# ghar1821/Chronoclust

Hardware: AMD Instinct MI355X
Metric: points clustered/sec (20-dim) (higher is better)
Workload: dtype f64; 1 GPU; C2: 1 timepoint, 1000000x20 synthetic blobs (seed 42+rank), 5000 microclusters; exact sequential semantics; online + offline phases per step; one independent st; points=1000000, dim=20, microclusters=5000, clusters=5000, streams=1

## Files before the change

### chronoclust_amd/csrc/cc_api.hip

```cpp
#include <hip/hip_runtime.h>

#include <algorithm>
#include <chrono>
#include <cmath>
#include <cstdio>
#include <cstdlib>
#include <cstring>
#include <limits>
#include <optional>
#include <string>
#include <thread>
#include <type_traits>
#include <vector>

#include "../../include/chronoclust_hip.h"
#include "cc_comm.h"
#include "cc_common.h"
#include "cc_csv.h"
#include "cc_offline.h"
#include "cc_online.h"
#include "cc_policy.h"

#include "cc_handle.h"

namespace {


template <int DP, bool DIRTY>
void launch_scan_dp(cc_handle* h, hipStream_t st, int win, Rows rows, const Cand* clean, Cand* part, int S, int round,
                    int mode, int shard_rank, int shard_world, int phase);

template <int DP>
int scan_u_wgs_per_cu()
{
    constexpr int NW = ScanShape<DP, false>::NW;
    static int blocks = 0;
    static const bool ok = hipOccupancyMaxActiveBlocksPerMultiprocessor(&blocks, k_scan_u<DP, NW>, 64 * NW, 0) == hipSuccess && blocks >= 1;
    return ok ? blocks : ScanUShape<DP>::WGS;
}

template <int DP>
ScanPlan scan_plan_dp(const cc_handle* h)
{
    ScanPlan p;
    p.dp = DP;
    const bool filter = h->hc.filter != 0, pow2 = h->hc.pow2 != 0;
    p.scan_u = h->allow_scan_u && !filter && pow2 && h->d == DP;
    if (p.scan_u && DP > 8) p.chain = ScanPlan::COMMON;
    else if (h->allow_scan_p3 && h->allow_prune_general && h->d == DP && DP > 8 && DP <= 40 && (filter || !pow2))
        p.chain = ScanPlan::GENERAL;
    const bool p3 = h->allow_scan_p3 && DP <= 40;
    p.form = p3 ? ScanPlan::P3 : (h->allow_scan_p2 && DP <= 40 ? ScanPlan::P2 : ScanPlan::P1);
    if (p.chain == ScanPlan::COMMON && h->split_a_mode == 2) p.split_rows = 0;
    else if (p.chain == ScanPlan::COMMON && h->split_a_mode == 1 && !p3) p.split_rows = 10000;
    p.listed_rows = h->p3_listed_rows;
    const bool p3_sized = p3 && h->split_a_mode != 2;
    p.seed16 = h->allow_seed16 && (p.chain == ScanPlan::GENERAL || p3_sized);
    p.prune_applicable = p.chain != ScanPlan::NONE ? 1 : 0;
    p.allow_guess = (h->allow_guess && p.chain != ScanPlan::GENERAL) ? (h->allow_lean ? 1 : 2) : 0;
    p.allow_probe = (h->allow_probe && p.chain != ScanPlan::GENERAL) ? 1 : 0;
    p.force_prune_rows = (p.prune_applicable && h->allow_seed16 && p3_sized) ? h->force_prune_rows : 0;
    p.waves = ScanShape<DP, false>::NW;
    p.dirty_waves = ScanShape<DP, true>::NW;
    p.plain_wgs_per_cu = p.scan_u ? scan_u_wgs_per_cu<DP>() : ScanShape<DP, false>::WGS;
    p.prune_wgs_per_cu = h->prune_rounds4 > 0 ? h->prune_rounds4 : (DP <= 20 ? (p3_sized ? 8 : 16) : 24);
    return p;
}

ScanPlan scan_plan(const cc_handle* h)
{
    const int d = h->d;
    return d <= 4 ? scan_plan_dp<4>(h) : d <= 8 ? scan_plan_dp<8>(h) : d <= 14 ? scan_plan_dp<14>(h) : d <= 16 ? scan_plan_dp<16>(h)
         : d <= 20 ? scan_plan_dp<20>(h) : d <= 32 ? scan_plan_dp<32>(h) : d <= 40 ? scan_plan_dp<40>(h) : scan_plan_dp<64>(h);
}

template <int DP>
struct ScanCall {
    static constexpr int NW = ScanShape<DP, false>::NW;
    cc_handle* h; hipStream_t st; const Rows& rows;
    int round, mode, win, S;
    Cand* part;

    void scan_u(int n_pts, int srank, int sworld, const int* plist) const
    {
        hipLaunchKernelGGL((k_scan_u<DP, NW>), dim3((n_pts + 63) / 64, S), dim3(64 * NW), 0, st, h->ctl.p, h->Xt.p, rows.cen,
                           rows.scl, rows.kind, rows.key, part, round, mode, h->part_stride, srank, sworld, plist);
    }
    void prefix16() const
    {
        ensure_prefix16(h);
        const size_t a16_rows = h->tab.cap + 2 * CC_P16_TM;
        hipLaunchKernelGGL((k_prefix16<DP>), dim3((unsigned)((a16_rows + 255) / 256)), dim3(256), 0, st, (const Ctl*)h->ctl.p,
                           rows.cen, rows.kind, h->a16.p, h->hdr16.p, h->a16_stride, round, mode);
    }
    void seeds(int n_pts, int Sp, const int* plist, bool s16) const
    {
        const dim3 grid((n_pts + 127) / 128, Sp), block(64 * NW);
        if (s16) {
            if constexpr (DP <= 40) {
                hipLaunchKernelGGL((k_seed16<DP, NW>), grid, block, 0, st, (const Ctl*)h->ctl.p, (const double*)h->Xt.p, rows.cen, h->spart.p,
                                   round, mode, h->spart_stride, (const cc_h8*)h->a16.p, (const Prefix16Hdr*)h->hdr16.p, h->a16_stride);
                ++h->stats.seed16_launches;
            } else {
                throw HipErr{hipErrorInvalidValue, "k_seed16 is compiled up to 40 dimensions"};
            }
        } else {
            hipLaunchKernelGGL((k_seed<DP, NW>), grid, block, 0, st, h->ctl.p, h->Xt.p, rows.cen, rows.kind, h->spart.p, round, mode,
                               h->spart_stride, h->cmax.p, plist);
        }
        hipLaunchKernelGGL((k_seed_merge<DP>), dim3((2 * n_pts + 63) / 64), dim3(64), 0, st, h->ctl.p, h->X.p, rows.cen, rows.scl, h->spart.p,
                           h->spart_stride, Sp, h->thr.p, h->thr32.p, h->thr_stride, s16 ? 0.0 : h->prune_F, round, mode, h->cmax.p,
                           h->pstat_p(), plist);
    }
    template <bool LISTED, bool GENERAL>
    void scan_p3(unsigned lds, int srank, int sworld, double gF, unsigned long long* found) const
    {
        hipLaunchKernelGGL((k_scan_p3<DP, NW, LISTED, GENERAL>), dim3((win + 127) / 128, S), dim3(64 * NW), lds, st, h->ctl.p, h->Xt.p,
                           rows.cen, rows.scl, rows.kind, rows.key, h->thr.p, h->thr_stride, part, round, mode, h->part_stride, srank,
                           sworld, h->pstat_p(), gF, found, (const cc_h8*)h->a16.p, (const Prefix16Hdr*)h->hdr16.p, h->a16_stride,
                           GENERAL ? (const double*)h->X.p : nullptr, GENERAL ? rows.cf1 : nullptr, GENERAL ? rows.cf2 : nullptr,
                           GENERAL ? rows.w : nullptr);
    }
    void scan_p(int n_pts, int Sp, Cand* p, size_t p_stride, int srank, int sworld, const int* plist, double gF,
                unsigned long long* found) const
    {
        hipLaunchKernelGGL((k_scan_p<DP, NW, false>), dim3((n_pts + 63) / 64, Sp), dim3(64 * NW), 0, st, h->ctl.p, h->Xt.p, rows.cen,
                           rows.scl, rows.kind, rows.key, h->thr.p, h->thr32.p, h->thr_stride, p, round, mode, p_stride, srank, sworld,
                           h->pstat_p(), plist, gF, found, (const unsigned*)nullptr, (size_t)0, 0, 1);
    }
    void scan_split(int srank, int sworld, double gF, unsigned long long* found) const
    {
        const int nsub = S * NW;
        const int tps = cc_mask_tiles_per_sub((int)std::min<size_t>(h->tab.cap, (size_t)INT_MAX - 64), nsub);
        const size_t need = (size_t)((win + 127) / 128) * (size_t)nsub * (size_t)tps;
        if (need > h->mask_stride) { h->masks.ensure(2 * need); h->mask_stride = need; }
        hipLaunchKernelGGL((k_scan_a<DP, NW>), dim3((win + 127) / 128, S), dim3(64 * NW), 0, st, (const Ctl*)h->ctl.p,
                           (const double*)h->Xt.p, rows.cen, rows.kind, (const double*)h->thr.p, h->thr_stride, h->masks.p,
                           h->mask_stride, tps, round, mode, srank, sworld, gF);
        int q = 1;
        const int tiles = (win + 63) / 64;
        const int resident = h->n_cus * (DP <= 20 ? CC_SCANP_WGS20 : (DP <= 40 ? 3 : 2));
        for (int c = 1; c <= S; ++c)
            if (S % c == 0 && 2 * tiles * (S / c) >= 3 * resident) q = c;
        static const int q_env = []() { const char* e = getenv("CHRONOCLUST_HIP_SCANB_Q"); return e ? atoi(e) : 0; }();
        if (q_env > 0 && S % q_env == 0) q = q_env;
        hipLaunchKernelGGL((k_scan_p<DP, NW, true>), dim3(tiles, S / q), dim3(64 * NW), 0, st, h->ctl.p, h->Xt.p, rows.cen, rows.scl,
                           rows.kind, rows.key, h->thr.p, h->thr32.p, h->thr_stride, part, round, mode, h->part_stride, srank, sworld,
                           h->pstat_p(), (const int*)nullptr, gF, found, (const unsigned*)h->masks.p, h->mask_stride, tps, q);
    }
};

template <int DP, bool DIRTY>
void launch_scan_dp(cc_handle* h, hipStream_t st, int win, Rows rows, const Cand* clean, Cand* part, int S, int round,
                    int mode, int shard_rank, int shard_world, int phase)
{
    constexpr int NW = ScanShape<DP, DIRTY>::NW;
    const dim3 block(64 * NW);
    constexpr int TILE = 64 * ScanShape<DP, DIRTY>::PT;
    const dim3 grid((win + TILE - 1) / TILE, S);
    if constexpr (!DIRTY) {
        static_assert(ScanShape<DP, false>::PT == 1, "k_scan_u holds one window point per lane");
        const ScanPlan& pl = h->scan_plan;
        const ScanCall<DP> L{h, st, rows, round, mode, win, S, part};
        if (pl.scan_u) ++h->stats.scan_u_launches;
        if constexpr (DP > 8) {
            auto window_scan = [&](int srank, int sworld, double gF, unsigned long long* found, bool have_prefix16) {
                if (pl.split(h->hc.m_rows)) return L.scan_split(srank, sworld, gF, found);
                if constexpr (DP <= 40) {
                    if (pl.form == ScanPlan::P3) {
                        if (!have_prefix16) L.prefix16();
                        const bool listed = pl.listed(h->hc.m_rows);
                        if (pl.chain == ScanPlan::GENERAL) {
                            if (listed) L.template scan_p3<true, true>(0, srank, sworld, gF, found);
                            else L.template scan_p3<false, true>(0, srank, sworld, gF, found);
                        } else {
                            static const char* const lds_kb = getenv("CHRONOCLUST_HIP_SCAN_LDS_KB");
                            static const unsigned p3_lds = lds_kb ? (unsigned)atoi(lds_kb) * 1024u : 0u;
                            if (listed) L.template scan_p3<true, false>(p3_lds, srank, sworld, gF, found);
                            else L.template scan_p3<false, false>(p3_lds, srank, sworld, gF, found);
                        }
                        ++h->stats.scan_p2_launches;
                        return;
                    }
                    if (pl.form == ScanPlan::P2) {
                        hipLaunchKernelGGL((k_scan_p2<DP, NW>), dim3((win + 127) / 128, S), block, 0, st, h->ctl.p, h->Xt.p, rows.cen, rows.scl,
                                           rows.kind, rows.key, h->thr.p, h->thr_stride, part, round, mode, h->part_stride, srank, sworld,
                                           h->pstat_p(), gF, found);
                        ++h->stats.scan_p2_launches;
                        return;
                    }
                }
                L.scan_p(win, S, part, h->part_stride, srank, sworld, nullptr, gF, found);
            };
            auto seeded_chain = [&](int n_pts, const int* plist, Cand* p, size_t p_stride, int Sp, int srank, int sworld) {
                const bool whole_window = plist == nullptr && n_pts == win && p_stride == h->part_stride && Sp == S;
                const bool s16 = whole_window && pl.seed16;
                const bool have_prefix16 = whole_window && (s16 || pl.chain == ScanPlan::GENERAL);
                if constexpr (DP <= 40) if (have_prefix16) L.prefix16();
                L.seeds(n_pts, Sp, plist, s16);
                if (whole_window) window_scan(srank, sworld, 0.0, nullptr, have_prefix16);
                else L.scan_p(n_pts, Sp, p, p_stride, srank, sworld, plist, 0.0, nullptr);
            };
            auto missed_scan = [&](const int* list) {
                if (!h->allow_missed_plain) return seeded_chain(CC_MISSED_CAP, list, part, h->part_stride, S, shard_rank, shard_world);
                ++h->stats.missed_plain_launches;
                L.scan_u(CC_MISSED_CAP, shard_rank, shard_world, list);
            };
            if (pl.chain == ScanPlan::GENERAL && h->prune_now && phase == 0) {
                ++h->stats.scan_p_launches;
                return seeded_chain(win, nullptr, part, h->part_stride, S, shard_rank, shard_world);
            }
            if (pl.chain == ScanPlan::COMMON) {
                if (phase == 1) {
                    hipLaunchKernelGGL(k_missed_g, dim3(1), dim3(1024), 0, st, h->ctl.p, (const Cand*)h->gpart.p, h->gpart_stride,
                                       (size_t)win * 4 + 4, shard_world, h->missed.p, CC_MISSED_CAP, round, mode, h->found.p);
                    return missed_scan(h->missed.p);
                }
                if (!h->prune_now) {
                    L.scan_u(win, shard_rank, shard_world, nullptr);
                    if (!h->probe_now) return;
                    ++h->stats.probe_launches;
                    const int Sp = (int)std::max<size_t>(1, std::min<size_t>(128, h->spart_stride / 2 / 128));
                    h->probe_part.ensure((size_t)2 * 128 * Sp * 4);
                    return seeded_chain(std::min(win, 128), nullptr, h->probe_part.p, (size_t)128 * Sp * 4, Sp, 0, 1);
                }
                ++h->stats.scan_p_launches;
                if (!h->guess_now) return seeded_chain(win, nullptr, part, h->part_stride, S, shard_rank, shard_world);
                ++h->stats.scan_g_launches;
                unsigned long long* const found = h->lean_now ? nullptr : h->found.p;
                if (h->group_guess_now) {
                    hipLaunchKernelGGL(k_pstat_zero, dim3(1), dim3(2), 0, st, (const Ctl*)h->ctl.p, h->pstat_p(), round, mode);
                    return window_scan(shard_rank, shard_world, h->prune_F, found, false);
                }
                window_scan(0, 1, h->prune_F, found, false);
                if (h->lean_now) { ++h->stats.scan_lean_launches; return; }
                hipLaunchKernelGGL(k_missed, dim3(1), dim3(1024), 0, st, h->ctl.p, h->found.p, h->missed.p, CC_MISSED_CAP, round, mode);
                return missed_scan(h->missed.p);
            }
        }
// ... 386 lines not shown
```

### chronoclust_amd/csrc/cc_api_comm.inc

```

namespace {

void comm_all_reduce_sum(cc_handle* h, double* buf, size_t count, hipStream_t st)
{
    cc::Comm& cm = h->comm;
    if (cm.broken) throw cc::CommErr{"the group has failed earlier"};
    if (cm.rccl()) {
        cm.check(cc::RcclApi::get().AllReduce(buf, buf, count, ncclDouble, ncclSum, cm.lane(0), st), "ncclAllReduce");
        return;
    }
    if (!cm.local || cm.world == 1) return;
    h->r_gather.ensure((size_t)cm.world * count);
    cm.all_gather(buf, h->r_gather.p, count * 8, st);
    hipLaunchKernelGGL(k_sum_ranks, dim3((unsigned)((count + 255) / 256)), dim3(256), 0, st, h->r_gather.p, cm.world, count, buf);
}

int online_relaxed(cc_handle* h)
{
    const long long N = h->n_points;
    const int W = h->comm.world, rank = h->comm.rank, d = h->d;
    if (N == 0) return (int)CC_OK;
    if (d == 0) return fail(h, CC_ERR_BAD_ARG, "no points uploaded");
    const long long L = (N + W - 1) / W;
    const long long a0 = std::min(N, (long long)rank * L), e0 = std::min(N, a0 + L);
// ... 69 lines not shown
        }
        if (h->trace) {
            const auto tA3 = std::chrono::steady_clock::now();
            auto ms = [](auto x, auto y) { return std::chrono::duration<double, std::milli>(y - x).count(); };
            fprintf(stderr, "[cc] relaxed super-step %lld: %lld points | snapshot %.3f ms, sharded half %.3f ms, merge + collect %.3f ms, set aside %lld\n",
                    sidx, e - a, ms(tA0, tA1), ms(tA1, tA2), ms(tA2, tA3), total);
        }
        h->rstats.super_steps += 1;
        h->rstats.minibatch_points += e - a;
        const long long K = (long long)list.size();
        if (K > 0) {
            h->rstats.deferred_points += K;
            h->r_didx_all.ensure((size_t)std::max<long long>((long long)W * (b + 1), K));
            HIPCHK(hipMemcpyAsync(h->r_didx_all.p, list.data(), (size_t)K * 4, hipMemcpyHostToDevice, st));
            h->rg_X.ensure((size_t)K * d); h->rg_Xt.ensure((size_t)K * d); h->rg_uid.ensure((size_t)K); h->rg_path.ensure((size_t)K);
            hipLaunchKernelGGL(k_rel_gather_points, dim3((unsigned)(((size_t)K * d + 255) / 256)), dim3(256), 0, st, h->X.p,
                               h->r_didx_all.p, (int)K, d, h->rg_X.p);
            hipLaunchKernelGGL(k_transpose_points, dim3((unsigned)(((size_t)K * d + 255) / 256)), dim3(256), 0, st, h->rg_X.p,
                               h->rg_Xt.p, K, d);
            auto swap_in = [&]() {
                h->X.swap(h->rg_X);
                h->Xt.swap(h->rg_Xt);
                h->lab_uid.swap(h->rg_uid);
                h->lab_path.swap(h->rg_path);
            };
            swap_in();
            h->n_points = K;
            const int keep_win = h->adapt_win, keep_clean = h->clean_batches, keep_shrink = h->since_shrink;
            auto restore_policy = [&]() { h->adapt_win = keep_win; h->clean_batches = keep_clean; h->since_shrink = keep_shrink; };
            try {
                rc = online_range(h, 0, K, false, false);
            } catch (...) {
                swap_in();
                h->n_points = N;
                restore_policy();
                throw;
            }
            swap_in();
            h->n_points = N;
            restore_policy();
            if (rc != CC_OK) return rc;
            hipLaunchKernelGGL(k_rel_scatter_labels, dim3((unsigned)((K + 255) / 256)), dim3(256), 0, st, h->rg_uid.p,
                               h->rg_path.p, h->r_didx_all.p, (int)K, h->lab_uid.p, h->lab_path.p);
        }
    }
    h->comm.all_gather(h->lab_uid.p + (size_t)rank * L, h->lab_uid.p, (size_t)L * 8, st);
    h->comm.all_gather(h->lab_path.p + (size_t)rank * L, h->lab_path.p, (size_t)L, st);
    sync_stream(h, st);
    HIPCHK(hipGetLastError());
    h->stats.points = N;
    return (int)CC_OK;
}

}

extern "C" {


int cc_comm_unique_id(void* out_id)
{
    if (!out_id) return CC_ERR_BAD_ARG;
    cc::RcclApi& api = cc::RcclApi::get();
    if (!api.ok()) return CC_ERR_COMM;
    ncclUniqueId id;
    if (api.GetUniqueId(&id) != ncclSuccess) return CC_ERR_COMM;
    static_assert(sizeof(id) == CC_COMM_ID_BYTES, "ncclUniqueId size");
    memcpy(out_id, &id, sizeof(id));
    return CC_OK;
}

int cc_comm_init_rccl(cc_handle* h, const void* id_bytes, int rank, int world)
{
    if (!h || !id_bytes || world < 1 || rank < 0 || rank >= world) return CC_ERR_BAD_ARG;
    return guarded(h, [&]() {
        if (h->comm.active()) return fail(h, CC_ERR_BAD_ARG, "the handle already belongs to a group");
        cc::RcclApi& api = cc::RcclApi::get();
        if (!api.ok()) return fail(h, CC_ERR_COMM, std::string("librccl could not be loaded: ") + (dlerror() ? dlerror() : "missing symbol"));
        ncclUniqueId id;
        memcpy(&id, id_bytes, sizeof(id));
        ncclComm_t comm = nullptr;
        ncclResult_t r = api.CommInitRank(&comm, world, id, rank);
        if (r != ncclSuccess) return fail(h, CC_ERR_COMM, std::string("ncclCommInitRank: ") + api.GetErrorString(r));
        h->comm.nccl[0] = comm;
        h->comm.rank = rank;
        h->comm.world = world;
        h->comm.broken = false;
        const char* to = getenv("CHRONOCLUST_HIP_COMM_TIMEOUT_S");
        if (to && atof(to) > 0.0) h->comm.timeout_s = atof(to);
        const char* two = getenv("CHRONOCLUST_HIP_TWO_COMMS");
        if (two && two[0] == '1') {
            DevBuf<char> ids;
            ids.ensure((size_t)world * sizeof(ncclUniqueId) + sizeof(ncclUniqueId));
            ncclUniqueId id2;
            memset(&id2, 0, sizeof id2);
            if (rank == 0) {
                r = api.GetUniqueId(&id2);
                if (r != ncclSuccess) return fail(h, CC_ERR_COMM, std::string("ncclGetUniqueId: ") + api.GetErrorString(r));
            }
            char* send = ids.p + (size_t)world * sizeof(ncclUniqueId);
            HIPCHK(hipMemcpyAsync(send, &id2, sizeof id2, hipMemcpyHostToDevice, h->stream));
            h->comm.all_gather(send, ids.p, sizeof id2, h->stream, 0);
            HIPCHK(hipMemcpyAsync(&id2, ids.p, sizeof id2, hipMemcpyDeviceToHost, h->stream));
            sync_stream(h, h->stream);
            ncclComm_t comm2 = nullptr;
            r = api.CommInitRank(&comm2, world, id2, rank);
            if (r != ncclSuccess) return fail(h, CC_ERR_COMM, std::string("ncclCommInitRank (second communicator): ") + api.GetErrorString(r));
            h->comm.nccl[1] = comm2;
        }
        const char* cal = getenv("CHRONOCLUST_HIP_CALIBRATE");
        if (!(cal && cal[0] == '0')) {
            const int rc = cc_comm_calibrate(h);
            if (rc != CC_OK) return rc;
        }
        return (int)CC_OK;
    });
}

int cc_comm_calibrate(cc_handle* h)
{
    if (!h) return CC_ERR_BAD_ARG;
    return guarded(h, [&]() {
        if (!h->comm.active()) return fail(h, CC_ERR_BAD_ARG, "cc_comm_calibrate: the handle belongs to no group");
        const int world = h->comm.world, rank = h->comm.rank;
        hipEvent_t e0 = nullptr, e1 = nullptr;
        HIPCHK(hipEventCreate(&e0));
        HIPCHK(hipEventCreate(&e1));
        auto timed3 = [&](auto&& fn) {
            fn();
            sync_stream(h, h->stream);
            float best = 1e30f;
            for (int i = 0; i < 3; ++i) {
                HIPCHK(hipEventRecord(e0, h->stream));
                fn();
                HIPCHK(hipEventRecord(e1, h->stream));
                sync_stream(h, h->stream);
                float ms = 0.f;
                HIPCHK(hipEventElapsedTime(&ms, e0, e1));
                best = std::min(best, ms);
            }
            return (double)best * 1e3;
        };
        const int win = std::min(h->tun.window, CC_MAX_WINDOW);
        const size_t rec = ((size_t)win * 4 + 4) * sizeof(Cand);
        DevBuf<char> sbuf, rbuf;
        sbuf.ensure(rec);
        rbuf.ensure(rec * (size_t)world);
        HIPCHK(hipMemsetAsync(sbuf.p, 0, rec, h->stream));
        const double ag_us = timed3([&]() { h->comm.all_gather(sbuf.p, rbuf.p, rec, h->stream, 0); });
        constexpr int DPc = 20, Rc = 4096;
        constexpr int NWc = ScanShape<DPc, false>::NW;
        DevBuf<Ctl> cctl;
        DevBuf<double> cxt, ccen, cscl;
        DevBuf<int> ckind, ckey;
        DevBuf<Cand> cpart;
        const int tiles = (win + 63) / 64;
        const int Sc = std::max(1, std::min(16, (h->n_cus * scan_u_wgs_per_cu<DPc>()) / std::max(1, tiles)));
        cctl.ensure(1); cxt.ensure((size_t)win * DPc); ccen.ensure((size_t)Rc * DPc); cscl.ensure((size_t)Rc * DPc);
        ckind.ensure(Rc); ckey.ensure(Rc); cpart.ensure((size_t)2 * win * Sc * 4);
        {
            std::vector<double> x((size_t)win * DPc), cen((size_t)Rc * DPc), scl((size_t)Rc * DPc, 0.25);
            unsigned long long st = 0x9E3779B97F4A7C15ull;
            auto rnd = [&]() { st = st * 6364136223846793005ull + 1442695040888963407ull; return (double)(st >> 11) * 0x1p-53; };
            for (auto& v : x) v = 0.1 + 0.8 * rnd();
            for (auto& v : cen) v = 0.1 + 0.8 * rnd();
            std::vector<int> kind(Rc, CC_KIND_PCORE), key(Rc);
            for (int i = 0; i < Rc; ++i) key[i] = i;
            Ctl c;
            memset(&c, 0, sizeof c);
            c.d = DPc; c.m_rows = Rc; c.win_b = win; c.win_cfg = win; c.n_points = win; c.xt_stride = win;
            c.k = 4.0; c.inv_k = 0.25; c.pow2 = 1;
            HIPCHK(hipMemcpyAsync(cctl.p, &c, sizeof c, hipMemcpyHostToDevice, h->stream));
            HIPCHK(hipMemcpyAsync(cxt.p, x.data(), x.size() * 8, hipMemcpyHostToDevice, h->stream));
            HIPCHK(hipMemcpyAsync(ccen.p, cen.data(), cen.size() * 8, hipMemcpyHostToDevice, h->stream));
            HIPCHK(hipMemcpyAsync(cscl.p, scl.data(), scl.size() * 8, hipMemcpyHostToDevice, h->stream));
            HIPCHK(hipMemcpyAsync(ckind.p, kind.data(), (size_t)Rc * 4, hipMemcpyHostToDevice, h->stream));
            HIPCHK(hipMemcpyAsync(ckey.p, key.data(), (size_t)Rc * 4, hipMemcpyHostToDevice, h->stream));
            sync_stream(h, h->stream);
        }
        const double scan_us = timed3([&]() {
            hipLaunchKernelGGL((k_scan_u<DPc, NWc>), dim3(tiles, Sc), dim3(64 * NWc), 0, h->stream, (const Ctl*)cctl.p, (const double*)cxt.p,
                               (const double*)ccen.p, (const double*)cscl.p, (const int*)ckind.p, (const int*)ckey.p, cpart.p, 0, 0,
                               (size_t)win * Sc * 4, 0, 1);
        });
        HIPCHK(hipGetLastError());
        (void)hipEventDestroy(e0);
        (void)hipEventDestroy(e1);
        double mine[2] = {ag_us, scan_us * 1e3 / ((double)Rc * DPc)};
        DevBuf<double> dsend, drecv;
        dsend.ensure(2);
        drecv.ensure((size_t)2 * world);
        HIPCHK(hipMemcpyAsync(dsend.p, mine, sizeof mine, hipMemcpyHostToDevice, h->stream));
        h->comm.all_gather(dsend.p, drecv.p, sizeof mine, h->stream, 0);
        std::vector<double> all((size_t)2 * world);
        HIPCHK(hipMemcpyAsync(all.data(), drecv.p, all.size() * 8, hipMemcpyDeviceToHost, h->stream));
        sync_stream(h, h->stream);
        double ag = 0.0, sc = 0.0;
        for (int r = 0; r < world; ++r) { ag = std::max(ag, all[(size_t)2 * r]); sc = std::max(sc, all[(size_t)2 * r + 1]); }
        h->calib_ag_us = ag;
        h->calib_scan_ns = sc;
        if (world > 1 && sc > 0.0) {
            const double row_dims = ag * 1e3 * (double)world / (double)(world - 1) / sc;
            h->shard_min_row_dims = (long long)std::min(row_dims, 1e15);
            h->shard_min_row_dims_pruned = (long long)std::min(row_dims * 3.3, 1e15);
        }
        if (h->trace)
            fprintf(stderr, "[cc] rank %d of %d: all-gather of a %d-point window's records %.1f us, plain scan %.3f ns per (row, dim) "
                    "(group maxima) -> scans split from %lld (plain) / %lld (pruned) row-dims on\n", rank, world, win, ag, sc,
                    (long long)h->shard_min_row_dims, (long long)(h->shard_min_row_dims_pruned > 0 ? h->shard_min_row_dims_pruned : h->shard_min_row_dims));
        return (int)CC_OK;
    });
}

int cc_comm_init_local(cc_handle** handles, int world)
{
    if (!handles || world < 1) return CC_ERR_BAD_ARG;
    for (int r = 0; r < world; ++r)
        if (!handles[r] || handles[r]->comm.active()) return CC_ERR_BAD_ARG;
    auto grp = std::make_shared<cc::LocalGroup>(world);
    for (int r = 0; r < world; ++r) {
        cc_handle* h = handles[r];
        int rc = guarded(h, [&]() {
            HIPCHK(hipEventCreateWithFlags(&h->comm.ev_ready, hipEventDisableTiming));
            HIPCHK(hipEventCreateWithFlags(&h->comm.ev_done, hipEventDisableTiming));
            return (int)CC_OK;
        });
        if (rc != CC_OK) {
            for (int q = 0; q <= r; ++q) handles[q]->comm.destroy();
            return rc;
        }
    }
    for (int r = 0; r < world; ++r) {
        handles[r]->comm.local = grp;
        handles[r]->comm.rank = r;
        handles[r]->comm.world = world;
    }
    return CC_OK;
}

int cc_comm_destroy(cc_handle* h)
{
    if (!h) return CC_ERR_BAD_ARG;
    return guarded(h, [&]() {
        try {
            sync_stream(h, h->stream);
            sync_stream(h, h->stream2);
        } catch (const cc::CommErr&) {
        }
        h->comm.destroy();
        return (int)CC_OK;
    });
}

int cc_comm_info(cc_handle* h, int32_t* rank, int32_t* world, int32_t* transport)
{
    if (!h) return CC_ERR_BAD_ARG;
    if (rank) *rank = h->comm.rank;
    if (world) *world = h->comm.world;
    if (transport) *transport = h->comm.rccl() ? 1 : (h->comm.local ? 2 : 0);
    return CC_OK;
}

int cc_comm_set_relaxed(cc_handle* h, int32_t minibatch_points)
{
    if (!h || minibatch_points < 0) return CC_ERR_BAD_ARG;
    if (minibatch_points > 0 && !h->comm.active()) return fail(h, CC_ERR_BAD_ARG, "the relaxed mode needs a group (cc_comm_init_*)");
    h->relaxed_minibatch = minibatch_points;
    return CC_OK;
}

int cc_get_relaxed_stats(cc_handle* h, cc_relaxed_stats* out)
{
    if (!h || !out) return CC_ERR_BAD_ARG;
    *out = h->rstats;
    return CC_OK;
}

int cc_set_shard_thresholds(cc_handle* h, int64_t min_row_dims, int32_t offline_min_rows)
{
    if (!h) return CC_ERR_BAD_ARG;
    if (min_row_dims >= 0) { h->shard_min_row_dims = min_row_dims; h->shard_min_row_dims_pruned = 0; }
    if (offline_min_rows >= 0) h->offline_shard_min_rows = offline_min_rows;
    return CC_OK;
}

}
```

### chronoclust_amd/csrc/cc_common.h

```cpp
#pragma once
#include <hip/hip_runtime.h>
#include <stdint.h>

#include "cc_host.h"

#define CC_KIND_PCORE 0
#define CC_KIND_OUTLIER 1
#define CC_KIND_DEAD 2

#define CC_MAX_ROUNDS 8
#define CC_T_UNKNOWN (-2)
#define CC_T_NONE (-3)
#define CC_IDX_INF 0x7fffffff

#define CC_SLOT_BOUND (-2)
struct __attribute__((aligned(16))) Cand {
    double dist;
    int key;
    int slot;
};

struct Table {
    double* cf1;
    double* cf2;
    double* cen;
    double* pref;
    double* scl;
    double* w;
    int* kind;
    int* key;
    long long* id;
    long long* uid;
    unsigned long long* touch;
    unsigned long long* last;
    unsigned long long* carry_of;
    unsigned long long* cnt;
    int* memb;
    int* clen;
    int* heavy;
    size_t cap;
};
#define CC_HEAVY_CAP 64
#define CC_HEAVY_NEW 32

#define CC_CAR_BASE (1 << 24)
#define CC_MAX_WINDOW 49152
#define CC_CHAIN_MEMB 32
#define CC_LONG_CAP 512
#define CC_LONG_LISTED (1ull << 23)
#ifndef CC_CHAIN_AHEAD
#define CC_CHAIN_AHEAD 4
#endif

struct Carry {
    double* cf1;
    double* cf2;
    double* cen;
    double* pref;
    double* scl;
    double* w;
    int* kind;
    int* key;
    int* slot;
    double* c0;
    double* w0;
    int* kind0;
    double* dsq;
    unsigned long long* tile_dsq;
};

struct Versions {
    double* cf1;
    double* cf2;
    double* cen;
    double* pref;
    double* scl;
    double* w;
    int* kind;
    int* key;
    int* next;
    int* upg;
    int* acc;
    int* tgt;
    double* dsq;
    unsigned long long* tile_dsq;
    double* tau;
    int* skip;
    int* skip_car;
    int* unsafe;
};

struct Rows {
    const double* cen;
    const double* scl;
    const double* pref;
    const double* cf1;
    const double* cf2;
    const double* w;
    const int* kind;
    const int* key;
    const int* next;
    const unsigned long long* tile_dsq;
    const double* dsq;
    const double* tau;
    const int* skip;
    const int* plist;
    const int* slot;
    const unsigned long long* touch;
    size_t cap;
};

struct Ctl {
    long long cursor;
    long long n_points;
    long long xt_stride;
    int no_create;
    int pad1;
    int d;
    int m_rows;
    int n_pkeys, n_okeys;
    long long pcore_last_id, outlier_last_id;
    unsigned long long window_seq;
    int win_cfg;
    int win_b;
    int max_rounds;
    int last_round;
    int fc[CC_MAX_ROUNDS + 2];
    int any_new[CC_MAX_ROUNDS + 2], any_up[CC_MAX_ROUNDS + 2];
    int n_long[CC_MAX_ROUNDS + 2];
    long long stat_long;
    double eps_sq, delta_sq, k, inv_k, beta_mu, mu, omicron;
    int pi;
    int filter;
    int pow2;
    int pad0;
    int mode;
    int car_n;
    int la_on;
    int stall_b;
    long long la_cursor[2];
    int la_b[2];
    int la_rows[2];
    long long stat_windows, stat_rounds, stat_truncated;
    long long stat_table_rows;
    double stat_pair_rows;
    long long round_hist[CC_MAX_ROUNDS + 2];
    long long stat_lookahead;
    long long stat_trunc_unknown;
    long long stat_unprovable, stat_unsafe;
    long long stat_tiles, stat_dirty_tiles;
    long long stat_seq_points;
    long long stat_seq_clk, stat_seq_wall;
    unsigned long long stat_prune_rows, stat_prune_full;
    int n_sparse;
    int pad2;
    double tg[2][2];
    int tg_ok[2][2];
    int n_missed[2];
    unsigned long long cen_absmax;
    double x_absmax;
    long long stat_missed;
    unsigned long long pstat[2][2];
    int n_missed_all[2];
    int seq_rest;
    int pad3;
    long long stat_seq_r_points;
    long long seed_at;
    int rdiff[CC_MAX_ROUNDS + 2];
    int n_heavy, n_heavy_new;
    int heavy_list[CC_HEAVY_CAP];
    int heavy_new[CC_HEAVY_NEW];
#ifdef CC_LONG_TIMERS
    unsigned long long dbg_long[8];
#endif
#ifdef CC_ROUND_DEBUG
    unsigned long long dbg_round[CC_MAX_ROUNDS + 2][6];
#endif
};

#define CC_MISSED_CAP 2048
#define CC_DSQ_STRIDE 4
#define CC_TAU_STRIDE 4
#define CC_FLAG_U0 1
#define CC_FLAG_U1 2
#define CC_FLAG_C0 4
#define CC_FLAG_C1 8
#define CC_FLAG_N1SKIP 32
#define CC_FLAG_SPARSE 64

__host__ __device__ inline bool cand_less(double ad, int ak, double bd, int bk)
{
    return ad < bd || (ad == bd && ak < bk);
}
```

### chronoclust_amd/csrc/cc_handle.h

```cpp
#pragma once
#include "cc_knobs.h"

namespace {

struct HipErr {
    hipError_t e;
    const char* what;
};

#define HIPCHK(call)                                  \
    do {                                              \
        hipError_t _e = (call);                       \
        if (_e != hipSuccess) throw HipErr{_e, #call}; \
    } while (0)

template <typename T>
struct DevBuf {
    T* p = nullptr;
    size_t n = 0;
    void ensure(size_t count)
    {
        if (count <= n && p) return;
        release();
        size_t want = std::max<size_t>(count, 1);
        if (hipMalloc((void**)&p, want * sizeof(T)) != hipSuccess) {
            p = nullptr;
            throw HipErr{hipErrorOutOfMemory, "hipMalloc"};
        }
        n = want;
    }
    void release()
    {
        if (p) (void)hipFree(p);
        p = nullptr;
        n = 0;
    }
    ~DevBuf() { release(); }
    DevBuf() = default;
    DevBuf(const DevBuf&) = delete;
    DevBuf& operator=(const DevBuf&) = delete;
    DevBuf(DevBuf&& o) noexcept { swap(o); }
    DevBuf& operator=(DevBuf&& o) noexcept
    {
        if (this != &o) { release(); swap(o); }
        return *this;
    }
    void swap(DevBuf& o) noexcept
    {
        std::swap(p, o.p);
        std::swap(n, o.n);
    }
};

struct TableStore {
    DevBuf<double> cf1, cf2, cen, pref, scl, w;
    DevBuf<int> kind, key;
    DevBuf<long long> id, uid;
    DevBuf<unsigned long long> touch, last, carry_of, cnt;
    DevBuf<int> memb, clen, heavy;
    size_t cap = 0;
    int d = 0;
    enum Grow { KEPT, CLEARED, CLEARED_KEPT, SCRATCH };
    template <typename F>
    static void for_each_column(int dims, F&& f)
    {
        const size_t dim = (size_t)dims;
        f(&TableStore::cf1, dim, KEPT); f(&TableStore::cf2, dim, KEPT); f(&TableStore::cen, dim, KEPT);
        f(&TableStore::pref, dim, KEPT); f(&TableStore::scl, dim, KEPT);
        f(&TableStore::w, (size_t)1, KEPT); f(&TableStore::kind, (size_t)1, KEPT); f(&TableStore::key, (size_t)1, KEPT);
        f(&TableStore::id, (size_t)1, KEPT); f(&TableStore::uid, (size_t)1, KEPT);
        f(&TableStore::touch, (size_t)2, CLEARED); f(&TableStore::last, (size_t)2, CLEARED);
        f(&TableStore::carry_of, (size_t)1, CLEARED_KEPT);
        f(&TableStore::cnt, (size_t)1, CLEARED); f(&TableStore::memb, (size_t)CC_CHAIN_MEMB, SCRATCH);
        f(&TableStore::clen, (size_t)1, CLEARED);
        f(&TableStore::heavy, (size_t)1, CLEARED_KEPT);
    }
    void alloc(size_t rows, int dim)
    {
        for_each_column(dim, [&](auto col, size_t per_row, Grow) { (this->*col).ensure(rows * per_row); });
        cap = rows;
        d = dim;
    }
    Table view() const { return Table{cf1.p, cf2.p, cen.p, pref.p, scl.p, w.p, kind.p, key.p, id.p, uid.p, touch.p, last.p, carry_of.p, cnt.p, memb.p, clen.p, heavy.p, cap}; }
};

struct HostClusters {
    std::vector<int> mem, off{0};
    size_t size() const { return off.size() - 1; }
    void clear() { mem.clear(); off.assign(1, 0); }
};

}

struct PinArena {
    char* p = nullptr;
    size_t cap = 0, used = 0;
    void reset() { used = 0; }
    void reserve(size_t bytes)
    {
        if (bytes <= cap) return;
        if (p) (void)hipHostFree(p);
        p = nullptr;
        cap = 0;
        const size_t want = std::max<size_t>(bytes, (size_t)1 << 20);
        if (hipHostMalloc((void**)&p, want, hipHostMallocDefault) != hipSuccess) {
            p = nullptr;
            throw HipErr{hipErrorOutOfMemory, "hipHostMalloc"};
        }
        cap = want;
    }
    template <typename T>
    T* take(size_t n)
    {
        used = (used + 63) & ~(size_t)63;
        T* r = reinterpret_cast<T*>(p + used);
        used += std::max<size_t>(n, 1) * sizeof(T);
        if (used > cap) throw HipErr{hipErrorOutOfMemory, "page-locked scratch exhausted"};
        return r;
    }
    ~PinArena() { if (p) (void)hipHostFree(p); }
    PinArena() = default;
    PinArena(const PinArena&) = delete;
    PinArena& operator=(const PinArena&) = delete;
};

struct ScanPlan {
    int dp = 0;
    bool scan_u = false;
    enum Chain { NONE, COMMON, GENERAL } chain = NONE;
    enum Form { P3, P2, P1 } form = P1;
    long long split_rows = std::numeric_limits<long long>::max(), listed_rows = 0;
    bool seed16 = false;
    int prune_applicable = 0, allow_guess = 0, allow_probe = 0, force_prune_rows = 0;
    int waves = 4, dirty_waves = 4;
    int plain_wgs_per_cu = 1, prune_wgs_per_cu = 1;
    bool split(long long m_rows) const { return m_rows >= split_rows; }
    bool listed(long long m_rows) const { return m_rows >= listed_rows; }
};


struct BatchScanState {
    bool prune_now = false;
    bool group_guess_now = false;
    bool lean_now = false;
    bool guess_now = false;
    bool probe_now = false;
    ScanPlan scan_plan;
    void set_prune(int prune)
    {
        prune_now = prune != 0;
        guess_now = prune >= 2;
        lean_now = prune == 3;
    }
};

struct PrunedScanBuffers {
    DevBuf<Cand> probe_part;
    DevBuf<unsigned long long> found;
    DevBuf<int> missed;
    DevBuf<SeedCand> spart;
    DevBuf<double> thr;
    DevBuf<float> thr32;
    DevBuf<unsigned long long> cmax;
    DevBuf<cc_h8> a16;
    DevBuf<Prefix16Hdr> hdr16;
    size_t a16_stride = 0;
    DevBuf<unsigned> masks;
    size_t mask_stride = 0;
    size_t spart_stride = 0, thr_stride = 0;
};

struct WindowBuffers {
    int win_alloc = 0, seg_alloc = 0, d_alloc = 0;
    DevBuf<double> v_cf1, v_cf2, v_cen, v_pref, v_scl, v_w, v_dsq, v_tau;
    DevBuf<unsigned long long> v_tile_dsq;
    DevBuf<int> v_kind, v_key, v_next, v_upg, v_acc, v_tgt, v_skip, v_skip_car, v_unsafe;
    DevBuf<Cand> part, clean, dpart, dpart2, dseed;
    size_t part_stride = 0;
    DevBuf<double> c_cf1v, c_cf2v, c_cenv, c_prefv, c_sclv, c_wv, c_c0, c_w0, c_dsq;
    DevBuf<int> c_kind, c_key, c_slot, c_kind0;
    DevBuf<unsigned long long> c_tile_dsq;
    DevBuf<int> T0, T1, rk;
    DevBuf<int> link_near;
    DevBuf<int> sp_list;
    DevBuf<int> long_list;
    DevBuf<unsigned long long> lstat, lprev;
    bool prep_launched = false;
    DevBuf<CommitRec> rec;
    DevBuf<double> sh_cen[2], sh_scl[2], sh_cf1[2], sh_cf2[2], sh_w[2];
    DevBuf<int> sh_kind[2], sh_key[2];
    DevBuf<int8_t> dpath;
};

struct OfflineResults {
    DevBuf<double> pv_cf1, pv_cf2, pv_cen, pv_pref, pv_w, wvec;
    DevBuf<long long> pv_id;
    DevBuf<int> prow, nn, pdim, mem_dev, off_dev, nw_cnt, nw_nbr;
    DevBuf<long long> nw_off;
    DevBuf<int8_t> core;
    DevBuf<unsigned long long> adj, adjw;
    DevBuf<double> c_cf1, c_cf2, c_cen, c_pref, c_w;
    HostClusters clusters;
    PinArena pin;
    std::vector<long long> pcore_ids_host, pcore_uid_host;
    DevBuf<int32_t> pc_map, pc_out;
    int n_core = 0;
};

struct AssocScratch {
    DevBuf<double> a_cur_cen, a_cur_pref, a_prev_cen, a_dist, a_pdist;
    DevBuf<int> a_idx, a_pidx;
    DevBuf<int> flags;
};

struct RelaxedState {
    int relaxed_minibatch = 0;
    bool shard_suspended = false;
    DevBuf<double> rs_cf1, rs_cf2, rs_w, r_delta, r_gather;
    DevBuf<int> rs_kind, rs_key, r_didx, r_didx_all, r_cnt_all;
    DevBuf<long long> rs_id;
    DevBuf<double> rg_X, rg_Xt;
    DevBuf<long long> rg_uid;
    DevBuf<int8_t> rg_path;
    cc_relaxed_stats rstats{};
};

struct cc_handle : Knobs, BatchScanState, PrunedScanBuffers, WindowBuffers, OfflineResults, AssocScratch, RelaxedState {
    int device = 0;
    hipStream_t stream = nullptr;
    hipStream_t stream2 = nullptr;
    std::string err;
    cc_params par{};
    bool have_par = false;
    cc_tuning tun{};
    cc_stats stats{};

    int d = 0;
    TableStore tab, tab2;
    Ctl hc{};
    Ctl* hc_pin = nullptr;
    DevBuf<Ctl> ctl;
    unsigned long long* pstat_p() const { return (unsigned long long*)((char*)ctl.p + offsetof(Ctl, pstat)); }
    bool tainted = false;
    int adapt_win = 0;
    int clean_batches = 0;
    int since_shrink = 1000;
    DevBuf<int> seq_lists;
    DevBuf<double> seq_img;
    bool seq_sticky = false;
    int n_cus = 256;

    DevBuf<double> X, Xt;
    long long n_points = 0;
    double x_absmax = 0.0;
    DevBuf<long long> lab_uid;
    DevBuf<int8_t> lab_path;
    DevBuf<int> badflag;
    DevBuf<double> scr, scr2;

    struct Prefetch {
        std::thread worker;
        bool active = false;
        const double* x = nullptr;
        long long n = 0;
        int d = 0;
        bool scaled = false;
        std::vector<double> scale, mn;
        DevBuf<double> X, Xt, sm;
        DevBuf<int> bad;
        hipStream_t stream = nullptr;
        void* pin[2] = {nullptr, nullptr};
        size_t pin_bytes = 0;
        int bad_host[4] = {0, 0, 0, 0};
        int rc = 0;
        const char* what = "";
    } pf;

    std::vector<hipEvent_t> ev_pool, sync_pool;

    cc::Comm comm;
    long long shard_min_row_dims = 400000;
    long long shard_min_row_dims_pruned = 0;
    double calib_ag_us = 0.0, calib_scan_ns = 0.0;
    int offline_shard_min_rows = 8192;
    DevBuf<Cand> gsend, gpart;
    DevBuf<Cand> gsend2, gpart2;
    size_t gsend_stride = 0, gpart_stride = 0;
    DevBuf<int> g_i32;
};

namespace {

template <typename F>
void with_bools(F&& f)
{
    f();
}
template <typename F, typename... Rest>
void with_bools(F&& f, bool b, Rest... rest)
{
    if (b) with_bools([&](auto... c) { f(std::true_type{}, c...); }, rest...);
    else with_bools([&](auto... c) { f(std::false_type{}, c...); }, rest...);
}

struct CapacityErr {
    std::string what;
};

int fail(cc_handle* h, int code, const std::string& msg)
{
    if (h) h->err = msg;
    return code;
}

void group_lost(cc_handle* h)
{
    if (h && h->comm.active()) h->comm.fail_group();
}

template <typename F>
int guarded(cc_handle* h, F&& f)
{
    try {
        if (h) HIPCHK(hipSetDevice(h->device));
        const int rc = f();
        if (rc < 0) group_lost(h);
        return rc;
    } catch (const HipErr& e) {
        char buf[512];
        snprintf(buf, sizeof buf, "HIP error %d (%s) in %s", (int)e.e, hipGetErrorString(e.e), e.what);
        group_lost(h);
        return fail(h, e.e == hipErrorOutOfMemory ? CC_ERR_OOM : CC_ERR_NO_DEVICE, buf);
    } catch (const cc::CommErr& e) {
        group_lost(h);
        return fail(h, CC_ERR_COMM, "exchange between ranks failed: " + e.what);
    } catch (const std::bad_alloc&) {
        group_lost(h);
        return fail(h, CC_ERR_OOM, "host allocation failed");
    } catch (const CapacityErr& e) {
        group_lost(h);
        return fail(h, CC_ERR_OOM, e.what);
    }
}

void sync_stream(cc_handle* h, hipStream_t st)
{
    if (h->comm.rccl() || h->comm.broken) h->comm.wait_stream(st);
    else HIPCHK(hipStreamSynchronize(st));
}

bool is_pow2(double k)
{
    if (!(k > 0.0) || !std::isfinite(k)) return false;
    int e;
    double m = std::frexp(k, &e);
    return m == 0.5 && e > -1000 && e < 1000;
}

void refresh_ctl_params(cc_handle* h)
{
    Ctl& c = h->hc;
    const cc_params& p = h->par;
    c.eps_sq = p.eps_sq;
    c.delta_sq = p.delta_sq;
    c.k = p.k;
    c.pow2 = (is_pow2(p.k) && !h->tainted) ? 1 : 0;
    c.inv_k = c.pow2 ? 1.0 / p.k : 0.0;
    c.beta_mu = p.beta * p.mu;
    c.mu = p.mu;
    c.omicron = p.omicron;
    c.pi = p.pi;
    c.filter = (h->d > 0 && p.pi < h->d) ? 1 : 0;
    c.d = h->d;
}

void push_ctl(cc_handle* h)
{
    memset(h->hc.pstat, 0, sizeof(h->hc.pstat));
    h->hc.n_missed_all[0] = h->hc.n_missed_all[1] = 0;
    HIPCHK(hipMemcpyAsync(h->ctl.p, &h->hc, sizeof(Ctl), hipMemcpyHostToDevice, h->stream));
}
void pull_ctl(cc_handle* h)
{
    HIPCHK(hipMemcpyAsync(&h->hc, h->ctl.p, sizeof(Ctl), hipMemcpyDeviceToHost, h->stream));
    sync_stream(h, h->stream);
}
void pull_ctl_pinned(cc_handle* h)
{
    if (!h->hc_pin) { pull_ctl(h); return; }
    HIPCHK(hipMemcpyAsync(h->hc_pin, h->ctl.p, sizeof(Ctl), hipMemcpyDeviceToHost, h->stream));
    sync_stream(h, h->stream);
    memcpy(&h->hc, h->hc_pin, sizeof(Ctl));
}
void push_ctl_pinned(cc_handle* h)
{
    if (!h->hc_pin) { push_ctl(h); return; }
    memset(h->hc.pstat, 0, sizeof(h->hc.pstat));
    h->hc.n_missed_all[0] = h->hc.n_missed_all[1] = 0;
    memcpy(h->hc_pin + 1, &h->hc, sizeof(Ctl));
    HIPCHK(hipMemcpyAsync(h->ctl.p, h->hc_pin + 1, sizeof(Ctl), hipMemcpyHostToDevice, h->stream));
}

#define CC_MAX_TABLE_ELEMS ((size_t)INT_MAX - 1023)

void ensure_table(cc_handle* h, size_t rows)
{
    if (h->tab.cap >= rows && h->tab.d == h->d) return;
    const size_t max_rows = CC_MAX_TABLE_ELEMS / (size_t)std::max(h->d, 1);
    if (rows > max_rows)
        throw CapacityErr{"a table of " + std::to_string(rows) + " rows of " + std::to_string(h->d) + " dimensions: more than " +
                          std::to_string(max_rows) + " rows (" + std::to_string(CC_MAX_TABLE_ELEMS) + " elements) at this width"};
    size_t want = std::min(max_rows, std::max<size_t>(rows, std::max<size_t>(1024, h->tab.cap * 2)));
    TableStore nt;
    nt.alloc(want, h->d);
    const size_t m = (size_t)h->hc.m_rows;
    TableStore& old = h->tab;
    TableStore::for_each_column(h->d, [&](auto col, size_t per_row, TableStore::Grow grow) {
        auto& to = nt.*col;
        const size_t elem = sizeof(*to.p);
        if (grow == TableStore::CLEARED || grow == TableStore::CLEARED_KEPT)
            HIPCHK(hipMemsetAsync(to.p, 0, want * per_row * elem, h->stream));
        if ((grow == TableStore::KEPT || grow == TableStore::CLEARED_KEPT) && m > 0)
            HIPCHK(hipMemcpyAsync(to.p, (old.*col).p, m * per_row * elem, hipMemcpyDeviceToDevice, h->stream));
    });
    sync_stream(h, h->stream);
    std::swap(h->tab, nt);
}

int set_dim(cc_handle* h, int d)
{
    if (d <= 0 || d > CC_MAX_DIM) return fail(h, CC_ERR_BAD_ARG, "d must be in 1.." + std::to_string(CC_MAX_DIM));
    if (h->d == 0) h->d = d;
    if (h->d != d) {
        if (h->hc.m_rows == 0) h->d = d;
        else return fail(h, CC_ERR_BAD_ARG, "dimensionality differs from the microclusters already held");
    }
    return CC_OK;
}

void ensure_window_buffers(cc_handle* h, int win, int seg)
{
    if (win <= h->win_alloc && seg <= h->seg_alloc && h->d <= h->d_alloc) return;
    win = std::max(win, h->win_alloc);
    seg = std::max(seg, h->seg_alloc);
    const size_t w = (size_t)win, d = (size_t)std::max(h->d, h->d_alloc);
    h->v_cf1.ensure(w * d); h->v_cf2.ensure(w * d); h->v_cen.ensure(w * d); h->v_pref.ensure(w * d); h->v_scl.ensure(w * d); h->v_w.ensure(w);
    h->v_kind.ensure(w); h->v_key.ensure(w); h->v_next.ensure(w); h->v_upg.ensure(w); h->v_acc.ensure(w);
    h->v_dsq.ensure(w); h->v_tau.ensure(CC_TAU_STRIDE * w); h->v_tile_dsq.ensure(CC_DSQ_STRIDE * (w / 16 + 2));
    h->v_tgt.ensure(w);
    h->v_skip.ensure(w / 64 + 2); h->v_skip_car.ensure(w / 64 + 2); h->v_unsafe.ensure(w);
    h->part_stride = w * seg * 4;
    h->spart_stride = w * seg * 2;
    h->thr_stride = w * 2;
    h->spart.ensure(2 * h->spart_stride);
    h->thr.ensure(2 * h->thr_stride);
    h->thr32.ensure(2 * h->thr_stride);
    h->cmax.ensure(2);
    h->found.ensure(2 * (CC_MAX_WINDOW / 64));
    h->missed.ensure(2 * CC_MISSED_CAP);
    h->part.ensure(2 * h->part_stride); h->dpart.ensure(w * seg * 2); h->dpart2.ensure(w * seg * 2);
    h->clean.ensure(w * 4); h->dseed.ensure(w * 4);
    h->c_cf1v.ensure(w * d); h->c_cf2v.ensure(w * d); h->c_cenv.ensure(w * d); h->c_prefv.ensure(w * d);
    h->c_sclv.ensure(w * d); h->c_wv.ensure(w); h->c_c0.ensure(w * d); h->c_w0.ensure(w * d);
    h->c_kind.ensure(w); h->c_key.ensure(w); h->c_slot.ensure(w); h->c_kind0.ensure(w); h->c_dsq.ensure(w); h->c_tile_dsq.ensure(CC_DSQ_STRIDE * (w / 16 + 2));
    h->T0.ensure(w + 128); h->T1.ensure(w + 128);
    h->long_list.ensure(2 * CC_LONG_CAP);
    h->lstat.ensure(2 * CC_LSTAT_ROWS + 2);
    h->lprev.ensure(CC_MAX_WINDOW);
    h->dpath.ensure(w); h->rk.ensure(w); h->rec.ensure(1); h->sp_list.ensure(w); h->link_near.ensure(w);
    h->win_alloc = win; h->seg_alloc = seg; h->d_alloc = (int)d;
}

Carry carry_view(cc_handle* h)
{
    return Carry{h->c_cf1v.p, h->c_cf2v.p, h->c_cenv.p, h->c_prefv.p, h->c_sclv.p, h->c_wv.p, h->c_kind.p, h->c_key.p,
                 h->c_slot.p, h->c_c0.p, h->c_w0.p, h->c_kind0.p, h->c_dsq.p, h->c_tile_dsq.p};
}

void scan_copy_sync(cc_handle* h, ScanCopy (&out)[2])
{
    const size_t cap = h->tab.cap, d = (size_t)h->d, m = (size_t)h->hc.m_rows;
    const bool filter = h->hc.filter != 0;
    const TableStore& t = h->tab;
    for (int q = 0; q < 2; ++q) {
        h->sh_cen[q].ensure(cap * d); h->sh_scl[q].ensure(cap * d); h->sh_kind[q].ensure(cap); h->sh_key[q].ensure(cap);
        if (filter) { h->sh_cf1[q].ensure(cap * d); h->sh_cf2[q].ensure(cap * d); h->sh_w[q].ensure(cap); }
        if (m > 0) {
            HIPCHK(hipMemcpyAsync(h->sh_cen[q].p, t.cen.p, m * d * 8, hipMemcpyDeviceToDevice, h->stream));
            HIPCHK(hipMemcpyAsync(h->sh_scl[q].p, t.scl.p, m * d * 8, hipMemcpyDeviceToDevice, h->stream));
            HIPCHK(hipMemcpyAsync(h->sh_kind[q].p, t.kind.p, m * 4, hipMemcpyDeviceToDevice, h->stream));
            HIPCHK(hipMemcpyAsync(h->sh_key[q].p, t.key.p, m * 4, hipMemcpyDeviceToDevice, h->stream));
            if (filter) {
                HIPCHK(hipMemcpyAsync(h->sh_cf1[q].p, t.cf1.p, m * d * 8, hipMemcpyDeviceToDevice, h->stream));
                HIPCHK(hipMemcpyAsync(h->sh_cf2[q].p, t.cf2.p, m * d * 8, hipMemcpyDeviceToDevice, h->stream));
                HIPCHK(hipMemcpyAsync(h->sh_w[q].p, t.w.p, m * 8, hipMemcpyDeviceToDevice, h->stream));
            }
        }
        out[q] = ScanCopy{h->sh_cen[q].p, h->sh_scl[q].p, h->sh_cf1[q].p, h->sh_cf2[q].p, h->sh_w[q].p, h->sh_kind[q].p,
                          h->sh_key[q].p};
    }
}

Versions versions_view(cc_handle* h)
{
    return Versions{h->v_cf1.p, h->v_cf2.p, h->v_cen.p, h->v_pref.p, h->v_scl.p, h->v_w.p, h->v_kind.p,
                    h->v_key.p, h->v_next.p, h->v_upg.p, h->v_acc.p, h->v_tgt.p, h->v_dsq.p, h->v_tile_dsq.p,
                    h->v_tau.p, h->v_skip.p, h->v_skip_car.p, h->v_unsafe.p};
}

void ensure_prefix16(cc_handle* h)
{
    const size_t a16_rows = h->tab.cap + 2 * CC_P16_TM;
    if (h->a16_stride >= a16_rows * 4) return;
    sync_stream(h, h->stream);
    sync_stream(h, h->stream2);
    h->a16.ensure(2 * a16_rows * 4);
    h->a16_stride = a16_rows * 4;
    h->hdr16.ensure(2);
}

hipEvent_t get_event(cc_handle* h, size_t i)
{
    while (h->ev_pool.size() <= i) {
        hipEvent_t e;
        HIPCHK(hipEventCreateWithFlags(&e, h->light_sync_events ? hipEventReleaseToDevice : hipEventDefault));
        h->ev_pool.push_back(e);
    }
    return h->ev_pool[i];
}

hipEvent_t get_sync_event(cc_handle* h, size_t i)
{
    if (!h->light_sync_events) return get_event(h, i);
    while (h->sync_pool.size() <= i) {
        hipEvent_t e;
        HIPCHK(hipEventCreateWithFlags(&e, hipEventDisableTiming | hipEventReleaseToDevice));
        h->sync_pool.push_back(e);
    }
    return h->sync_pool[i];
}


}
```

### chronoclust_amd/csrc/cc_knobs.h

```cpp
#pragma once
#include <algorithm>
#include <climits>
#include <cstdlib>

struct Knobs {
    bool trace = false;
    bool light_sync_events = true;
    int chain_threads = 64, decide_threads = 256, commit_threads = 256;
    bool allow_scan_u = true;
    int prune_mode = 1;
    double prune_F = 16.0;
    int prune_rounds4 = 0;
    bool group_guess_always = false;
    bool allow_guess = true;
    bool allow_lean = true;
    int force_prune_rows = 0;
    bool allow_seed16 = false;
    bool allow_prune_general = true;
    bool la_pruned = false;
    bool allow_probe = true;
    int split_a_mode = 1;
    bool allow_nodirty = true;
    bool allow_claims = true;
    bool allow_long = true;
    bool allow_prep = true;
    bool allow_quiet = true;
    bool allow_missed_plain = true;
    int p3_listed_rows = 10000;
    bool allow_scan_p3 = true;
    bool allow_scan_p2 = true;
    bool allow_link = true;
    bool allow_heavy = true;
    bool allow_seq_r = true;
    bool allow_seq_g = true;
    int allow_sparse = 128;
};

namespace {

void knob_off_when_starts_with_0(bool& v, const char* name) { const char* e = getenv(name); v = !(e && e[0] == '0'); }
void knob_on_when_starts_with_1(bool& v, const char* name) { const char* e = getenv(name); v = e && e[0] == '1'; }
void knob_atoi_nonzero_when_set(bool& v, const char* name) { if (const char* e = getenv(name)) v = atoi(e) != 0; }
void knob_int_in(int& v, const char* name, int lo, int hi) { const char* e = getenv(name); if (e && atoi(e) >= lo && atoi(e) <= hi) v = atoi(e); }
void knob_threads(int& v, const char* name) { int t = 0; knob_int_in(t, name, 64, 256); if (t == 64 || t == 128 || t == 256) v = t; }

void read_knobs(Knobs& k)
{
    knob_on_when_starts_with_1(k.trace, "CHRONOCLUST_HIP_TRACE");
    knob_on_when_starts_with_1(k.group_guess_always, "CHRONOCLUST_HIP_GROUP_GUESS");
    knob_off_when_starts_with_0(k.allow_nodirty, "CHRONOCLUST_HIP_NODIRTY");
    knob_off_when_starts_with_0(k.allow_claims, "CHRONOCLUST_HIP_CLAIMS");
    knob_off_when_starts_with_0(k.allow_long, "CHRONOCLUST_HIP_LONGCHAINS");
    knob_off_when_starts_with_0(k.allow_prep, "CHRONOCLUST_HIP_LONGPREP");
    knob_off_when_starts_with_0(k.allow_quiet, "CHRONOCLUST_HIP_QUIET");
    knob_off_when_starts_with_0(k.allow_heavy, "CHRONOCLUST_HIP_HEAVY");
    knob_off_when_starts_with_0(k.allow_seq_r, "CHRONOCLUST_HIP_SEQR");
    knob_off_when_starts_with_0(k.allow_seq_g, "CHRONOCLUST_HIP_SEQG");
    knob_off_when_starts_with_0(k.allow_probe, "CHRONOCLUST_HIP_PROBE");
    knob_off_when_starts_with_0(k.allow_guess, "CHRONOCLUST_HIP_GUESS");
    knob_off_when_starts_with_0(k.allow_lean, "CHRONOCLUST_HIP_LEAN");
    knob_off_when_starts_with_0(k.allow_scan_p2, "CHRONOCLUST_HIP_SCANP2");
    knob_off_when_starts_with_0(k.allow_link, "CHRONOCLUST_HIP_LINK");
    knob_atoi_nonzero_when_set(k.light_sync_events, "CHRONOCLUST_HIP_LIGHT_EVENTS");
    knob_atoi_nonzero_when_set(k.allow_scan_u, "CHRONOCLUST_HIP_SCANU");
    knob_atoi_nonzero_when_set(k.allow_seed16, "CHRONOCLUST_HIP_SEED16");
    knob_atoi_nonzero_when_set(k.allow_missed_plain, "CHRONOCLUST_HIP_MISSED_PLAIN");
    knob_atoi_nonzero_when_set(k.allow_prune_general, "CHRONOCLUST_HIP_PRUNE_GENERAL");
    knob_atoi_nonzero_when_set(k.allow_scan_p3, "CHRONOCLUST_HIP_SCANP3");
    knob_atoi_nonzero_when_set(k.la_pruned, "CHRONOCLUST_HIP_LA_PRUNED");
    knob_threads(k.chain_threads, "CHRONOCLUST_HIP_CHAIN_THREADS");
    knob_threads(k.decide_threads, "CHRONOCLUST_HIP_DECIDE_THREADS");
    knob_threads(k.commit_threads, "CHRONOCLUST_HIP_COMMIT_THREADS");
    knob_int_in(k.prune_mode, "CHRONOCLUST_HIP_PRUNE", 0, 2);
    knob_int_in(k.prune_rounds4, "CHRONOCLUST_HIP_PRUNE_WGS", 1, 64);
    knob_int_in(k.allow_sparse, "CHRONOCLUST_HIP_SPARSE", 0, INT_MAX);
    knob_int_in(k.force_prune_rows, "CHRONOCLUST_HIP_FORCE_PRUNE_ROWS", INT_MIN, INT_MAX);
    knob_int_in(k.p3_listed_rows, "CHRONOCLUST_HIP_P3_LISTED", INT_MIN, INT_MAX);
    if (const char* e = getenv("CHRONOCLUST_HIP_SCANA")) k.split_a_mode = std::max(0, std::min(2, atoi(e)));
    if (const char* e = getenv("CHRONOCLUST_HIP_PRUNE_F")) if (atof(e) >= 1.0) k.prune_F = atof(e);
}

}
```

### chronoclust_amd/csrc/cc_online.h

```cpp
#pragma once
#include <type_traits>

#include "cc_common.h"

#define CC_INF (__builtin_huge_val())
#define CC_GROUP_THREADS 256

#define CC_LATENCY_KERNEL() __builtin_amdgcn_s_setprio(3)

#define CC_WAVE_SYNC()                                          \
    do {                                                        \
        __builtin_amdgcn_fence(__ATOMIC_RELEASE, "wavefront"); \
        __builtin_amdgcn_wave_barrier();                        \
        __builtin_amdgcn_fence(__ATOMIC_ACQUIRE, "wavefront"); \
    } while (0)


__device__ __forceinline__ double cc_sqvar(double cf1, double cf2, double w)
{
    double a = cf2 / w;
    double b = cf1 / w;
    b = b * b;
    return a - b;
}

struct Par {
    double delta_sq, k, inv_k, eps_sq, beta_mu;
    int pow2, pi, filter, d;
};

__device__ __forceinline__ Par cc_load_par(const Ctl* ctl)
{
    Par p;
    p.delta_sq = ctl->delta_sq; p.k = ctl->k; p.inv_k = ctl->inv_k; p.eps_sq = ctl->eps_sq; p.beta_mu = ctl->beta_mu;
    p.pow2 = ctl->pow2; p.pi = ctl->pi; p.filter = ctl->filter; p.d = ctl->d;
    return p;
}

__device__ __forceinline__ double cc_div_pref(double x, double pref, const Par& c)
{
    if (pref == 1.0) return x;
    return (c.pow2 && pref == c.k) ? x * c.inv_k : x / pref;
}

__device__ inline double cc_tentative_radius(const double* bcf1, const double* bcf2, double bw, const double* p,
                                             int d, const Par& c, int* cnt_gt1, int* cnt_ne1)
{
    const double w1 = bw + 1.0;
    double r2 = 0.0;
    int g = 0, n = 0;
    for (int i = 0; i < d; ++i) {
        double x = p[i];
        double c1 = (bcf1 ? bcf1[i] : 0.0) + x;
        double c2 = (bcf2 ? bcf2[i] : 0.0) + x * x;
        double var = cc_sqvar(c1, c2, w1);
        double pr = (var <= c.delta_sq) ? c.k : 1.0;
        g += (pr > 1.0);
        n += (pr != 1.0);
        r2 = r2 + cc_div_pref(var, pr, c);
    }
    if (cnt_gt1) *cnt_gt1 = g;
    if (cnt_ne1) *cnt_ne1 = n;
    return r2;
}

__device__ __forceinline__ void cc_top2_push(Cand& a, Cand& b, const Cand& x)
{
    const bool ok = x.slot != -1;
    const bool beats_a = ok && (a.slot == -1 || cand_less(x.dist, x.key, a.dist, a.key));
    const bool beats_b = ok && !beats_a && (b.slot == -1 || cand_less(x.dist, x.key, b.dist, b.key));
    b.dist = beats_a ? a.dist : (beats_b ? x.dist : b.dist);
    b.key = beats_a ? a.key : (beats_b ? x.key : b.key);
    b.slot = beats_a ? a.slot : (beats_b ? x.slot : b.slot);
    a.dist = beats_a ? x.dist : a.dist;
    a.key = beats_a ? x.key : a.key;
    a.slot = beats_a ? x.slot : a.slot;
}

__device__ __forceinline__ double cc_vmin(double a, double b)
{
    double r;
    asm("v_min_f64 %0, %1, %2" : "=v"(r) : "v"(a), "v"(b));
    return r;
}
__device__ __forceinline__ double cc_vmax(double a, double b)
{
    double r;
    asm("v_max_f64 %0, %1, %2" : "=v"(r) : "v"(a), "v"(b));
    return r;
}

template <int N, int I = 0, typename F>
__device__ __forceinline__ void cc_static_for(F&& f)
{
    if constexpr (I < N) {
        f(std::integral_constant<int, I>{});
        cc_static_for<N, I + 1>(f);
    }
}

#define CC_TINY 0x1p-400
__device__ __forceinline__ bool cc_is_tiny(double v) { return v != 0.0 && __builtin_fabs(v) < CC_TINY; }

__device__ __forceinline__ unsigned long long cc_dsq_code(double dq) { return (unsigned long long)__double_as_longlong(dq) + 1ull; }
__device__ __forceinline__ bool cc_dsq_below(unsigned long long code, double tau)
{
    if (code == 0ull) return true;
    const double dq = __longlong_as_double((long long)(code - 1ull));
    return dq < CC_INF && sqrt(dq) * (1.0 + 1e-9) < tau;
}

__device__ __forceinline__ int cc_dsq_class(int kind, double dsq_stored)
{
    return (kind == CC_KIND_PCORE) ? (__builtin_signbit(dsq_stored) ? 2 : 0) : 1;
}
__device__ __forceinline__ double cc_dsq_store(double dq, int kind, int kind0, int* cls)
{
    const bool promoted = kind == CC_KIND_PCORE && kind0 == CC_KIND_OUTLIER && dq < CC_INF;
    *cls = (kind == CC_KIND_PCORE) ? (promoted ? 2 : 0) : 1;
    return promoted ? -dq : dq;
}
template <int BIT>
__device__ __forceinline__ double cc_sel_scale(unsigned mask, double scaled, double one)
{
    double r;
    asm("s_bitcmp1_b32 %1, %2\n\ts_cselect_b64 %0, %3, %4" : "=s"(r) : "s"(mask), "n"(BIT), "s"(scaled), "s"(one) : "scc");
    return r;
}

#include "cc_scan.h"
#include "cc_scan16.h"
#include "cc_validate.h"
#include "cc_link.h"
#include "cc_seq.h"
#include "cc_seq_r.h"
#include "cc_seq_g.h"
#include "cc_relaxed.h"
#include "cc_points.h"
```

### chronoclust_amd/csrc/cc_online_run.h

```cpp
#pragma once

namespace {

struct PolicyTrace {
    FILE* f = nullptr;
    static void obs_json(FILE* f, const cc_policy_obs& o)
    {
        fprintf(f, "{\"cursor\": %lld, \"m_rows\": %d, \"stall_b\": %d, \"stat_windows\": %lld, \"stat_truncated\": %lld, "
                   "\"stat_trunc_unknown\": %lld, \"stat_tiles\": %lld, \"stat_dirty_tiles\": %lld, \"stat_unsafe\": %lld, \"stat_missed\": %lld, \"tg_ok\": %d, \"round_hist\": [",
                (long long)o.cursor, o.m_rows, o.stall_b, (long long)o.stat_windows, (long long)o.stat_truncated,
                (long long)o.stat_trunc_unknown, (long long)o.stat_tiles, (long long)o.stat_dirty_tiles, (long long)o.stat_unsafe,
                (long long)o.stat_missed, o.tg_ok);
        for (int r = 0; r < CC_POLICY_MAX_ROUNDS + 2; ++r) fprintf(f, "%s%lld", r ? ", " : "", (long long)o.round_hist[r]);
        fprintf(f, "], \"prune_rows\": %llu, \"prune_full\": %llu, \"after_sequential\": %d}", (unsigned long long)o.prune_rows,
                (unsigned long long)o.prune_full, o.after_sequential);
    }
    static void dec_json(FILE* f, const cc_policy_decision& d)
    {
        fprintf(f, "{\"win_cfg\": %d, \"want\": %d, \"rounds\": %d, \"batch_windows\": %d, \"lookahead\": %d, \"nodirty\": %d, "
                   "\"prune\": %d, \"shard\": %d, \"restart\": %d, \"bad\": %d, \"stalled\": %d, \"sparse\": %d, \"probe\": %d}",
                d.win_cfg, d.want, d.rounds, d.batch_windows, d.lookahead, d.nodirty, d.prune, d.shard, d.restart, d.bad, d.stalled, d.sparse, d.probe);
    }
    PolicyTrace(const cc_policy_config& c, const cc_policy_carry& k, long long cursor, int rows, const cc_policy_decision& d0,
                int rank)
    {
        const char* path = getenv("CHRONOCLUST_HIP_POLICY_TRACE");
        if (!path || !path[0]) return;
        const std::string name = rank >= 0 ? std::string(path) + ".rank" + std::to_string(rank) : std::string(path);
        f = fopen(name.c_str(), "a");
        if (!f) return;
        fprintf(f, "{\"call\": {\"config\": {\"window\": %d, \"rounds_max\": %d, \"windows_per_sync\": %d, \"early_window\": %d, "
                   "\"lookahead\": %d, \"allow_nodirty\": %d, \"prune_mode\": %d, \"prune_applicable\": %d, \"can_shard\": %d, \"d\": %d, "
                   "\"resume\": %d, \"allow_sparse\": %d, \"allow_guess\": %d, \"allow_probe\": %d, \"shard_min_row_dims\": %lld, \"n_end\": %lld, \"shard_min_row_dims_pruned\": %lld, \"lookahead_pruned\": %d, \"force_prune_rows\": %d}, \"carry\": [%d, %d, %d], \"start\": [%lld, %d], \"dec\": ",
                c.window, c.rounds_max, c.windows_per_sync, c.early_window, c.lookahead, c.allow_nodirty, c.prune_mode,
                c.prune_applicable, c.can_shard, c.d, c.resume, c.allow_sparse, c.allow_guess, c.allow_probe, (long long)c.shard_min_row_dims, (long long)c.n_end, (long long)c.shard_min_row_dims_pruned, c.lookahead_pruned, c.force_prune_rows,
                k.adapt_win, k.clean_batches, k.since_shrink, cursor, rows);
        dec_json(f, d0);
        fprintf(f, "}}\n");
    }
    void batch(const cc_policy_obs& o, const cc_policy_decision& d)
    {
        if (!f) return;
        fprintf(f, "{\"obs\": ");
        obs_json(f, o);
        fprintf(f, ", \"dec\": ");
        dec_json(f, d);
        fprintf(f, "}\n");
    }
    void sequential(long long cursor, int rows, const cc_policy_decision& d)
    {
        cc_policy_obs o{};
        o.cursor = cursor;
        o.m_rows = rows;
        o.after_sequential = 1;
        batch(o, d);
    }
    ~PolicyTrace()
    {
        if (f) fclose(f);
    }
    PolicyTrace(const PolicyTrace&) = delete;
    PolicyTrace& operator=(const PolicyTrace&) = delete;
};

void launch_link_scan(cc_handle* h, hipStream_t st, int win)
{
    const dim3 grid((win + 63) / 64, (win + 4 * CC_LINK_SUB - 1) / (4 * CC_LINK_SUB)), block(256);
    const int d = h->d;
#define CC_LINK_DP(DP) hipLaunchKernelGGL((k_link_scan<DP>), grid, block, 0, st, (const Ctl*)h->ctl.p, (const double*)h->X.p, \
                                          (const double*)h->Xt.p, (const int*)h->T0.p, h->link_near.p)
    if (d <= 4) CC_LINK_DP(4);
    else if (d <= 8) CC_LINK_DP(8);
    else if (d <= 14) CC_LINK_DP(14);
    else if (d <= 16) CC_LINK_DP(16);
    else if (d <= 20) CC_LINK_DP(20);
    else if (d <= 32) CC_LINK_DP(32);
    else if (d <= 40) CC_LINK_DP(40);
    else CC_LINK_DP(64);
#undef CC_LINK_DP
}

struct OnlineRun {
    cc_handle* const h;
    const long long range_a, N;
    const bool no_create, resume;
    Ctl& c;

    int win = 0, R = 0;
    int S_cfg = 1, Sd_full = 1, Sd = 1;
    int world = 1, myrank = 0;
    bool grouped = false;
    size_t batch_max = 2;
    bool timing = false;
    int seq_mode = 0, seq_cap = 0;
    Versions ver{};
    Carry car{};
    hipStream_t sA = nullptr, sB = nullptr;
    static constexpr size_t ev_base = 4;

    cc_policy_config pcfg{};
    std::optional<cc::WindowPolicy> policy;
    std::optional<PolicyTrace> ptrace;
    cc_policy_decision dec{};
    bool nodirty = false;
    bool sparse_now = false;
    bool la_on = false;
    bool shard_on = false;
    bool link_now = false;
    int Rcur = 1;
    int batch_windows = 2;

    long long done = 0;
    int m_known = 0;
    unsigned long long seq_host = 0;
    long long cursor_prev = 0;
    double batch_t0 = 0.0;

    hipEvent_t ev0 = nullptr, ev1 = nullptr, evCommit = nullptr, evScan = nullptr;
    size_t ev_used = 2, ev_sync = ev_base;
    std::vector<std::pair<size_t, double>> timed;
    std::vector<size_t> timed_comm;
    double pair_rows_eff = 0.0, pair_rows_prev = 0.0;
    double pair_rows_pruned = 0.0;
    long long sharded_windows = 0;

    bool seq_on = false;
    int bad_batches = 0;
    long long seq_stint_len = 32768, seq_stint_left = 32768;
    bool seq_probe = false;
    double win_rate = 0.0, seq_rate_last = 0.0;

    long long long_prev = 0;
    bool long_seen = false;
    bool long_few = true;
    long long rounds_prev = 0, long_avg = 1;
    long long long_launches = 0;

    OnlineRun(cc_handle* handle, long long a, long long e, bool no_create_, bool resume_)
        : h(handle), range_a(a), N(e), no_create(no_create_), resume(resume_), c(handle->hc) {}

    static double now_ms()
    {
        return std::chrono::duration<double, std::milli>(std::chrono::steady_clock::now().time_since_epoch()).count();
    }
    bool seq_r_applies() const { return h->allow_seq_r && h->d >= 2 && h->d <= 4; }
    bool wide() const { return h->d > CC_WINDOW_MAX_DIM; }
    size_t window_rows() const { return wide() ? 0 : (size_t)win * batch_max; }
    bool seq_g_applies() const { return h->allow_seq_g && h->hc.m_rows >= seq_cap; }
    double seq_rate_guess() const { return cc::seq_rate_guess(h->d, h->hc.m_rows, seq_cap, h->allow_seq_r, h->allow_seq_g); }
    bool seq_possible() const { return seq_mode != 1 && !h->comm.active() && !no_create && (h->hc.m_rows < seq_cap || h->allow_seq_g); }

    void set_lookahead(bool on)
    {
        la_on = on;
        c.la_on = on ? 1 : 0;
        c.stall_b = 0;
        c.mode = 0;
        c.car_n = 0;
        const int q = (int)((c.window_seq + 1ull) & 1ull);
        const long long c1 = c.cursor + c.win_b;
        const long long left1 = c.n_points - c1;
        c.la_cursor[q] = c1;
        c.la_b[q] = (on && left1 > 0) ? (int)std::min<long long>(left1, c.win_cfg) : 0;
        c.la_rows[q] = c.m_rows;
        c.la_cursor[q ^ 1] = 0;
        c.la_b[q ^ 1] = 0;
        c.la_rows[q ^ 1] = 0;
    }

    void prepare()
    {
        refresh_ctl_params(h);
        h->scan_plan = scan_plan(h);
        const ScanPlan& plan = h->scan_plan;
        win = h->tun.window; R = h->tun.rounds;
        S_cfg = std::max(1, h->tun.segments / plan.waves);
        Sd_full = std::max(1, (h->tun.dirty_segments > 0 ? h->tun.dirty_segments : h->tun.segments) / plan.dirty_waves);
        Sd = Sd_full;
        nodirty = false;
        ensure_window_buffers(h, wide() ? 64 : win, std::max(S_cfg, Sd_full));
        world = h->comm.world; myrank = h->comm.rank;
        grouped = h->comm.active();
        if (grouped) {
            const size_t gmax = (size_t)std::max(64, h->win_alloc);
            h->gsend_stride = gmax * 4 + 4;
            h->gpart_stride = (size_t)world * (gmax * 4 + 4);
            h->gsend.ensure(2 * h->gsend_stride);
            h->gpart.ensure(2 * h->gpart_stride);
            h->gsend2.ensure((size_t)2 * CC_MISSED_CAP * 4);
            h->gpart2.ensure((size_t)2 * world * CC_MISSED_CAP * 4);
        }
        batch_max = (size_t)std::max(2, h->tun.windows_per_sync);
        ensure_table(h, (size_t)h->hc.m_rows + window_rows() + 1);

        c.cursor = range_a;
        c.n_points = N;
        c.xt_stride = h->n_points;
        c.no_create = no_create ? 1 : 0;
        pcfg.window = win;
        pcfg.rounds_max = R;
        pcfg.windows_per_sync = h->tun.windows_per_sync;
        pcfg.early_window = h->tun.early_window;
        pcfg.lookahead = h->tun.lookahead;
        pcfg.allow_nodirty = h->allow_nodirty ? 1 : 0;
        pcfg.prune_mode = h->prune_mode;
        pcfg.prune_applicable = plan.prune_applicable;
        pcfg.can_shard = (grouped && !h->shard_suspended) ? 1 : 0;
        pcfg.d = h->d;
        pcfg.resume = resume ? 1 : 0;
        pcfg.allow_sparse = h->allow_sparse;
        pcfg.allow_guess = plan.allow_guess;
        pcfg.allow_probe = plan.allow_probe;
        pcfg.lookahead_pruned = h->la_pruned ? 1 : 0;
        pcfg.force_prune_rows = plan.force_prune_rows;
        pcfg.shard_min_row_dims = h->shard_min_row_dims;
        pcfg.shard_min_row_dims_pruned = h->shard_min_row_dims_pruned;
        pcfg.n_end = N;
        const cc_policy_carry pcarry{h->adapt_win, h->clean_batches, h->since_shrink, 0};
        policy.emplace(pcfg, pcarry);
        dec = policy->start(range_a, c.m_rows);
        ptrace.emplace(pcfg, pcarry, range_a, c.m_rows, dec, grouped ? myrank : -1);
        c.win_cfg = dec.win_cfg;
        c.win_b = (int)std::min<long long>(c.win_cfg, N - range_a);
        c.max_rounds = R;
        c.last_round = 0;
        c.fc[0] = 0;
        for (int i = 1; i < CC_MAX_ROUNDS + 2; ++i) c.fc[i] = CC_IDX_INF;
        c.stat_windows = c.stat_rounds = c.stat_truncated = 0;
        c.stat_lookahead = 0;
        c.stat_tiles = c.stat_dirty_tiles = 0;
        c.stat_unprovable = c.stat_unsafe = 0;
        c.stat_long = 0;
        for (int i = 0; i < CC_MAX_ROUNDS + 2; ++i) c.n_long[i] = 0;
        c.stat_trunc_unknown = 0;
        c.stat_table_rows = 0;
        c.stat_seq_points = 0;
        c.stat_seq_r_points = 0;
#ifdef CC_LONG_TIMERS
        for (int i = 0; i < 8; ++i) c.dbg_long[i] = 0;
#endif
#ifdef CC_ROUND_DEBUG
        for (int i = 0; i < CC_MAX_ROUNDS + 2; ++i)
            for (int q = 0; q < 6; ++q) c.dbg_round[i][q] = 0;
#endif
        c.n_heavy = c.n_heavy_new = 0;
        HIPCHK(hipMemsetAsync(h->tab.heavy.p, 0, h->tab.cap * sizeof(int), h->stream));
        c.stat_seq_clk = c.stat_seq_wall = 0;
        c.stat_prune_rows = c.stat_prune_full = 0;
        c.stat_missed = 0;
        c.seed_at = -1;
        for (int q = 0; q < 2; ++q) {
            c.n_missed[q] = 0;
            for (int K = 0; K < 2; ++K) { c.tg[q][K] = 0.0; c.tg_ok[q][K] = 0; }
        }
        c.cen_absmax = 0ull;
        c.x_absmax = h->x_absmax;
        set_lookahead(dec.lookahead != 0);
        c.stat_pair_rows = 0.0;
        for (int i = 0; i < CC_MAX_ROUNDS + 2; ++i) c.round_hist[i] = 0;
        push_ctl(h);

        HIPCHK(hipMemsetAsync(h->rec.p, 0, sizeof(CommitRec), h->stream));
        HIPCHK(hipMemsetAsync(h->cmax.p, 0, 2 * sizeof(unsigned long long), h->stream));
        HIPCHK(hipMemsetAsync(h->found.p, 0, h->found.n * sizeof(unsigned long long), h->stream));
        HIPCHK(hipMemsetAsync(h->lstat.p, 0, h->lstat.n * sizeof(unsigned long long), h->stream));
        HIPCHK(hipMemsetAsync(h->lprev.p, 0, h->lprev.n * sizeof(unsigned long long), h->stream));
        if (c.m_rows > 0)
            hipLaunchKernelGGL(k_rebuild_scl, dim3((c.m_rows * h->d + 255) / 256), dim3(256), 0, h->stream, h->ctl.p, h->tab.view(),
                               c.m_rows, h->d, c.pow2, c.inv_k);
        ev0 = get_event(h, 0); ev1 = get_event(h, 1);
        HIPCHK(hipEventRecord(ev0, h->stream));
        ev_used = 2;
        timing = h->tun.time_kernels != 0;
        shard_on = dec.shard != 0;

        ver = versions_view(h);
        car = carry_view(h);
        sA = h->stream; sB = h->stream2;
        evCommit = get_event(h, 2); evScan = nullptr;
        ev_sync = ev_base;
        ev_used = ev_base + 3 * (batch_max + 2);

        done = range_a;
        m_known = c.m_rows;
        seq_mode = wide() ? 2 : h->tun.sequential;
        seq_cap = wide() ? 0 : cc_seq_cap_rows(h->d);
        seq_on = seq_possible() && (seq_mode == 2 || h->seq_sticky);
        Rcur = dec.rounds;
        batch_windows = dec.batch_windows;
        h->set_prune(dec.prune);
        nodirty = dec.nodirty != 0;
        sparse_now = dec.sparse != 0;
        cursor_prev = range_a;
        seq_host = c.window_seq;
        link_now = h->allow_link && !no_create && !wide();
    }

    void sequential_stint(const Table& tab)
    {
        const int chunk = 8192;
        const double t0 = now_ms();
        const bool use_g = seq_g_applies();
        const bool f = h->hc.filter != 0, p2 = h->hc.pow2 != 0;
        if (use_g) {
            const int list_cap = (int)std::min<size_t>(h->tab.cap, (size_t)INT_MAX / 2);
            h->seq_lists.ensure(2 * (size_t)list_cap);
            h->seq_img.ensure(4 * (size_t)list_cap * (size_t)h->d);
            with_bools([&](auto F, auto P, auto W) {
                hipLaunchKernelGGL((k_seq_g<decltype(F)::value, decltype(P)::value, decltype(W)::value>), dim3(1), dim3(CC_SEQG_THREADS), 0, sA, h->ctl.p, h->X.p, tab,
                                   h->lab_uid.p, h->lab_path.p, chunk, h->seq_lists.p, list_cap, h->seq_img.p);
            }, f, p2, h->d > CC_SEQG_NARROW_DIM);
        } else {
            int follow = 0;
            auto seq_r = [&](auto D) {
                with_bools([&](auto P) {
                    hipLaunchKernelGGL((k_seq_r<decltype(D)::value, decltype(P)::value>), dim3(1), dim3(64), 0, sA, h->ctl.p, h->X.p, tab, h->lab_uid.p,
                                       h->lab_path.p, chunk);
                }, p2);
                follow = 1;
            };
            if (h->allow_seq_r) {
                if (h->d == 2) seq_r(std::integral_constant<int, 2>{});
                else if (h->d == 3) seq_r(std::integral_constant<int, 3>{});
                else if (h->d == 4) seq_r(std::integral_constant<int, 4>{});
            }
            with_bools([&](auto F, auto P) {
                hipLaunchKernelGGL((k_seq<decltype(F)::value, decltype(P)::value>), dim3(1), dim3(64), 0, sA, h->ctl.p, h->X.p, tab, h->lab_uid.p,
                                   h->lab_path.p, chunk, follow);
            }, f, p2);
        }
        HIPCHK(hipGetLastError());
        pull_ctl(h);
        const double dt = now_ms() - t0;
        const long long got = h->hc.cursor - done;
        done = h->hc.cursor;
        m_known = h->hc.m_rows;
        seq_host = h->hc.window_seq;
        cursor_prev = h->hc.cursor;
        const double seq_rate = got > 0 ? (double)got / std::max(dt, 1e-3) : 0.0;
        if (h->trace)
            fprintf(stderr, "[cc] done %lld rows %d | sequential kernel: %lld points in %.3f ms (so far %lld shader cycles, %.3f ms of kernel time)\n",
                    done, h->hc.m_rows, got, dt, (long long)h->hc.stat_seq_clk, (double)h->hc.stat_seq_wall / 1e5);
        if (got >= 1024) seq_rate_last = seq_rate;
        seq_stint_left -= got;
        if (use_g) h->stats.seq_g_points += got;
        const bool full = !seq_possible() || (got < chunk && done < N && (use_g || !h->allow_seq_g));
        const bool stint_over = seq_mode != 2 && seq_stint_left <= 0;
        if ((full || stint_over) && done < N && !wide()) {
            seq_on = false;
            seq_probe = stint_over && !full;
            bad_batches = 0;
            HIPCHK(hipMemsetAsync(h->rec.p, 0, sizeof(CommitRec), h->stream));
            h->hc.win_b = (int)std::min<long long>(h->hc.win_cfg, N - done);
            dec = policy->after_sequential(h->hc.cursor, h->hc.m_rows);
            ptrace->sequential(h->hc.cursor, h->hc.m_rows, dec);
            nodirty = dec.nodirty != 0;
            sparse_now = dec.sparse != 0;
            set_lookahead(dec.lookahead != 0);
            push_ctl(h);
        }
    }

    void enqueue_batch(const Table& tab)
    {
        batch_t0 = now_ms();
        const Rows trows{tab.cen, tab.scl, tab.pref, tab.cf1, tab.cf2, tab.w, tab.kind, tab.key, nullptr, nullptr, nullptr,
                         nullptr, nullptr, nullptr, nullptr, nullptr, 0};
        const Rows vrows{ver.cen, ver.scl, ver.pref, ver.cf1, ver.cf2, ver.w, ver.kind, ver.key, ver.next,
                         ver.tile_dsq, ver.dsq, ver.tau, ver.skip, nullptr, nullptr, nullptr, 0};
        const Rows crows{car.cen, car.scl, car.pref, car.cf1, car.cf2, car.w, car.kind, car.key, nullptr,
                         car.tile_dsq, car.dsq, ver.tau, ver.skip_car, nullptr, car.slot, tab.touch, tab.cap};
        Rows vrows_sp = vrows, crows_sp = crows;
        vrows_sp.skip = nullptr; vrows_sp.plist = h->sp_list.p;
        crows_sp.skip = nullptr; crows_sp.plist = h->sp_list.p;
        ev_sync = ev_base;
        const int gw = std::max(64, std::min(win, h->hc.win_cfg));
        const int scan_cus = h->n_cus;
        const ScanPlan& plan = h->scan_plan;
        const int S = h->prune_now ? std::max(1, std::min(S_cfg, (scan_cus * plan.prune_wgs_per_cu) / std::max(1, (gw + 63) / 64)))
                                   : scan_partials_for((gw + 63) / 64, S_cfg, scan_cus * plan.plain_wgs_per_cu);
        const int sparse_cap = std::min(CC_MAX_WINDOW / 16, std::max(64, ((gw / 16 + 63) / 64) * 64));
        const int decide_threads = h->decide_threads;
        const int dblocks = (gw + decide_threads / 32 - 1) / (decide_threads / 32);
        const int chain_threads = h->chain_threads;
        const int cblocks = (gw + chain_threads / 32 - 1) / (chain_threads / 32);
        const int commit_threads = h->commit_threads;
        const int rblocks = std::min((gw + commit_threads / 32 - 1) / (commit_threads / 32), 1024 * (256 / commit_threads));
        const int scan_rows = (h->allow_claims && h->hc.m_rows > 0 && h->hc.m_rows <= 1024) ? h->hc.m_rows : 0;
        const int long_rows = h->allow_long ? scan_rows : 0;
        const bool long_listed = h->allow_long && scan_rows == 0 && long_seen;
        const bool heavy_on = h->allow_heavy && scan_rows == 0 && h->hc.n_heavy > 0;
        int* const long_list = long_listed ? h->long_list.p : nullptr;
        const int long_cap = long_few ? (int)std::min<long long>(CC_LONG_CAP, 2 * long_avg + 8) : CC_LONG_CAP;
        ScanCopy scopy[2] = {ScanCopy{}, ScanCopy{}};
        if (la_on) scan_copy_sync(h, scopy);
        Rows srows[2];
        for (int q = 0; q < 2; ++q)
            srows[q] = Rows{scopy[q].cen, scopy[q].scl, nullptr, scopy[q].cf1, scopy[q].cf2, scopy[q].w, scopy[q].kind,
                            scopy[q].key, nullptr, nullptr, nullptr, nullptr, nullptr, nullptr, nullptr, nullptr, 0};
        evScan = nullptr;
        if (la_on) HIPCHK(hipEventRecord(evCommit, sA));
        int probe_left = (dec.probe != 0) ? 1 : 0;
        const int windows_now = (int)std::max<long long>(1, std::min<long long>(batch_windows,
                                    (N - done + (long long)std::max(1, h->hc.win_cfg) - 1) / (long long)std::max(1, h->hc.win_cfg)));
        for (int wv = 0; wv < windows_now; ++wv, ++seq_host) {
            hipEvent_t scan_end = nullptr;
            auto timed_scan = [&](hipStream_t st, int mode, int round) {
                const Rows& rws = (mode == 1) ? srows[round & 1] : trows;
                h->probe_now = probe_left > 0 && !h->prune_now;
                if (h->probe_now) --probe_left;
                const int srank = shard_on ? myrank : 0, sworld = shard_on ? world : 1;
                h->group_guess_now = shard_on && (sworld > 1 || h->group_guess_always);
                scan_end = nullptr;
                if (timing) {
                    hipEvent_t a = get_event(h, ev_used), b = get_event(h, ev_used + 1);
                    HIPCHK(hipEventRecord(a, st));
                    launch_scan<false>(h, st, gw, rws, nullptr, h->part.p, S, round, mode, srank, sworld);
                    HIPCHK(hipEventRecord(b, st));
                    timed.push_back({ev_used, h->prune_now ? 1.0 : 0.0});
                    ev_used += 2;
                    if (!shard_on) scan_end = b;
                } else {
                    launch_scan<false>(h, st, gw, rws, nullptr, h->part.p, S, round, mode, srank, sworld);
                }
                if (shard_on) {
                    const int q = (mode == 1) ? (round & 1) : (int)(seq_host & 1ull);
                    if (timing) HIPCHK(hipEventRecord(get_event(h, ev_used), st));
                    hipLaunchKernelGGL(k_merge_partials, dim3((gw + 255) / 256), dim3(256), 0, st, h->ctl.p, h->part.p,
                                       h->part_stride, S, h->gsend.p, h->gsend_stride, round, mode,
                                       (const unsigned long long*)h->pstat_p(), gw * 4,
                                       (const int*)nullptr);
                    h->comm.all_gather(h->gsend.p + (size_t)q * h->gsend_stride, h->gpart.p + (size_t)q * h->gpart_stride,
                                       ((size_t)gw * 4 + 4) * sizeof(Cand), st, st == h->stream2 ? 1 : 0);
                    if (h->prune_now && h->guess_now && h->group_guess_now && h->lean_now) ++h->stats.scan_lean_launches;
                    if (h->prune_now && h->guess_now && h->group_guess_now && !h->lean_now) {
                        launch_scan<false>(h, st, gw, rws, nullptr, h->part.p, S, round, mode, srank, sworld, 1);
                        Cand* const send2 = h->gsend2.p + (size_t)q * CC_MISSED_CAP * 4;
                        Cand* const recv2 = h->gpart2.p + (size_t)q * sworld * CC_MISSED_CAP * 4;
                        hipLaunchKernelGGL(k_merge_partials, dim3((CC_MISSED_CAP + 255) / 256), dim3(256), 0, st, h->ctl.p,
                                           h->part.p, h->part_stride, S, send2, (size_t)0, round, mode,
                                           (const unsigned long long*)nullptr, 0, (const int*)h->missed.p);
                        h->comm.all_gather(send2, recv2, (size_t)CC_MISSED_CAP * 4 * sizeof(Cand), st, st == h->stream2 ? 1 : 0);
                        hipLaunchKernelGGL(k_scatter_missed, dim3((CC_MISSED_CAP * sworld + 255) / 256), dim3(256), 0, st,
                                           (const Ctl*)h->ctl.p, (const int*)h->missed.p, (const Cand*)recv2, sworld,
                                           h->gpart.p, h->gpart_stride, (size_t)gw * 4 + 4, round, mode);
                    }
                    if (timing) {
                        HIPCHK(hipEventRecord(get_event(h, ev_used + 1), st));
                        timed_comm.push_back(ev_used);
                        ev_used += 2;
                    }
                }
            };
            const Cand* const dec_part = shard_on ? h->gpart.p : h->part.p;
            const size_t dec_stride = shard_on ? h->gpart_stride : h->part_stride;
            const int dec_S = shard_on ? world : S, dec_inner = shard_on ? 1 : S;
            const size_t dec_outer = shard_on ? (size_t)gw * 4 + 4 : 0;
            const int dec_tail = shard_on ? gw * 4 : -1;
            if (la_on) {
                if (evScan) HIPCHK(hipStreamWaitEvent(sA, evScan, 0));
                HIPCHK(hipStreamWaitEvent(sB, evCommit, 0));
                timed_scan(sB, 1, (int)((seq_host + 1ull) & 1ull));
                if (scan_end) evScan = scan_end;
                else {
                    evScan = get_sync_event(h, ev_sync++);
                    HIPCHK(hipEventRecord(evScan, sB));
                }
                if (wv == 0 && h->hc.mode == 0) timed_scan(sA, 0, 0);
            } else {
                timed_scan(sA, 0, 0);
            }
            const ScanCopy sc_now = scopy[seq_host & 1ull];
            const int ac_blocks = la_on ? rblocks : 0;
            hipLaunchKernelGGL(k_decide, dim3(dblocks + ac_blocks), dim3(decide_threads), 0, sA, h->ctl.p, h->X.p, tab, ver, car,
                               dec_part, dec_stride, h->clean.p, h->dpart.p, h->dpart2.p, h->dseed.p, (const int*)nullptr,
                               h->T0.p, h->dpath.p, dec_S, Sd, 0, 0, scan_rows, dec_inner, dec_outer,
                               (const CommitRec*)h->rec.p, sc_now, ac_blocks, long_list, long_cap, dec_tail, 0, heavy_on ? 1 : 0, 0,
                               link_now ? h->link_near.p : (int*)nullptr);
            if (link_now) {
                launch_link_scan(h, sA, gw);
                hipLaunchKernelGGL(k_link_apply, dim3((gw + 255) / 256), dim3(256), 0, sA, h->ctl.p, tab, h->T0.p,
                                   (const int*)h->link_near.p, h->dpath.p);
                ++h->stats.link_launches;
            }
            if (scan_rows > 0)
                hipLaunchKernelGGL(k_claims, dim3(scan_rows), dim3(256), 0, sA, h->ctl.p, tab, (const int*)h->T0.p, 0, scan_rows, 0);
            if (heavy_on && ++h->stats.heavy_launches > 0)
                hipLaunchKernelGGL(k_claims_heavy, dim3(CC_HEAVY_CAP), dim3(256), 0, sA, h->ctl.p, tab, (const int*)h->T0.p, 0,
                                   long_list, long_cap, 0);
            for (int r = 1; r <= Rcur; ++r) {
                const int* told = ((r - 1) & 1) ? h->T1.p : h->T0.p;
                int* tnew = (r & 1) ? h->T1.p : h->T0.p;
                const bool prep = h->allow_prep && ((long_rows > 0 && long_rows <= 64) || (long_listed && long_few));
                unsigned long long* const lstat = prep ? h->lstat.p : nullptr;
                unsigned long long* const lprev = prep ? h->lprev.p : nullptr;
                if (prep) h->prep_launched = true;
                if (prep && long_rows > 0)
                    hipLaunchKernelGGL((k_chain_long<true, true>), dim3(long_rows), dim3(CC_LONG_THREADS), 0, sA, h->ctl.p, h->X.p, tab,
                                       ver, car, told, r, long_rows, (const int*)nullptr, lstat, lprev);
                else if (prep)
                    hipLaunchKernelGGL((k_chain_long<true, true>), dim3(long_cap), dim3(CC_LONG_THREADS), 0, sA, h->ctl.p, h->X.p,
                                       tab, ver, car, told, r, 0, (const int*)long_list, lstat, lprev);
                hipLaunchKernelGGL(k_chain, dim3(cblocks), dim3(chain_threads), 0, sA,
                                   h->ctl.p, h->X.p, tab, ver, car, told, r, long_rows, (const unsigned long long*)lprev, lstat);
                if (long_rows > 0 && long_rows <= 256)
                    hipLaunchKernelGGL((k_chain_long<true, false>), dim3(long_rows), dim3(CC_LONG_THREADS), 0, sA, h->ctl.p, h->X.p, tab,
                                       ver, car, told, r, long_rows, (const int*)nullptr, lstat, lprev);
                else if (long_rows > 0)
                    hipLaunchKernelGGL((k_chain_long<false, false>), dim3(long_rows), dim3(256), 0, sA, h->ctl.p, h->X.p, tab, ver, car,
                                       told, r, long_rows, (const int*)nullptr, lstat, lprev);
                else if (long_listed && ++long_launches > 0) {
                    if (long_few)
                        hipLaunchKernelGGL((k_chain_long<true, false>), dim3(long_cap), dim3(CC_LONG_THREADS), 0, sA, h->ctl.p, h->X.p,
                                           tab, ver, car, told, r, 0, (const int*)long_list, lstat, lprev);
                    else
                        hipLaunchKernelGGL((k_chain_long<false, false>), dim3(long_cap), dim3(256), 0, sA, h->ctl.p, h->X.p, tab, ver,
                                           car, told, r, 0, (const int*)long_list, lstat, lprev);
                }
                const bool sparse_r = nodirty && sparse_now;
                hipLaunchKernelGGL(k_dseed, dim3((gw + 63) / 64), dim3(64), 0, sA, h->ctl.p, h->X.p, tab, ver, car,
                                   h->clean.p, h->dseed.p, told, r, (const int8_t*)h->dpath.p, h->sp_list.p,
                                   sparse_r ? sparse_cap : 0);
                if (!nodirty) {
                    launch_scan<true>(h, sA, gw, vrows, h->dseed.p, h->dpart.p, Sd, r, 0);
                    if (la_on) launch_scan<true>(h, sA, gw, crows, h->dseed.p, h->dpart2.p, Sd, r, 1);
                } else if (sparse_r) {
                    launch_scan<true>(h, sA, sparse_cap, vrows_sp, h->dseed.p, h->dpart.p, Sd, r, 0);
                    if (la_on) launch_scan<true>(h, sA, sparse_cap, crows_sp, h->dseed.p, h->dpart2.p, Sd, r, 1);
                }
                hipLaunchKernelGGL(k_decide, dim3(dblocks), dim3(decide_threads), 0, sA, h->ctl.p, h->X.p, tab, ver, car, dec_part,
                                   dec_stride, h->clean.p, h->dpart.p, h->dpart2.p, h->dseed.p, told, tnew, h->dpath.p, dec_S, Sd, r, nodirty ? (sparse_r ? 2 : 1) : 0, scan_rows,
                                   dec_inner, dec_outer, (const CommitRec*)nullptr, ScanCopy{}, 0, long_list, long_cap, -1,
                                   r == Rcur ? 1 : 0, heavy_on ? 1 : 0, h->allow_quiet ? 1 : 0, (int*)nullptr);
                if (scan_rows > 0 && r < Rcur)
                    hipLaunchKernelGGL(k_claims, dim3(scan_rows), dim3(256), 0, sA, h->ctl.p, tab, (const int*)tnew, r, scan_rows, h->allow_quiet ? 1 : 0);
                if (heavy_on && r < Rcur && ++h->stats.heavy_launches > 0)
                    hipLaunchKernelGGL(k_claims_heavy, dim3(CC_HEAVY_CAP), dim3(256), 0, sA, h->ctl.p, tab, (const int*)tnew, r,
                                       long_list, long_cap, h->allow_quiet ? 1 : 0);
            }
            hipLaunchKernelGGL(k_commit_a, dim3(1), dim3(1024), 0, sA, h->ctl.p, tab, ver, car, h->T0.p, h->T1.p,
                               h->rk.p, h->rec.p, (const Cand*)h->clean.p, (const int8_t*)h->dpath.p);
            hipLaunchKernelGGL(k_commit_b, dim3(rblocks), dim3(commit_threads), 0, sA, h->rec.p, tab, ver, car, h->rk.p, h->dpath.p,
                               h->lab_uid.p, h->lab_path.p, h->d, sc_now, h->hc.filter);
            if (la_on) {
                evCommit = get_sync_event(h, ev_sync++);
                HIPCHK(hipEventRecord(evCommit, sA));
            }
        }
    }

    int after_batch()
    {
// ... 17 lines not shown
            long_prev = h->hc.stat_long;
            rounds_prev = h->hc.stat_rounds;
        }
        {
            cc_policy_obs o{};
            o.cursor = h->hc.cursor;
            o.m_rows = h->hc.m_rows;
            o.stall_b = h->hc.stall_b;
            o.stat_windows = h->hc.stat_windows;
            o.stat_truncated = h->hc.stat_truncated;
            o.stat_trunc_unknown = h->hc.stat_trunc_unknown;
            o.stat_tiles = h->hc.stat_tiles;
            o.stat_dirty_tiles = h->hc.stat_dirty_tiles;
            o.stat_unsafe = h->hc.stat_unsafe;
            o.stat_missed = h->hc.stat_missed;
            o.tg_ok = (h->hc.tg_ok[0][0] != 0 && h->hc.tg_ok[1][0] != 0) ? 1 : 0;
            for (int r = 0; r < CC_MAX_ROUNDS + 2; ++r) o.round_hist[r] = h->hc.round_hist[r];
            o.prune_rows = h->hc.stat_prune_rows;
            o.prune_full = h->hc.stat_prune_full;
            dec = policy->after_batch(o);
            ptrace->batch(o, dec);
            const cc_policy_carry& k = policy->carry();
            h->adapt_win = k.adapt_win; h->clean_batches = k.clean_batches; h->since_shrink = k.since_shrink;
            if (dec.stalled)
                return fail(h, CC_ERR_INTERNAL, "the online phase made no progress in five consecutive batches of windows");
            if (h->trace && dec.prune_rows > 0)
                fprintf(stderr, "[cc] pruned scans of the batch%s (sample): %lld (wave, row) pairs, %.1f %% evaluated in full; points missed by guessed thresholds so far: %lld\n",
                        h->guess_now ? ", guessed thresholds" : "", (long long)dec.prune_rows,
                        100.0 * (double)dec.prune_full / (double)dec.prune_rows, (long long)h->hc.stat_missed);
            pair_rows_eff += (h->hc.stat_pair_rows - pair_rows_prev) / (shard_was ? (double)world : 1.0);
            if (h->prune_now) pair_rows_pruned += (h->hc.stat_pair_rows - pair_rows_prev) / (shard_was ? (double)world : 1.0);
            pair_rows_prev = h->hc.stat_pair_rows;
            if (shard_was) sharded_windows += dec.wins;
            Rcur = dec.rounds;
            Sd = Sd_full;
            nodirty = dec.nodirty != 0;
            sparse_now = dec.sparse != 0;
            shard_on = dec.shard != 0;
            h->set_prune(dec.prune);
            if (dec.restart) {
                h->hc.win_cfg = dec.win_cfg;
                h->hc.win_b = (int)std::min<long long>(dec.win_cfg, N - done);
                set_lookahead(dec.lookahead != 0);
                push_ctl_pinned(h);
            }
#ifdef CC_ROUND_DEBUG
            for (int r = 1; r <= CC_MAX_ROUNDS; ++r)
                if (h->hc.dbg_round[r][5] != 0)
                    fprintf(stderr, "[cc]    round %d so far: %llu decisions, %llu refused, create->join new %llu, create->join row %llu, join->create %llu, other MC %llu | windows ended in round %d: %lld\n",
                            r, h->hc.dbg_round[r][5], h->hc.dbg_round[r][0], h->hc.dbg_round[r][1], h->hc.dbg_round[r][2], h->hc.dbg_round[r][3],
                            h->hc.dbg_round[r][4], r, (long long)h->hc.round_hist[r]);
#endif
            if (h->trace)
                fprintf(stderr, "[cc] %.2f ms done %lld rows %d | batch: %lld windows %lld points trunc %lld (%lld at an undecidable point) lookahead %lld dirty tiles %lld / %lld (points so far: %lld unlocated, %lld unsafe) | next window %d rounds %d\n",
                        now_ms() - batch_t0, done, h->hc.m_rows, (long long)dec.wins, (long long)dec.pts, (long long)dec.trunc, (long long)dec.unk, (long long)h->hc.stat_lookahead, (long long)dec.dtiles, (long long)dec.tiles,
                        (long long)h->hc.stat_unprovable, (long long)h->hc.stat_unsafe, dec.want, Rcur);
            batch_windows = dec.batch_windows;
            {
                const bool bad = dec.bad != 0;
                bad_batches = bad ? bad_batches + 1 : 0;
                if (seq_mode == 0 && seq_possible() && done < N) {
                    if (seq_probe) {
                        if (bad && seq_rate_last > 0.0 && win_rate < seq_rate_last) {
                            seq_on = true;
                            seq_stint_len = std::min<long long>(seq_stint_len * 2, 1 << 20);
                        } else {
                            seq_stint_len = 32768;
                        }
                    } else if (bad_batches >= (seq_r_applies() ? 1 : 2) &&
                               win_rate < (seq_rate_last > 0.0 ? seq_rate_last : seq_rate_guess())) {
                        seq_on = true;
                    }
                    if (seq_on) seq_stint_left = seq_stint_len;
                }
                seq_probe = false;
                if (seq_mode == 2 && seq_possible() && done < N) seq_on = true;
            }
        }
        return (int)CC_OK;
    }

    void finish()
    {
        HIPCHK(hipEventRecord(ev1, h->stream));
        HIPCHK(hipEventSynchronize(ev1));
        float ms = 0.f;
        HIPCHK(hipEventElapsedTime(&ms, ev0, ev1));
        h->stats.run_ms += ms;
        h->stats.points += N - range_a;
        h->stats.windows += h->hc.stat_windows;
        h->stats.rounds += h->hc.stat_rounds;
        h->stats.truncated += h->hc.stat_truncated;
        h->stats.rows = h->hc.m_rows;
        h->stats.scan_pair_dims += pair_rows_eff * (double)h->d;
        h->stats.scan_pair_dims_pruned += pair_rows_pruned * (double)h->d;
        h->stats.sharded_windows += sharded_windows;
        h->stats.seq_points += h->hc.stat_seq_points;
        h->stats.seq_r_points += h->hc.stat_seq_r_points;
#ifdef CC_SEQG_TIMERS
        fprintf(stderr, "[cc] k_seq_g (shader cycles, thread 0): scan %llu minimum %llu add %llu barrier %llu rest %llu chunk %llu | points %llu\n",
                h->hc.dbg_long[0], h->hc.dbg_long[1], h->hc.dbg_long[2], h->hc.dbg_long[3], h->hc.dbg_long[4], h->hc.dbg_long[5], h->hc.dbg_long[7]);
#endif
#ifdef CC_LONG_TIMERS
        fprintf(stderr, "[cc] k_chain_long, workgroup 0 (shader cycles): collect %llu stage %llu chains %llu step-dim %llu step %llu rows %llu state %llu | batches %llu\n",
                h->hc.dbg_long[0], h->hc.dbg_long[1], h->hc.dbg_long[2], h->hc.dbg_long[3], h->hc.dbg_long[4], h->hc.dbg_long[5], h->hc.dbg_long[6], h->hc.dbg_long[7]);
#endif
        h->seq_sticky = seq_on;
        h->stats.table_rows_scanned += h->hc.stat_table_rows;
        h->stats.lookahead_windows += h->hc.stat_lookahead;
        h->stats.pruned_scan_rows += (int64_t)h->hc.stat_prune_rows;
        h->stats.pruned_scan_full_rows += (int64_t)h->hc.stat_prune_full;
        h->stats.long_chains += (int64_t)h->hc.stat_long;
        h->stats.long_chain_launches += long_launches;
        if (h->prep_launched) {
            h->prep_launched = false;
            unsigned long long lp[2] = {0ull, 0ull};
            HIPCHK(hipMemcpy(lp, h->lstat.p + 2 * CC_LSTAT_ROWS, sizeof(lp), hipMemcpyDeviceToHost));
            h->stats.long_prepared += (int64_t)lp[0];
            h->stats.long_replayed += (int64_t)lp[1];
        }
        h->stats.tiles += h->hc.stat_tiles;
        h->stats.dirty_tiles += h->hc.stat_dirty_tiles;
        h->stats.missed_points += h->hc.stat_missed;
        h->probe_now = false;
        if (timing) {
            double tot = 0.0, tot_p = 0.0;
            int64_t n_p = 0;
            for (auto& t : timed) {
                float e = 0.f;
                HIPCHK(hipEventElapsedTime(&e, h->ev_pool[t.first], h->ev_pool[t.first + 1]));
                tot += e;
                if (t.second != 0.0) { tot_p += e; ++n_p; }
            }
            h->stats.scan_launches += (int64_t)timed.size();
            h->stats.scan_ms += tot;
            h->stats.scan_launches_pruned += n_p;
            h->stats.scan_ms_pruned += tot_p;
            double ctot = 0.0;
            for (size_t i : timed_comm) {
                float e = 0.f;
                HIPCHK(hipEventElapsedTime(&e, h->ev_pool[i], h->ev_pool[i + 1]));
                ctot += e;
            }
            h->stats.comm_launches += (int64_t)timed_comm.size();
            h->stats.comm_ms += ctot;
        }
    }

    int run()
    {
        prepare();
        while (done < N) {
            ensure_table(h, (size_t)m_known + std::max<size_t>(window_rows(), seq_on ? 8192 : 0) + 1);
            const Table tab = h->tab.view();
            if (seq_on) {
                sequential_stint(tab);
                continue;
            }
            enqueue_batch(tab);
            const int rc = after_batch();
            if (rc != CC_OK) return rc;
        }
        finish();
        return (int)CC_OK;
    }
};

int online_range(cc_handle* h, long long range_a, long long range_e, bool no_create, bool resume)
{
    if (range_e <= range_a) return (int)CC_OK;
    if (h->d > CC_WINDOW_MAX_DIM && (h->comm.active() || no_create || !h->allow_seq_g))
        return fail(h, CC_ERR_BAD_ARG, "more than " + std::to_string(CC_WINDOW_MAX_DIM) + " dimensions: the online phase runs on the sequential "
                    "workgroup kernel (k_seq_g) only - not in a multi-GPU group, not with CHRONOCLUST_HIP_SEQG=0");
    if (h->d == 0) return fail(h, CC_ERR_BAD_ARG, "no points uploaded");
    OnlineRun run(h, range_a, range_e, no_create, resume);
    return run.run();
}

}
```

### chronoclust_amd/csrc/cc_scan.h

```cpp
#pragma once


#define CC_SCAN_TM 16
#ifndef CC_SCAN_PT_CLEAN
#define CC_SCAN_PT_CLEAN 1
#endif
#ifndef CC_SCAN_WGS_CLEAN
#define CC_SCAN_WGS_CLEAN 4
#endif
#ifndef CC_SCAN_WGS_CLEAN40
#define CC_SCAN_WGS_CLEAN40 3
#endif
#ifndef CC_SCAN_WGS_DIRTY32
#define CC_SCAN_WGS_DIRTY32 3
#endif
#ifndef CC_SCAN_NW_CLEAN
#define CC_SCAN_NW_CLEAN 4
#endif
template <int DP, bool DIRTY>
struct ScanShape {
    static constexpr int PT = (!DIRTY && DP == 20) ? CC_SCAN_PT_CLEAN : 1;
    static constexpr int NW = (!DIRTY && DP == 20) ? CC_SCAN_NW_CLEAN : 4;
    static constexpr int WGS = (!DIRTY && DP == 20) ? CC_SCAN_WGS_CLEAN
                               : (DP <= 20 ? 4 : (DP <= 40 ? (DIRTY ? CC_SCAN_WGS_DIRTY32 : (DP == 40 ? CC_SCAN_WGS_CLEAN40 : 3)) : 2));
// ... 365 lines not shown
            const bool liveB = RB2 ? row_bounds(m + 1, kindB, boundB) : false;
            if (!liveA && !liveB) continue;

            double accA[PT], accB[PT];
#pragma unroll
            for (int t = 0; t < PT; ++t) { accA[t] = 0.0; accB[t] = 0.0; }
            bool alive = true;
            const int mB = (m + 1 < CC_SCAN_TM) ? m + 1 : m;
#pragma unroll
            for (int i0 = 0; i0 < DP; i0 += 4) {
#pragma unroll
                for (int q = 0; q < 4; ++q) {
                    const int i = i0 + q;
                    if (i < DP) {
                        const double cA = s_c_base[m * DP + i], sA = s_s_base[m * DP + i];
                        const double cB = s_c_base[mB * DP + i], sB = s_s_base[mB * DP + i];
#pragma unroll
                        for (int t = 0; t < PT; ++t) {
                            double x = p[t][i] - cA;
                            x = x * x;
                            if (FUSE) accA[t] = __builtin_fma(x, sA, accA[t]);
                            else {
                                x = POW2 ? x * sA : x / sA;
                                accA[t] = accA[t] + x;
                            }
                            if (RB2) {
                                double y = p[t][i] - cB;
                                y = y * y;
                                if (FUSE) accB[t] = __builtin_fma(y, sB, accB[t]);
                                else {
                                    y = POW2 ? y * sB : y / sB;
                                    accB[t] = accB[t] + y;
                                }
                            }
                        }
                    }
                }
                if (i0 + 4 < DP) {
                    bool q = false;
#pragma unroll
                    for (int t = 0; t < PT; ++t) q = q || (accA[t] <= boundA[t]) || (RB2 && accB[t] <= boundB[t]);
                    if (__builtin_amdgcn_ballot_w64(q) == 0ull) {
                        alive = false;
                        break;
                    }
                }
            }
            if (!alive) continue;

            auto insert_row = [&](int mm, int kind, const double (&acc)[PT], const double (&bound)[PT]) {
                const int rowg = rt + mm;
                const int rowc = carried ? CC_CAR_BASE + rowg : rowg;
                const int key = s_key_w[mm];
#pragma unroll
                for (int t = 0; t < PT; ++t) {
                    if (!(acc[t] <= bound[t])) continue;
                    auto consider = [&](auto KC) {
                        constexpr int K = decltype(KC)::value;
                        constexpr int R = DIRTY ? 0 : 1;
                        if (!cand_less(acc[t], key, bd[K][t][R], bk[K][t][R])) return;
                        if (K == 0 && filter) {
                            int ne1 = 0;
                            cc_tentative_radius(rows.cf1 + (size_t)rowg * d, rows.cf2 + (size_t)rowg * d,
                                                rows.w[rowg], X + (cursor + jj[t]) * d, d, par, nullptr, &ne1);
                            if (ne1 > par.pi) return;
                        }
                        if (cand_less(acc[t], key, bd[K][t][0], bk[K][t][0])) {
                            bd[K][t][1] = bd[K][t][0]; bk[K][t][1] = bk[K][t][0]; bs[K][t][1] = bs[K][t][0];
                            bd[K][t][0] = acc[t]; bk[K][t][0] = key; bs[K][t][0] = rowc;
                        } else {
                            bd[K][t][1] = acc[t]; bk[K][t][1] = key; bs[K][t][1] = rowc;
                        }
                    };
                    if (kind == 0) consider(std::integral_constant<int, 0>{});
                    else consider(std::integral_constant<int, 1>{});
                }
            };
            if (liveA) insert_row(m, kindA, accA, boundA);
            if (RB2 && liveB) insert_row(m + 1, kindB, accB, boundB);
        }
        };
        if (POW2 && fuse_tile) dirty_rows(std::true_type{});
        else dirty_rows(std::false_type{});
    }

    if (!DIRTY) {
#pragma unroll
        for (int kd = 0; kd < 2; ++kd)
#pragma unroll
            for (int t = 0; t < PT; ++t)
#pragma unroll
                for (int r = 0; r < 2; ++r) bk[kd][t][r] = bs[kd][t][r] >= 0 ? rows.key[bs[kd][t][r]] : CC_IDX_INF;
    }
    Cand* const s_m = reinterpret_cast<Cand*>(smem);
    auto s_m_at = [&](int w, int t, int c) -> Cand& { return s_m[((w * PT + t) * 4 + c) * 64 + lane]; };
    __syncthreads();
    if (wv > 0) {
#pragma unroll
        for (int t = 0; t < PT; ++t) {
            s_m_at(wv - 1, t, 0) = Cand{bd[0][t][0], bk[0][t][0], bs[0][t][0]};
            s_m_at(wv - 1, t, 1) = Cand{bd[0][t][1], bk[0][t][1], bs[0][t][1]};
            s_m_at(wv - 1, t, 2) = Cand{bd[1][t][0], bk[1][t][0], bs[1][t][0]};
            s_m_at(wv - 1, t, 3) = Cand{bd[1][t][1], bk[1][t][1], bs[1][t][1]};
        }
    }
    __syncthreads();
    if (wv != 0) return;
#pragma unroll
    for (int t = 0; t < PT; ++t) {
        if (!valid[t]) continue;
        Cand c0{bd[0][t][0], bk[0][t][0], bs[0][t][0]}, c1{bd[0][t][1], bk[0][t][1], bs[0][t][1]};
        Cand c2{bd[1][t][0], bk[1][t][0], bs[1][t][0]}, c3{bd[1][t][1], bk[1][t][1], bs[1][t][1]};
#pragma unroll
        for (int w = 0; w < NW - 1; ++w) {
            cc_top2_push(c0, c1, s_m_at(w, t, 0));
            cc_top2_push(c0, c1, s_m_at(w, t, 1));
            cc_top2_push(c2, c3, s_m_at(w, t, 2));
            cc_top2_push(c2, c3, s_m_at(w, t, 3));
        }
        if (DIRTY) {
            Cand* o = part + ((size_t)jj[t] * S + blockIdx.y) * 2;
            o[0] = c0;
            o[1] = c2;
        } else {
            Cand* o = part + ((size_t)jj[t] * S + blockIdx.y) * 4;
            o[0] = c0; o[1] = c1; o[2] = c2; o[3] = c3;
        }
    }
    }
}

#ifndef CC_SCANU_WGS40
#define CC_SCANU_WGS40 4
#endif
template <int DP>
struct ScanUShape {
    static constexpr int WGS = DP <= 32 ? 4 : (DP <= 40 ? CC_SCANU_WGS40 : 2);
};
template <int BIT>
__device__ __forceinline__ void cc_sel_scale2(unsigned mask, double scaled, double one, double& o0, double& o1)
{
    asm("s_bitcmp1_b32 %2, %3\n\ts_cselect_b64 %0, %5, %6\n\ts_bitcmp1_b32 %2, %4\n\ts_cselect_b64 %1, %5, %6"
        : "=&s"(o0), "=&s"(o1)
        : "s"(mask), "n"(BIT), "n"(BIT + 1), "s"(scaled), "s"(one)
        : "scc");
}

__device__ __forceinline__ int cc_after(int row, double dep)
{
    asm("" : "+s"(row) : "v"(dep));
    return row;
}

template <int DP, int NW>
__global__ __launch_bounds__(64 * NW, ScanUShape<DP>::WGS) void k_scan_u(const Ctl* __restrict__ ctl, const double* __restrict__ Xt,
                                                                 const double* __restrict__ g_cen,
                                                                 const double* __restrict__ g_scl,
                                                                 const int* __restrict__ g_kind,
                                                                 const int* __restrict__ g_key, Cand* __restrict__ part,
                                                                 int round, int mode, size_t part_stride, int shard_rank,
                                                                 int shard_world, const int* __restrict__ plist = nullptr)
{
    static_assert(DP % 2 == 0 && DP >= 4 && DP <= 64, "padded dimensionalities are even");
    constexpr int NP = DP / 2;
    constexpr int NC = 2 * ((NP + 9) / 10);
    constexpr int CH_MAX = 2 * ((NP + NC - 1) / NC);
    int B, m_rows_scan, q;
    long long cursor;
    if (mode == 1) {
        q = round & 1;
        B = ctl->la_b[q];
        m_rows_scan = ctl->la_rows[q];
        cursor = ctl->la_cursor[q];
    } else {
        B = ctl->win_b;
        m_rows_scan = ctl->m_rows;
        cursor = ctl->cursor;
        if (ctl->mode != 0) return;
        q = (int)(ctl->window_seq & 1ull);
    }
    part += (size_t)q * part_stride;
    if (B == 0) return;
    if (plist) plist += (size_t)q * CC_MISSED_CAP;
    const int n_here = plist ? ctl->n_missed[q] : B;
    const int j0 = (int)blockIdx.x * 64;
    if (j0 >= n_here) return;
    const int lane = threadIdx.x & 63;
    const int wv = __builtin_amdgcn_readfirstlane(threadIdx.x >> 6);
    const int S = gridDim.y;
    const int nsub = S * NW;
    const int sub = blockIdx.y * NW + wv;
    int row_lo = 0, row_hi = m_rows_scan;
    if (shard_world > 1) cc_shard_range(m_rows_scan, shard_world, shard_rank, 1, &row_lo, &row_hi);
    const int nrows = row_hi - row_lo;
    const int per = (nrows + nsub - 1) / nsub;
    const int r0 = row_lo + sub * per;
    const int r1 = min(row_hi, r0 + per);
    const size_t n_pts = (size_t)ctl->xt_stride;
    const double k = ctl->k;
    const double inv_k = ctl->inv_k;
    const bool valid = j0 + lane < n_here;
    const int jj = plist ? (valid ? plist[j0 + lane] : 0) : j0 + lane;

    double p[DP];
    {
        const double* xp = Xt + cursor + (valid ? jj : 0);
#pragma unroll
        for (int i = 0; i < DP; ++i) p[i] = valid ? xp[(size_t)i * n_pts] : 0.0;
    }
    bool fuse_wave = k >= 0x1p-64 && k <= 0x1p64;
    {
        bool tn = false;
#pragma unroll
        for (int i = 0; i < DP; ++i) tn = tn || cc_is_tiny(p[i]);
        fuse_wave = fuse_wave && __builtin_amdgcn_ballot_w64(tn) == 0ull;
    }
    double bd[2][2];
    int bs[2][2];
#pragma unroll
    for (int kd = 0; kd < 2; ++kd)
#pragma unroll
        for (int r = 0; r < 2; ++r) {
            bd[kd][r] = valid ? CC_INF : -CC_INF;
            bs[kd][r] = -1;
        }

    for (int rt = r0; rt < r1; rt += CC_SCAN_TM) {
        const int tm = __builtin_amdgcn_readfirstlane(min(CC_SCAN_TM, r1 - rt));
        double buf[2][CH_MAX];
        {
            const double* __restrict__ c0 = g_cen + (size_t)rt * DP;
#pragma unroll
            for (int i = 0; i < 2 * (NP / NC); ++i) buf[0][i] = c0[i];
        }
        constexpr int NL = (CC_SCAN_TM * DP + 63) / 64;
        int rm_lo = 0, rm_hi = 0;
        bool fuse_tile;
        {
            const double* gc = g_cen + (size_t)rt * DP;
            const double* gs = g_scl + (size_t)rt * DP;
            unsigned long long rmask = 0ull;
            bool tn = false;
            const int off = (lane & (CC_SCAN_TM - 1)) * DP;
#pragma unroll
            for (int q = 0; q < NL; ++q) {
                const int e = lane + q * 64;
                const bool in = e < tm * DP;
                const double tc = in ? gc[e] : 0.0;
                const double ts = in ? gs[e] : 1.0;
                tn = tn || cc_is_tiny(tc);
                const unsigned long long w = __builtin_amdgcn_ballot_w64(ts != 1.0);
                const int rel = off - 64 * q;
                const unsigned long long a = (rel >= 0 && rel < 64) ? (w >> (rel & 63)) : 0ull;
                const unsigned long long b = (rel < 0 && rel > -DP) ? (w << ((-rel) & 63)) : 0ull;
                rmask |= a | b;
            }
            if (DP < 64) rmask &= (1ull << (DP & 63)) - 1ull;
            rm_lo = (int)(unsigned)(rmask & 0xFFFFFFFFull);
            rm_hi = (int)(unsigned)(rmask >> 32);
            fuse_tile = fuse_wave && __builtin_amdgcn_ballot_w64(tn) == 0ull;
        }
        unsigned pmask, omask;
        {
            const int kd = (lane < tm) ? g_kind[rt + lane] : CC_KIND_DEAD;
            pmask = (unsigned)__builtin_amdgcn_ballot_w64(kd == CC_KIND_PCORE);
            omask = (unsigned)__builtin_amdgcn_ballot_w64(kd == CC_KIND_OUTLIER);
        }
        auto rows_of_tile = [&](auto FUSEC, auto KSELC) {
            constexpr bool FUSE = decltype(FUSEC)::value;
            constexpr int KSEL = decltype(KSELC)::value;
            for (int m = 0; m < tm; ++m) {
                const unsigned mlo = (unsigned)__builtin_amdgcn_readlane(rm_lo, m);
                const unsigned mhi = (DP > 32) ? (unsigned)__builtin_amdgcn_readlane(rm_hi, m) : 0u;
                const int rowg = rt + m;
                const int rown = min(rowg + 1, rt + tm - 1);
                const double one = 1.0;
                double acc = 0.0;
                auto pair_step = [&](auto IC, double c0, double c1, double x0) {
                    constexpr int i = decltype(IC)::value;
                    double s0, s1;
                    cc_sel_scale2<(i & 31)>(i < 32 ? mlo : mhi, inv_k, one, s0, s1);
                    double x = x0;
                    double y = p[i + 1] - c1;
                    x = x * x;
                    y = y * y;
                    if (FUSE) {
                        acc = (i == 0) ? x * s0 : __builtin_fma(x, s0, acc);
                        acc = __builtin_fma(y, s1, acc);
                    } else {
                        x = x * s0;
                        y = y * s1;
                        acc = (i == 0) ? x : acc + x;
                        acc = acc + y;
                    }
                };
                cc_static_for<NC>([&](auto CC) {
                    constexpr int c = decltype(CC)::value;
                    constexpr int lo = 2 * (c * NP / NC), hi = 2 * ((c + 1) * NP / NC);
                    constexpr int cn = (c + 1) % NC;
                    constexpr int nlo = 2 * (cn * NP / NC), nhi = 2 * ((cn + 1) * NP / NC);
                    const double x0 = p[lo] - buf[c & 1][0];
                    const double* __restrict__ nx = g_cen + (size_t)cc_after(c + 1 < NC ? rowg : rown, x0) * DP;
#pragma unroll
                    for (int i = 0; i < nhi - nlo; ++i) buf[cn & 1][i] = nx[nlo + i];
                    cc_static_for<(hi - lo) / 2>([&](auto QC) {
                        constexpr int i = 2 * decltype(QC)::value;
                        pair_step(std::integral_constant<int, lo + i>{}, buf[c & 1][i], buf[c & 1][i + 1],
                                  (i == 0) ? x0 : p[lo + i] - buf[c & 1][i]);
                    });
                });
                auto update = [&](auto KC) {
                    constexpr int K = decltype(KC)::value;
                    const double a = acc;
                    double& d0 = bd[K][0];
                    double& d1 = bd[K][1];
                    int& s0 = bs[K][0];
                    int& s1 = bs[K][1];
                    bool ins = a < d1;
                    bool first = a < d0;
                    const unsigned long long e1 = __builtin_amdgcn_ballot_w64(a == d1);
                    const unsigned long long e0 = __builtin_amdgcn_ballot_w64(a == d0);
                    if ((e1 | e0) != 0ull) {
                        if (a == d1 || a == d0) {
                            const int key = g_key[rowg];
                            if (a == d1) ins = key < (s1 >= 0 ? g_key[s1] : CC_IDX_INF);
                            if (a == d0) first = key < (s0 >= 0 ? g_key[s0] : CC_IDX_INF);
                        }
                    }
                    d1 = cc_vmin(d1, cc_vmax(d0, a));
                    d0 = cc_vmin(d0, a);
                    s1 = first ? s0 : (ins ? rowg : s1);
                    s0 = first ? rowg : s0;
                };
                if constexpr (KSEL == 0) update(std::integral_constant<int, 0>{});
                else if constexpr (KSEL == 1) update(std::integral_constant<int, 1>{});
                else {
                    if ((pmask >> m) & 1u) update(std::integral_constant<int, 0>{});
                    else if ((omask >> m) & 1u) update(std::integral_constant<int, 1>{});
                }
            }
        };
        const unsigned full = (1u << tm) - 1u;
        if (fuse_tile) {
            if (pmask == full) rows_of_tile(std::true_type{}, std::integral_constant<int, 0>{});
            else if (omask == full) rows_of_tile(std::true_type{}, std::integral_constant<int, 1>{});
            else rows_of_tile(std::true_type{}, std::integral_constant<int, -1>{});
        } else rows_of_tile(std::false_type{}, std::integral_constant<int, -1>{});
    }

    int bk[2][2];
#pragma unroll
    for (int kd = 0; kd < 2; ++kd)
#pragma unroll
        for (int r = 0; r < 2; ++r) bk[kd][r] = bs[kd][r] >= 0 ? g_key[bs[kd][r]] : CC_IDX_INF;
    __shared__ Cand s_m[(NW > 1 ? NW - 1 : 1) * 4 * 64];
    auto s_m_at = [&](int w, int c) -> Cand& { return s_m[(w * 4 + c) * 64 + lane]; };
    if (wv > 0) {
        s_m_at(wv - 1, 0) = Cand{bd[0][0], bk[0][0], bs[0][0]};
        s_m_at(wv - 1, 1) = Cand{bd[0][1], bk[0][1], bs[0][1]};
        s_m_at(wv - 1, 2) = Cand{bd[1][0], bk[1][0], bs[1][0]};
        s_m_at(wv - 1, 3) = Cand{bd[1][1], bk[1][1], bs[1][1]};
    }
    __syncthreads();
    if (wv != 0 || !valid) return;
    Cand c0{bd[0][0], bk[0][0], bs[0][0]}, c1{bd[0][1], bk[0][1], bs[0][1]};
    Cand c2{bd[1][0], bk[1][0], bs[1][0]}, c3{bd[1][1], bk[1][1], bs[1][1]};
#pragma unroll
    for (int w = 0; w < NW - 1; ++w) {
        cc_top2_push(c0, c1, s_m_at(w, 0));
        cc_top2_push(c0, c1, s_m_at(w, 1));
        cc_top2_push(c2, c3, s_m_at(w, 2));
        cc_top2_push(c2, c3, s_m_at(w, 3));
    }
    Cand* o = part + ((size_t)jj * S + blockIdx.y) * 4;
    o[0] = c0; o[1] = c1; o[2] = c2; o[3] = c3;
}


struct __attribute__((aligned(8))) SeedCand {
    float part;
    int row;
};

struct ScanWin {
    int B, rows, q;
    long long cursor;
};
__device__ __forceinline__ ScanWin cc_scan_window(const Ctl* __restrict__ ctl, int round, int mode)
{
    ScanWin w;
    if (mode == 1) {
        w.q = round & 1;
        w.B = ctl->la_b[w.q];
        w.rows = ctl->la_rows[w.q];
        w.cursor = ctl->la_cursor[w.q];
    } else {
        w.B = (ctl->mode != 0) ? 0 : ctl->win_b;
        w.rows = ctl->m_rows;
        w.cursor = ctl->cursor;
        w.q = (int)(ctl->window_seq & 1ull);
    }
    return w;
}

typedef float cc_f2 __attribute__((ext_vector_type(2)));
typedef float cc_f4 __attribute__((ext_vector_type(4)));
#define CC_PRE 8

template <int DP>
__device__ __forceinline__ void cc_load_prefix(const double* __restrict__ g_cen, const int* __restrict__ g_kind, int rt,
                                               int tm, int lane, double (&tc)[2], int& kd)
{
#pragma unroll
    for (int q = 0; q < 2; ++q) {
        const int e = lane + q * 64, m = e >> 3, i = e & 7;
        tc[q] = (m < tm) ? g_cen[(size_t)(rt + m) * DP + i] : 0.0;
    }
    kd = (lane < tm) ? g_kind[rt + lane] : CC_KIND_DEAD;
}

__device__ __forceinline__ float cc_prefix_score(const cc_f2 (&p2)[CC_PRE / 2], const cc_f4* __restrict__ row)
{
    const cc_f4 c01 = row[0], c23 = row[1];
    cc_f2 x0 = p2[0] - cc_f2{c01.x, c01.y};
    cc_f2 x1 = p2[1] - cc_f2{c01.z, c01.w};
    cc_f2 x2 = p2[2] - cc_f2{c23.x, c23.y};
    cc_f2 x3 = p2[3] - cc_f2{c23.z, c23.w};
    cc_f2 acc = x0 * x0;
    acc = __builtin_elementwise_fma(x1, x1, acc);
    acc = __builtin_elementwise_fma(x2, x2, acc);
    acc = __builtin_elementwise_fma(x3, x3, acc);
    return acc.x + acc.y;
}

template <int DP, int NW>
__global__ __launch_bounds__(64 * NW, 4) void k_seed(const Ctl* __restrict__ ctl, const double* __restrict__ Xt,
                                                   const double* __restrict__ g_cen, const int* __restrict__ g_kind,
                                                   SeedCand* __restrict__ spart, int round, int mode, size_t spart_stride,
                                                   unsigned long long* __restrict__ cmax, const int* __restrict__ plist)
{
    static_assert(CC_PRE == 8 && CC_PRE <= DP, "prefix dimensions");
    const ScanWin win = cc_scan_window(ctl, round, mode);
    const int B = win.B;
    if (B == 0) return;
    const int j0 = (int)blockIdx.x * 128;
    if (plist) plist += (size_t)win.q * CC_MISSED_CAP;
    const int n_pts_here = plist ? ctl->n_missed[win.q] : B;
    if (j0 >= n_pts_here) return;
    spart += (size_t)win.q * spart_stride;
    const int lane = threadIdx.x & 63;
    const int wv = __builtin_amdgcn_readfirstlane(threadIdx.x >> 6);
    const int S = gridDim.y;
    const int nsub = S * NW;
    const int sub = blockIdx.y * NW + wv;
    const int per = (win.rows + nsub - 1) / nsub;
    const int r0 = sub * per;
    const int r1 = min(win.rows, r0 + per);
    const size_t n_pts = (size_t)ctl->xt_stride;
    double org[CC_PRE];
#pragma unroll
    for (int i = 0; i < CC_PRE; ++i) org[i] = g_cen[i];
    int jj[2];
    bool valid[2];
    cc_f2 p2[2][CC_PRE / 2];
#pragma unroll
    for (int u = 0; u < 2; ++u) {
        const int e = j0 + u * 64 + lane;
        valid[u] = e < n_pts_here;
        jj[u] = plist ? (valid[u] ? plist[e] : 0) : e;
        const double* xp = Xt + win.cursor + (valid[u] ? jj[u] : 0);
#pragma unroll
        for (int i = 0; i < CC_PRE / 2; ++i)
            p2[u][i] = cc_f2{valid[u] ? (float)(xp[(size_t)(2 * i) * n_pts] - org[2 * i]) : 0.f,
                             valid[u] ? (float)(xp[(size_t)(2 * i + 1) * n_pts] - org[2 * i + 1]) : 0.f};
    }
    __shared__ __attribute__((aligned(16))) float s_pre[NW * CC_SCAN_TM * CC_PRE];
    __shared__ float s_h[NW * CC_SCAN_TM];
    float* const tile = s_pre + (size_t)wv * CC_SCAN_TM * CC_PRE;
    float* const th = s_h + (size_t)wv * CC_SCAN_TM;
    float best[2][2];
    int idx[2][2];
#pragma unroll
    for (int u = 0; u < 2; ++u)
#pragma unroll
        for (int K = 0; K < 2; ++K) { best[u][K] = -__builtin_inff(); idx[u][K] = -1; }
    double tc[2];
    int kdl = CC_KIND_DEAD;
    double cm = 0.0;
    if (r0 < r1) cc_load_prefix<DP>(g_cen, g_kind, r0, min(CC_SCAN_TM, r1 - r0), lane, tc, kdl);
    for (int rt = r0; rt < r1; rt += CC_SCAN_TM) {
        const int tm = __builtin_amdgcn_readfirstlane(min(CC_SCAN_TM, r1 - rt));
        CC_WAVE_SYNC();
#pragma unroll
        for (int q = 0; q < 2; ++q) {
            cm = __builtin_fmax(cm, __builtin_fabs(tc[q]));
            const float v = (float)(tc[q] - org[lane & 7]);
            tile[lane + q * 64] = v;
            float hsum = v * v;
// ... 1172 lines not shown
```

### chronoclust_amd/csrc/cc_validate.h

```cpp
#pragma once


#define CC_LSTAT_ROWS 1024

__device__ __forceinline__ unsigned cc_group_ballot(bool p)
{
    const unsigned long long b = __builtin_amdgcn_ballot_w64(p);
    return (unsigned)(b >> (threadIdx.x & 32));
}

template <int CTRL>
__device__ __forceinline__ double cc_dpp_f64(double x)
{
    int lo = __double2loint(x), hi = __double2hiint(x);
    lo = __builtin_amdgcn_update_dpp(0, lo, CTRL, 0xF, 0xF, false);
    hi = __builtin_amdgcn_update_dpp(0, hi, CTRL, 0xF, 0xF, false);
    return __hiloint2double(hi, lo);
}
__device__ __forceinline__ double cc_group_sum_any_order(double x)
{
    x += cc_dpp_f64<0xB1>(x);
    x += cc_dpp_f64<0x4E>(x);
    x += cc_dpp_f64<0x141>(x);
    x += cc_dpp_f64<0x140>(x);
// ... 250 lines not shown
        if (look[kd * 2 + 1] && lv[kd * 2 + 1] == -2) lk_ok[kd] = false;
    }
    bool sd[4];
    int kvq[4], keyq[4];
    const double* vcen[4];
    const double* vpref[4];
#pragma unroll
    for (int q = 0; q < 4; ++q) {
        sd[q] = look[q] && lv[q] >= 0;
        const bool cr = sd[q] && lv[q] >= CC_CAR_BASE;
        const size_t r = sd[q] ? (size_t)(cr ? lv[q] - CC_CAR_BASE : lv[q]) : 0;
        kvq[q] = sd[q] ? (cr ? car.kind[r] : ver.kind[r]) : CC_KIND_DEAD;
        keyq[q] = sd[q] ? (cr ? car.key[r] : ver.key[r]) : 0;
        vcen[q] = (cr ? car.cen : ver.cen) + r * d;
        vpref[q] = (cr ? car.pref : ver.pref) + r * d;
    }
#pragma unroll
    for (int q = 0; q < 4; ++q) sd[q] = sd[q] && kvq[q] != CC_KIND_DEAD;
    double accq[4] = {0.0, 0.0, 0.0, 0.0};
    for (int i0 = 0; i0 < d; i0 += 4) {
        double pv[4], cv[4][4], fv[4][4];
#pragma unroll
        for (int c = 0; c < 4; ++c) {
            const int i = (i0 + c < d) ? i0 + c : d - 1;
            pv[c] = p[i];
#pragma unroll
            for (int q = 0; q < 4; ++q) {
                cv[q][c] = sd[q] ? vcen[q][i] : 0.0;
                fv[q][c] = sd[q] ? vpref[q][i] : 1.0;
            }
        }
#pragma unroll
        for (int c = 0; c < 4; ++c) {
            if (i0 + c < d) {
#pragma unroll
                for (int q = 0; q < 4; ++q) {
                    double x = pv[c] - cv[q][c];
                    x = x * x;
                    accq[q] = accq[q] + cc_div_pref(x, fv[q][c], par);
                }
            }
        }
    }
#pragma unroll
    for (int q = 0; q < 4; ++q) {
        if (!sd[q]) continue;
        if (kvq[q] == 0 && filter) {
            const bool cr = lv[q] >= CC_CAR_BASE;
            const size_t r = (size_t)(cr ? lv[q] - CC_CAR_BASE : lv[q]);
            int ne1 = 0;
            cc_tentative_radius((cr ? car.cf1 : ver.cf1) + r * d, (cr ? car.cf2 : ver.cf2) + r * d,
                                cr ? car.w[r] : ver.w[r], p, d, par, nullptr, &ne1);
            if (ne1 > par.pi) continue;
        }
        if (kvq[q] == 0) {
            if (cand_less(accq[q], keyq[q], first0.dist, first0.key)) first0 = Cand{accq[q], keyq[q], lv[q]};
        } else {
            if (cand_less(accq[q], keyq[q], first1.dist, first1.key)) first1 = Cand{accq[q], keyq[q], lv[q]};
        }
    }
    seed[(size_t)j * 4 + 0] = first0;
    seed[(size_t)j * 4 + 1] = Cand{cap[0], 0, 0};
    seed[(size_t)j * 4 + 2] = first1;
    seed[(size_t)j * 4 + 3] = Cand{cap[1], 0, 0};

    double tau[3];
    for (int kd = 0; kd < 3; ++kd) {
        double t;
        const int list = (kd == 1) ? 1 : 0;
        const int from = (kd == 0) ? 0 : 1;
        if (list == 0 && filter) t = -CC_INF;
        else if (kd != 2 && !have1[kd]) t = CC_INF;
        else {
            const double fb = (list == 0) ? first0.dist : first1.dist;
            const double ce = fb < cap[list] ? fb : cap[list];
            t = (d2v[from] == CC_INF) ? CC_INF : (sqrt(d2v[from]) - sqrt(K * ce));
        }
        if (!lk_ok[list] || lbound[list] || (kd == 2 && !lk_ok[1])) t = -CC_INF;
        t = (t == CC_INF) ? CC_INF : t * (1.0 - 1e-9) - 1e-290;
        tau[kd] = t;
    }
    const bool need0 = true;
    const bool need1 = !(T[j] >= 0 && dpath[j] == 0);
    int flags = 0;
    if (!(cc_dsq_below(maxd[0], tau[0]) && cc_dsq_below(maxd[2], tau[2]))) flags |= CC_FLAG_U0;
    if (!cc_dsq_below(maxd[1], tau[1])) flags |= CC_FLAG_U1;
    if (la_mode && !(cc_dsq_below(maxd_car[0], tau[0]) && cc_dsq_below(maxd_car[2], tau[2]))) flags |= CC_FLAG_C0;
    if (la_mode && !cc_dsq_below(maxd_car[1], tau[1])) flags |= CC_FLAG_C1;
    need_ver = (need0 && (flags & CC_FLAG_U0)) || (need1 && (flags & CC_FLAG_U1));
    need_car = (need0 && (flags & CC_FLAG_C0)) || (need1 && (flags & CC_FLAG_C1));
    flag_unprov = !(lk_ok[0] && lk_ok[1]);
    flag_unsafe = need_ver || need_car;
    flag_n1skip = !need1;
    flag_word = flags;
#pragma unroll
    for (int kd = 0; kd < 3; ++kd) tau_w[kd] = tau[kd];
    {
        const int t = T[j];
        const Cand c1 = cq[0], c2 = cq[1];
        if (flags == 0 && t >= 0 && dpath[j] == 0 && c1.slot >= 0 && ver.tgt[j] == t && ver.acc[j] != 0) {
            const int head0 = 0xFFFFF - (int)(tcq[0] & 0xFFFFFull);
            const bool dirty0 = ((tcq[0] >> 20) == stamp && head0 < j) || (la_mode && (coq[0] >> 20) == wseq);
            if (!dirty0) {
                repeats = c1.slot == t && !(first0.slot >= 0 && cand_less(first0.dist, first0.key, c1.dist, c1.key));
            } else if (first0.slot >= 0 && (c2.slot == -1 || cand_less(first0.dist, first0.key, c2.dist, c2.key))) {
                if (first0.slot >= CC_CAR_BASE) repeats = car.slot[first0.slot - CC_CAR_BASE] == t;
                else repeats = ver.tgt[first0.slot] == t && ver.next[first0.slot] == j;
            }
        }
    }
    }
    if (sparse_cap > 0) {
        const unsigned long long m = __builtin_amdgcn_ballot_w64(flag_unsafe);
        if (m != 0ull) {
            int base = 0;
            if (threadIdx.x == (unsigned)__builtin_ctzll(m)) base = atomicAdd(&ctl->n_sparse, __builtin_popcountll(m));
            base = __shfl(base, __builtin_ctzll(m));
            const int idx = base + __builtin_popcountll(m & ((1ull << threadIdx.x) - 1ull));
            if (flag_unsafe && idx < sparse_cap) {
                sparse_list[idx] = j;
                flag_word |= CC_FLAG_SPARSE;
                flag_n1skip = false;
            }
        }
    }
    const unsigned long long any_v = __builtin_amdgcn_ballot_w64(need_ver), any_c = __builtin_amdgcn_ballot_w64(need_car);
    if (j < B) {
        if (flag_n1skip && any_v == 0ull && any_c == 0ull) { tau_w[1] = CC_INF; flag_word |= CC_FLAG_N1SKIP; }
#pragma unroll
        for (int kd = 0; kd < 3; ++kd) ver.tau[(size_t)j * CC_TAU_STRIDE + kd] = tau_w[kd];
        ver.unsafe[j] = flag_word;
    }
    if (__builtin_amdgcn_ballot_w64(j < B && !(repeats && any_v == 0ull && any_c == 0ull)) != 0ull && threadIdx.x == 0)
        ctl->rdiff[round] = 1;
    {
        const unsigned long long b1 = __builtin_amdgcn_ballot_w64(flag_unprov), b2 = __builtin_amdgcn_ballot_w64(flag_unsafe);
        if (threadIdx.x == 0 && b1) atomicAdd((unsigned long long*)&ctl->stat_unprovable, (unsigned long long)__builtin_popcountll(b1));
        if (threadIdx.x == 0 && b2) atomicAdd((unsigned long long*)&ctl->stat_unsafe, (unsigned long long)__builtin_popcountll(b2));
    }
    if (threadIdx.x == 0) {
        ver.skip[blockIdx.x] = any_v == 0ull ? 1 : 0;
        ver.skip_car[blockIdx.x] = (!la_mode || any_c == 0ull) ? 1 : 0;
    }
}

struct ScanCopy {
    double* cen;
    double* scl;
    double* cf1;
    double* cf2;
    double* w;
    int* kind;
    int* key;
};

struct CommitRec {
    int n;
    int M0;
    int pk0, ok0;
    long long pid0, oid0;
    const int* T;
    long long cursor;
    int carry;
    unsigned long long next_seq;
};

__device__ __forceinline__ void cc_apply_carry(const CommitRec* __restrict__ rec, const Carry& car, const ScanCopy& sc, int d,
                                               int filter, int part, int parts)
{
    if (rec->carry == 0) return;
    const int n = rec->n;
    const int gl = threadIdx.x & 31;
    const int groups = (parts * (int)blockDim.x) >> 5;
    for (int j = (part * (int)blockDim.x + (int)threadIdx.x) >> 5; j < n; j += groups) {
        const int kind = car.kind[j];
        if (kind == CC_KIND_DEAD) continue;
        const size_t row = (size_t)car.slot[j];
#pragma unroll
        for (int h = 0; h < 2; ++h) {
            const int i = gl + 32 * h;
            if (i >= d) continue;
            const size_t e = row * d + i, v = (size_t)j * d + i;
            sc.cen[e] = car.cen[v];
            sc.scl[e] = car.scl[v];
            if (filter) { sc.cf1[e] = car.cf1[v]; sc.cf2[e] = car.cf2[v]; }
        }
        if (gl == 0) {
            sc.kind[row] = kind;
            sc.key[row] = car.key[j];
            if (filter) sc.w[row] = car.w[j];
        }
    }
}


__global__ __launch_bounds__(256) void k_decide(Ctl* __restrict__ ctl, const double* __restrict__ X, Table tab,
                                                Versions ver, Carry car, const Cand* __restrict__ part,
                                                size_t part_stride, Cand* __restrict__ clean,
                                                const Cand* __restrict__ dpart, const Cand* __restrict__ dpart2,
                                                const Cand* __restrict__ dseed,
                                                const int* __restrict__ Told, int* __restrict__ Tnew,
                                                int8_t* __restrict__ dpath, int S, int Sd, int round, int nodirty,
                                                int scan_rows, int part_inner, size_t part_outer,
                                                const CommitRec* __restrict__ ac_rec, ScanCopy ac_sc, int ac_blocks,
                                                int* __restrict__ long_list, int long_cap, int stat_tail, int last_round,
                                                int heavy_on, int quiet_ok, int* __restrict__ link_near)
{
    CC_LATENCY_KERNEL();
    if (ac_blocks > 0 && (int)blockIdx.x >= (int)gridDim.x - ac_blocks) {
        cc_apply_carry(ac_rec, car, ac_sc, ctl->d, ctl->filter, (int)blockIdx.x - ((int)gridDim.x - ac_blocks), ac_blocks);
        return;
    }
    const int B = ctl->win_b;
    if (B == 0) return;
    if (round == 0 && blockIdx.x == 0 && threadIdx.x == 0) {
        const int q = (int)(ctl->window_seq & 1ull);
        unsigned long long rows = 0ull, full = 0ull;
        if (stat_tail >= 0) {
            const Cand* g = part + (size_t)q * part_stride + (size_t)stat_tail;
            for (int r = 0; r < S; ++r) {
                rows += (unsigned long long)(unsigned)g[(size_t)r * part_outer].key;
                full += (unsigned long long)(unsigned)g[(size_t)r * part_outer].slot;
            }
        } else {
            rows = ctl->pstat[q][0];
            full = ctl->pstat[q][1];
        }
        ctl->pstat[q][0] = 0ull;
        ctl->pstat[q][1] = 0ull;
        ctl->stat_prune_rows += rows;
        ctl->stat_prune_full += full;
        if (ctl->n_missed_all[q] != 0) atomicAdd((unsigned long long*)&ctl->stat_missed, (unsigned long long)ctl->n_missed_all[q]);
        ctl->n_missed_all[q] = 0;
    }
    if (round > 0 && ctl->fc[round - 1] >= B) return;
    if (round > 0 && quiet_ok != 0 && ctl->rdiff[round] == 0) return;
    const int gl = threadIdx.x & 31;
    const int j = blockIdx.x * (blockDim.x >> 5) + (threadIdx.x >> 5);
    if (j >= B) return;
    const Par par = cc_load_par(ctl);
    const int d = par.d;
    const Cand none = Cand{CC_INF, CC_IDX_INF, -1};

    Cand p1 = none, p2 = none, o1 = none, o2 = none;
    const unsigned long long wseq = ctl->window_seq;
    const bool la_mode = ctl->mode != 0;
    if (round == 0) {
        part += (size_t)(wseq & 1ull) * part_stride;
        for (int s = gl & 15; s < S; s += 16) {
            const Cand* q = part + (size_t)(s / part_inner) * part_outer + ((size_t)j * part_inner + (s % part_inner)) * 4;
            cc_top2_push(p1, p2, q[0]);
            cc_top2_push(p1, p2, q[1]);
            cc_top2_push(o1, o2, q[2]);
            cc_top2_push(o1, o2, q[3]);
        }
        cc_row16_exchanges([&](auto CT) {
            constexpr int C = decltype(CT)::value;
            const Cand a0 = cc_dpp_cand<C>(p1), a1 = cc_dpp_cand<C>(p2);
            const Cand a2 = cc_dpp_cand<C>(o1), a3 = cc_dpp_cand<C>(o2);
            cc_top2_push(p1, p2, a0);
            cc_top2_push(p1, p2, a1);
            cc_top2_push(o1, o2, a2);
            cc_top2_push(o1, o2, a3);
        });
        if (gl == 0) {
            Cand* out = clean + (size_t)j * 4;
            out[0] = p1; out[1] = p2; out[2] = o1; out[3] = o2;
        }
    } else {
        const Cand* in = clean + (size_t)j * 4;
        p1 = in[0]; p2 = in[1]; o1 = in[2]; o2 = in[3];
    }
    Cand dvp = none, dvo = none;
    const int flags = (round > 0) ? ver.unsafe[j] : 0;
    const bool on_list = nodirty == 2 && (flags & CC_FLAG_SPARSE) != 0;
    const bool ran = round > 0 && ((nodirty == 0 && ver.skip[j >> 6] == 0) || on_list);
    const bool ran_car = round > 0 && la_mode && ((nodirty == 0 && ver.skip_car[j >> 6] == 0) || on_list);
    if (round > 0) {
        Cand dummy = none;
        if (!ran && !ran_car) {
            dvp = dseed[(size_t)j * 4 + 0];
            dvo = dseed[(size_t)j * 4 + 2];
        } else {
        if ((gl & 15) == 0 && !(ran && (ran_car || !la_mode))) {
            dvp = dseed[(size_t)j * 4 + 0];
            dvo = dseed[(size_t)j * 4 + 2];
        }
        for (int s = gl & 15; s < Sd; s += 16) {
            if (ran) {
                const Cand* q = dpart + ((size_t)j * Sd + s) * 2;
                cc_top2_push(dvp, dummy, q[0]);
                cc_top2_push(dvo, dummy, q[1]);
            }
            if (ran_car) {
                const Cand* q2 = dpart2 + ((size_t)j * Sd + s) * 2;
                cc_top2_push(dvp, dummy, q2[0]);
                cc_top2_push(dvo, dummy, q2[1]);
            }
        }
        cc_row16_exchanges([&](auto CT) {
            constexpr int C = decltype(CT)::value;
            const Cand b0 = cc_dpp_cand<C>(dvp), b1 = cc_dpp_cand<C>(dvo);
            cc_top2_push(dvp, dummy, b0);
            cc_top2_push(dvo, dummy, b1);
        });
        }
    }

    const unsigned long long stamp = ctl->window_seq * 16ull + (unsigned long long)round;
    auto dirty = [&](int slot) -> bool {
        if (round == 0) return false;
        const unsigned long long t = tab.touch[(size_t)(round & 1) * tab.cap + slot];
        if ((t >> 20) == stamp && (0xFFFFF - (int)(t & 0xFFFFFull)) < j) return true;
        return la_mode && (tab.carry_of[slot] >> 20) == wseq;
    };

    const int M0 = ctl->m_rows;
    const double* p = X + (ctl->cursor + j) * d;
    int T = -1;
    int path = 2;
    auto run_stage = [&](const Cand& c1, const Cand& c2, const Cand& dd, int stage) {
        int state;
        Cand cb = none;
        if (c1.slot == -1) state = 0;
        else if (c1.slot == CC_SLOT_BOUND) {
            if (gl == 0 && round == 0) atomicAdd((unsigned long long*)&ctl->stat_missed, 1ull);
            T = CC_T_UNKNOWN;
            return;
        }
        else if (!dirty(c1.slot)) { state = 1; cb = c1; }
        else if (c2.slot == -1) state = 0;
        else if (c2.slot == CC_SLOT_BOUND) { state = 2; cb = c2; }
        else if (!dirty(c2.slot)) { state = 1; cb = c2; }
        else { state = 2; cb = c2; }

        int wkind = 0;
        int wrow = -1;
        if (state == 0) {
            if (dd.slot >= 0) { wkind = 2; wrow = dd.slot; }
        } else if (state == 1) {
            if (dd.slot >= 0 && cand_less(dd.dist, dd.key, cb.dist, cb.key)) { wkind = 2; wrow = dd.slot; }
            else { wkind = 1; wrow = cb.slot; }
        } else {
// ... 1118 lines not shown
    const int per = (B + 1023) >> 10;
    unsigned mine = 0u;
    for (int q = 0; q < per; ++q) {
        const int j = tid * per + q;
        const unsigned f = (j < B) ? (unsigned)sflag[j] : 0u;
        mine += (f & 1u) | ((f & 2u) << 15);
    }
    unsigned v = mine;
    const int lane = tid & 63, wid = tid >> 6;
    for (int off = 1; off < 64; off <<= 1) {
        const unsigned o = __shfl_up(v, off);
        if (lane >= off) v += o;
    }
    if (lane == 63) wsum[wid] = v;
    __syncthreads();
    if (tid == 0) {
        unsigned run = 0u;
        for (int i = 0; i < 16; ++i) { const unsigned x = wsum[i]; wsum[i] = run; run += x; }
        tot = run;
    }
    __syncthreads();
    unsigned run = v - mine + wsum[wid];
    for (int q = 0; q < per; ++q) {
        const int j = tid * per + q;
        if (j < B) {
            rk[j] = (int)run;
            const unsigned f = (unsigned)sflag[j];
            run += (f & 1u) | ((f & 2u) << 15);
        }
    }
    }
    __syncthreads();
    const int tot_new = (int)(tot & 0xFFFFu), tot_up = (int)(tot >> 16);
    const unsigned long long seq = ctl->window_seq;
    const long long next_cursor = cursor + n;
    const long long left = n_points - next_cursor;
    const int next_b = (int)(left < (long long)win_cfg ? left : (long long)win_cfg);
    const int qn = (int)((seq + 1ull) & 1ull);
    const bool la_ok = ctl->la_on != 0 && n == B && next_b > 0 && ctl->la_b[qn] == next_b &&
                       ctl->la_cursor[qn] == next_cursor;
    if (la_ok)
        for (int i = tid; i < CC_DSQ_STRIDE * ((B + 15) / 16 + 1); i += 1024) car.tile_dsq[i] = 0ull;
    __shared__ double s_sum[2][16];
    __shared__ int s_cnt[2][16];
    {
        double sm[2] = {0.0, 0.0};
        int cn[2] = {0, 0};
        for (int j = tid * 8; j < n; j += 8192) {
            const int pth = dpath[j];
            if (T[j] >= 0 && (pth == 0 || pth == 1)) {
                const double dist = clean[(size_t)j * 4 + pth * 2].dist;
                if (dist < CC_INF) { sm[pth] += dist; cn[pth] += 1; }
            }
        }
#pragma unroll
        for (int K = 0; K < 2; ++K) {
            for (int off = 32; off >= 1; off >>= 1) {
                sm[K] += __shfl_xor(sm[K], off);
                cn[K] += __shfl_xor(cn[K], off);
            }
            if ((tid & 63) == 0) { s_sum[K][tid >> 6] = sm[K]; s_cnt[K][tid >> 6] = cn[K]; }
        }
    }
    __syncthreads();
    if (tid == 0) {
        const int slot = (int)(seq & 1ull);
        for (int K = 0; K < 2; ++K) {
            double sm = 0.0;
            int cn = 0;
            for (int i = 0; i < 16; ++i) { sm += s_sum[K][i]; cn += s_cnt[K][i]; }
            if (cn > 0) { ctl->tg[slot][K] = sm / (double)cn; ctl->tg_ok[slot][K] = 1; }
            else { ctl->tg[slot][K] = ctl->tg[slot ^ 1][K]; ctl->tg_ok[slot][K] = ctl->tg_ok[slot ^ 1][K]; }
        }
        rec->n = n; rec->M0 = M0; rec->pk0 = pk0; rec->ok0 = ok0; rec->pid0 = pid0; rec->oid0 = oid0; rec->T = T;
        rec->carry = la_ok ? 1 : 0;
        rec->cursor = cursor;
        rec->next_seq = seq + 1ull;
        ctl->mode = la_ok ? 1 : 0;
        ctl->car_n = la_ok ? B : 0;
        ctl->stat_lookahead += la_ok ? 1 : 0;
        const int q2 = (int)(seq & 1ull);
        const long long c2 = next_cursor + next_b;
        const long long left2 = n_points - c2;
        ctl->la_cursor[q2] = c2;
        ctl->la_b[q2] = (ctl->la_on != 0 && left2 > 0) ? (int)(left2 < (long long)win_cfg ? left2 : (long long)win_cfg) : 0;
        ctl->la_rows[q2] = M0 + tot_new;
        ctl->m_rows = M0 + tot_new;
        ctl->n_okeys = ok0 + tot_new;
        ctl->outlier_last_id = oid0 + tot_new;
        ctl->n_pkeys = pk0 + tot_up;
        ctl->pcore_last_id = pid0 + tot_up;
        ctl->cursor = cursor + n;
        ctl->stat_windows += 1;
        ctl->stat_rounds += r;
        ctl->round_hist[r] += 1;
        ctl->stat_truncated += (n < B) ? 1 : 0;
        ctl->stat_tiles += n_tiles;
        ctl->stat_dirty_tiles += dirty_tiles;
        ctl->stat_trunc_unknown += (n < B && T[n] == CC_T_UNKNOWN) ? 1 : 0;
        ctl->seed_at = (n < B && T[n] == CC_T_UNKNOWN) ? cursor + n : -1ll;
        ctl->stat_table_rows += M0;
        ctl->stat_pair_rows += (double)B * (double)M0;
        ctl->window_seq = seq + 1ull;
        if ((ctl->la_on != 0 && !la_ok && next_b > 0) || n == 0) {
            ctl->stall_b = next_b;
            ctl->win_b = 0;
            ctl->la_b[0] = 0;
            ctl->la_b[1] = 0;
        } else {
            ctl->win_b = next_b;
        }
        ctl->last_round = 0;
        ctl->fc[0] = 0;
        for (int i = 1; i < CC_MAX_ROUNDS + 2; ++i) ctl->fc[i] = CC_IDX_INF;
        for (int i = 0; i < CC_MAX_ROUNDS + 2; ++i) { ctl->any_new[i] = 0; ctl->any_up[i] = 0; ctl->n_long[i] = 0; }
    }
}

__global__ __launch_bounds__(256) void k_commit_b(const CommitRec* __restrict__ rec, Table tab, Versions ver,
                                                  Carry car, const int* __restrict__ rk,
                                                  const int8_t* __restrict__ dpath, long long* __restrict__ lab_uid,
                                                  int8_t* __restrict__ lab_path, int d, ScanCopy sc, int filter)
{
    CC_LATENCY_KERNEL();
    const int n = rec->n;
    if (n == 0) return;
    const int M0 = rec->M0;
    const int* T = rec->T;
    const bool carry = rec->carry != 0;
    const int gl = threadIdx.x & 31;
    const int groups = (gridDim.x * blockDim.x) >> 5;
    for (int j = (blockIdx.x * blockDim.x + threadIdx.x) >> 5; j < n; j += groups) {
        if (gl == 0) {
            const int tj = T[j];
            lab_uid[rec->cursor + j] = (tj < 0) ? -1ll : ((tj < M0) ? tab.uid[tj] : rec->oid0 + (rk[tj - M0] & 0xFFFF));
            lab_path[rec->cursor + j] = (int8_t)(dpath[j] | ((ver.upg[j] == j) ? 4 : 0));
        }
        if (ver.next[j] < n) {
            if (carry && gl == 0) { car.kind[j] = CC_KIND_DEAD; car.slot[j] = 0; }
            continue;
        }
        const int t = T[j];
        const int c = t - M0;
        const size_t row = (t < M0) ? (size_t)t : (size_t)(M0 + (rk[c] & 0xFFFF));
        const int u = ver.upg[j];
        const int kind = ver.kind[j];
        int key;
        if (u >= 0) key = rec->pk0 + (int)((unsigned)rk[u] >> 16);
        else if (t >= M0) key = rec->ok0 + (rk[c] & 0xFFFF);
        else key = tab.key[row];
        const int kind0 = (t < M0) ? tab.kind[row] : CC_KIND_DEAD;
        double dq = 0.0;
        bool metric_moved = false;
#pragma unroll
        for (int h = 0; h < 2; ++h) {
            const int i = gl + 32 * h;
            if (i >= d) continue;
            const size_t e = row * d + i, v = (size_t)j * d + i;
            const double ncen = ver.cen[v], npref = ver.pref[v], nscl = ver.scl[v], n1 = ver.cf1[v], n2 = ver.cf2[v];
            if (carry) {
                const double oc = (t < M0) ? tab.cen[e] : 0.0;
                const double ow = (t < M0) ? 1.0 / tab.pref[e] : 0.0;
                metric_moved = metric_moved || (t < M0 && npref != tab.pref[e]);
                car.c0[v] = oc; car.w0[v] = ow;
                car.cf1[v] = n1; car.cf2[v] = n2; car.cen[v] = ncen; car.pref[v] = npref; car.scl[v] = nscl;
                const double df = ncen - oc;
                dq += df * df * ow;
            }
            tab.cf1[e] = n1; tab.cf2[e] = n2; tab.cen[e] = ncen; tab.pref[e] = npref; tab.scl[e] = nscl;
            if (sc.cen) {
                sc.cen[e] = ncen; sc.scl[e] = nscl;
                if (filter) { sc.cf1[e] = n1; sc.cf2[e] = n2; }
            }
        }
        if (carry) {
            for (int off = 16; off >= 1; off >>= 1) dq += __shfl_xor(dq, off, 32);
            const bool promoted = kind == CC_KIND_PCORE && kind0 == CC_KIND_OUTLIER;
            if (kind0 == CC_KIND_DEAD || (kind != kind0 && !promoted) || !(dq >= 0.0) || cc_group_ballot(metric_moved) != 0u) dq = CC_INF;
        }
        if (gl == 0) {
            tab.w[row] = ver.w[j];
            tab.kind[row] = kind;
            if (u >= 0) {
                tab.key[row] = key;
                tab.id[row] = rec->pid0 + (long long)((unsigned)rk[u] >> 16);
            } else if (t >= M0) {
                tab.key[row] = key;
                tab.id[row] = rec->oid0 + (rk[c] & 0xFFFF);
            }
            if (t >= M0) tab.uid[row] = rec->oid0 + (rk[c] & 0xFFFF);
            if (sc.cen) {
                sc.kind[row] = kind;
                sc.key[row] = key;
                if (filter) sc.w[row] = ver.w[j];
            }
            if (carry) {
                car.w[j] = ver.w[j];
                car.kind[j] = kind;
                car.key[j] = key;
                car.slot[j] = (int)row;
                car.kind0[j] = kind0;
                int cls;
                car.dsq[j] = cc_dsq_store(dq, kind, kind0, &cls);
                atomicMax(&car.tile_dsq[(size_t)(j >> 4) * CC_DSQ_STRIDE + cls], cc_dsq_code(dq));
                tab.carry_of[row] = (rec->next_seq << 20) | (unsigned long long)j;
            }
        }
    }
}
```

Measured before the change: 75.06 million points/s.

## Precompute per-row scan records so the scan kernel skips per-tile recomputation

Adds a per-row record (a bitmask of scaled dimensions plus tiny/kind flags) that is maintained by the commit and copy kernels and built once by a new k_rowbits kernel. The scan_u kernel now reads one 64-bit mask and one flag word per row instead of reloading the row's centres, scales and kind to rebuild those masks on every tile visit. This cuts global loads in the hot scan, at the cost of extra writes in commit paths, extra device-to-device copies for the scan snapshots, and a verification mode behind an environment knob.

```diff
diff --git a/chronoclust_amd/csrc/cc_api.hip b/chronoclust_amd/csrc/cc_api.hip
--- a/chronoclust_amd/csrc/cc_api.hip
+++ b/chronoclust_amd/csrc/cc_api.hip
@@ -35,7 +35,7 @@
 {
     constexpr int NW = ScanShape<DP, false>::NW;
     static int blocks = 0;
-    static const bool ok = hipOccupancyMaxActiveBlocksPerMultiprocessor(&blocks, k_scan_u<DP, NW>, 64 * NW, 0) == hipSuccess && blocks >= 1;
+    static const bool ok = hipOccupancyMaxActiveBlocksPerMultiprocessor(&blocks, k_scan_u<DP, NW, true>, 64 * NW, 0) == hipSuccess && blocks >= 1;
     return ok ? blocks : ScanUShape<DP>::WGS;
 }
 
@@ -83,8 +83,19 @@
 
     void scan_u(int n_pts, int srank, int sworld, const int* plist) const
     {
-        hipLaunchKernelGGL((k_scan_u<DP, NW>), dim3((n_pts + 63) / 64, S), dim3(64 * NW), 0, st, h->ctl.p, h->Xt.p, rows.cen,
-                           rows.scl, rows.kind, rows.key, part, round, mode, h->part_stride, srank, sworld, plist);
+        const dim3 grid((n_pts + 63) / 64, S), block(64 * NW);
+        if (h->rowbits == 0 || !rows.rbm) {
+            if (h->rowbits != 0) throw HipErr{hipErrorInvalidValue, "k_scan_u: the rows carry no scan record"};
+            hipLaunchKernelGGL((k_scan_u<DP, NW, false>), grid, block, 0, st, h->ctl.p, h->Xt.p, rows.cen, rows.scl, rows.kind, rows.key,
+                               part, round, mode, h->part_stride, srank, sworld, plist, rows.rbm, rows.rbf);
+            return;
+        }
+        if (h->rowbits == 2)
+            hipLaunchKernelGGL((k_rowbits<true>), dim3(128), dim3(256), 0, st, (const Ctl*)h->ctl.p, rows.cen, rows.scl, rows.kind,
+                               const_cast<unsigned long long*>(rows.rbm), const_cast<unsigned*>(rows.rbf), 0, h->d, round, mode,
+                               h->badflag.p + 1);
+        hipLaunchKernelGGL((k_scan_u<DP, NW, true>), grid, block, 0, st, h->ctl.p, h->Xt.p, rows.cen, rows.scl, rows.kind, rows.key,
+                           part, round, mode, h->part_stride, srank, sworld, plist, rows.rbm, rows.rbf);
     }
     void prefix16() const
     {
diff --git a/chronoclust_amd/csrc/cc_api_comm.inc b/chronoclust_amd/csrc/cc_api_comm.inc
--- a/chronoclust_amd/csrc/cc_api_comm.inc
+++ b/chronoclust_amd/csrc/cc_api_comm.inc
@@ -245,11 +245,14 @@
         DevBuf<Ctl> cctl;
         DevBuf<double> cxt, ccen, cscl;
         DevBuf<int> ckind, ckey;
+        DevBuf<unsigned long long> crbm;
+        DevBuf<unsigned> crbf;
         DevBuf<Cand> cpart;
         const int tiles = (win + 63) / 64;
         const int Sc = std::max(1, std::min(16, (h->n_cus * scan_u_wgs_per_cu<DPc>()) / std::max(1, tiles)));
         cctl.ensure(1); cxt.ensure((size_t)win * DPc); ccen.ensure((size_t)Rc * DPc); cscl.ensure((size_t)Rc * DPc);
         ckind.ensure(Rc); ckey.ensure(Rc); cpart.ensure((size_t)2 * win * Sc * 4);
+        crbm.ensure(Rc + CC_RB_PAD); crbf.ensure(Rc + CC_RB_PAD);
         {
             std::vector<double> x((size_t)win * DPc), cen((size_t)Rc * DPc), scl((size_t)Rc * DPc, 0.25);
             unsigned long long st = 0x9E3779B97F4A7C15ull;
@@ -268,12 +271,17 @@
             HIPCHK(hipMemcpyAsync(cscl.p, scl.data(), scl.size() * 8, hipMemcpyHostToDevice, h->stream));
             HIPCHK(hipMemcpyAsync(ckind.p, kind.data(), (size_t)Rc * 4, hipMemcpyHostToDevice, h->stream));
             HIPCHK(hipMemcpyAsync(ckey.p, key.data(), (size_t)Rc * 4, hipMemcpyHostToDevice, h->stream));
+            hipLaunchKernelGGL((k_rowbits<false>), dim3((Rc + 7) / 8), dim3(256), 0, h->stream, (const Ctl*)cctl.p, (const double*)ccen.p,
+                               (const double*)cscl.p, (const int*)ckind.p, crbm.p, crbf.p, Rc, DPc, 0, 0, (int*)nullptr);
             sync_stream(h, h->stream);
         }
         const double scan_us = timed3([&]() {
-            hipLaunchKernelGGL((k_scan_u<DPc, NWc>), dim3(tiles, Sc), dim3(64 * NWc), 0, h->stream, (const Ctl*)cctl.p, (const double*)cxt.p,
-                               (const double*)ccen.p, (const double*)cscl.p, (const int*)ckind.p, (const int*)ckey.p, cpart.p, 0, 0,
-                               (size_t)win * Sc * 4, 0, 1);
+            with_bools([&](auto REC) {
+                hipLaunchKernelGGL((k_scan_u<DPc, NWc, decltype(REC)::value>), dim3(tiles, Sc), dim3(64 * NWc), 0, h->stream, (const Ctl*)cctl.p,
+                                   (const double*)cxt.p, (const double*)ccen.p, (const double*)cscl.p, (const int*)ckind.p,
+                                   (const int*)ckey.p, cpart.p, 0, 0, (size_t)win * Sc * 4, 0, 1, (const int*)nullptr,
+                                   (const unsigned long long*)crbm.p, (const unsigned*)crbf.p);
+            }, h->rowbits != 0);
         });
         HIPCHK(hipGetLastError());
         (void)hipEventDestroy(e0);
diff --git a/chronoclust_amd/csrc/cc_common.h b/chronoclust_amd/csrc/cc_common.h
--- a/chronoclust_amd/csrc/cc_common.h
+++ b/chronoclust_amd/csrc/cc_common.h
@@ -39,7 +39,13 @@
     int* clen;
     int* heavy;
     size_t cap;
-};
+    unsigned long long* rbm;
+    unsigned* rbf;
+};
+#define CC_RB_TINY 1u
+#define CC_RB_NOT_PCORE 2u
+#define CC_RB_NOT_OUTLIER 4u
+#define CC_RB_PAD 16
 #define CC_HEAVY_CAP 64
 #define CC_HEAVY_NEW 32
 
@@ -108,6 +114,8 @@
     const int* slot;
     const unsigned long long* touch;
     size_t cap;
+    const unsigned long long* rbm;
+    const unsigned* rbf;
 };
 
 struct Ctl {
diff --git a/chronoclust_amd/csrc/cc_handle.h b/chronoclust_amd/csrc/cc_handle.h
--- a/chronoclust_amd/csrc/cc_handle.h
+++ b/chronoclust_amd/csrc/cc_handle.h
@@ -58,9 +58,11 @@
     DevBuf<long long> id, uid;
     DevBuf<unsigned long long> touch, last, carry_of, cnt;
     DevBuf<int> memb, clen, heavy;
+    DevBuf<unsigned long long> rbm;
+    DevBuf<unsigned> rbf;
     size_t cap = 0;
     int d = 0;
-    enum Grow { KEPT, CLEARED, CLEARED_KEPT, SCRATCH };
+    enum Grow { KEPT, CLEARED, CLEARED_KEPT, SCRATCH, SCAN_RECORD };
     template <typename F>
     static void for_each_column(int dims, F&& f)
     {
@@ -74,14 +76,17 @@
         f(&TableStore::cnt, (size_t)1, CLEARED); f(&TableStore::memb, (size_t)CC_CHAIN_MEMB, SCRATCH);
         f(&TableStore::clen, (size_t)1, CLEARED);
         f(&TableStore::heavy, (size_t)1, CLEARED_KEPT);
+        f(&TableStore::rbm, (size_t)1, SCAN_RECORD); f(&TableStore::rbf, (size_t)1, SCAN_RECORD);
     }
     void alloc(size_t rows, int dim)
     {
-        for_each_column(dim, [&](auto col, size_t per_row, Grow) { (this->*col).ensure(rows * per_row); });
+        for_each_column(dim, [&](auto col, size_t per_row, Grow grow) {
+            (this->*col).ensure((rows + (grow == SCAN_RECORD ? (size_t)CC_RB_PAD : 0)) * per_row);
+        });
         cap = rows;
         d = dim;
     }
-    Table view() const { return Table{cf1.p, cf2.p, cen.p, pref.p, scl.p, w.p, kind.p, key.p, id.p, uid.p, touch.p, last.p, carry_of.p, cnt.p, memb.p, clen.p, heavy.p, cap}; }
+    Table view() const { return Table{cf1.p, cf2.p, cen.p, pref.p, scl.p, w.p, kind.p, key.p, id.p, uid.p, touch.p, last.p, carry_of.p, cnt.p, memb.p, clen.p, heavy.p, cap, rbm.p, rbf.p}; }
 };
 
 struct HostClusters {
@@ -189,6 +194,8 @@
     DevBuf<CommitRec> rec;
     DevBuf<double> sh_cen[2], sh_scl[2], sh_cf1[2], sh_cf2[2], sh_w[2];
     DevBuf<int> sh_kind[2], sh_key[2];
+    DevBuf<unsigned long long> sh_rbm[2];
+    DevBuf<unsigned> sh_rbf[2];
     DevBuf<int8_t> dpath;
 };
 
@@ -242,6 +249,7 @@
     DevBuf<Ctl> ctl;
     unsigned long long* pstat_p() const { return (unsigned long long*)((char*)ctl.p + offsetof(Ctl, pstat)); }
     bool tainted = false;
+    bool rowrec_ok = false;
     int adapt_win = 0;
     int clean_batches = 0;
     int since_shrink = 1000;
@@ -425,6 +433,7 @@
     });
     sync_stream(h, h->stream);
     std::swap(h->tab, nt);
+    h->rowrec_ok = false;
 }
 
 int set_dim(cc_handle* h, int d)
@@ -477,7 +486,7 @@
                  h->c_slot.p, h->c_c0.p, h->c_w0.p, h->c_kind0.p, h->c_dsq.p, h->c_tile_dsq.p};
 }
 
-void scan_copy_sync(cc_handle* h, ScanCopy (&out)[2])
+void scan_copy_sync(cc_handle* h, ScanCopy (&out)[2], bool rowrec)
 {
     const size_t cap = h->tab.cap, d = (size_t)h->d, m = (size_t)h->hc.m_rows;
     const bool filter = h->hc.filter != 0;
@@ -485,7 +494,12 @@
     for (int q = 0; q < 2; ++q) {
         h->sh_cen[q].ensure(cap * d); h->sh_scl[q].ensure(cap * d); h->sh_kind[q].ensure(cap); h->sh_key[q].ensure(cap);
         if (filter) { h->sh_cf1[q].ensure(cap * d); h->sh_cf2[q].ensure(cap * d); h->sh_w[q].ensure(cap); }
+        if (rowrec) { h->sh_rbm[q].ensure(cap + CC_RB_PAD); h->sh_rbf[q].ensure(cap + CC_RB_PAD); }
         if (m > 0) {
+            if (rowrec) {
+                HIPCHK(hipMemcpyAsync(h->sh_rbm[q].p, t.rbm.p, m * 8, hipMemcpyDeviceToDevice, h->stream));
+                HIPCHK(hipMemcpyAsync(h->sh_rbf[q].p, t.rbf.p, m * 4, hipMemcpyDeviceToDevice, h->stream));
+            }
             HIPCHK(hipMemcpyAsync(h->sh_cen[q].p, t.cen.p, m * d * 8, hipMemcpyDeviceToDevice, h->stream));
             HIPCHK(hipMemcpyAsync(h->sh_scl[q].p, t.scl.p, m * d * 8, hipMemcpyDeviceToDevice, h->stream));
             HIPCHK(hipMemcpyAsync(h->sh_kind[q].p, t.kind.p, m * 4, hipMemcpyDeviceToDevice, h->stream));
@@ -497,7 +511,7 @@
             }
         }
         out[q] = ScanCopy{h->sh_cen[q].p, h->sh_scl[q].p, h->sh_cf1[q].p, h->sh_cf2[q].p, h->sh_w[q].p, h->sh_kind[q].p,
-                          h->sh_key[q].p};
+                          h->sh_key[q].p, rowrec ? h->sh_rbm[q].p : nullptr, rowrec ? h->sh_rbf[q].p : nullptr};
     }
 }
 
diff --git a/chronoclust_amd/csrc/cc_knobs.h b/chronoclust_amd/csrc/cc_knobs.h
--- a/chronoclust_amd/csrc/cc_knobs.h
+++ b/chronoclust_amd/csrc/cc_knobs.h
@@ -33,6 +33,7 @@
     bool allow_heavy = true;
     bool allow_seq_r = true;
     bool allow_seq_g = true;
+    int rowbits = 1;
     int allow_sparse = 128;
 };
 
@@ -73,6 +74,7 @@
     knob_threads(k.commit_threads, "CHRONOCLUST_HIP_COMMIT_THREADS");
     knob_int_in(k.prune_mode, "CHRONOCLUST_HIP_PRUNE", 0, 2);
     knob_int_in(k.prune_rounds4, "CHRONOCLUST_HIP_PRUNE_WGS", 1, 64);
+    knob_int_in(k.rowbits, "CHRONOCLUST_HIP_ROWBITS", 0, 2);
     knob_int_in(k.allow_sparse, "CHRONOCLUST_HIP_SPARSE", 0, INT_MAX);
     knob_int_in(k.force_prune_rows, "CHRONOCLUST_HIP_FORCE_PRUNE_ROWS", INT_MIN, INT_MAX);
     knob_int_in(k.p3_listed_rows, "CHRONOCLUST_HIP_P3_LISTED", INT_MIN, INT_MAX);
diff --git a/chronoclust_amd/csrc/cc_online.h b/chronoclust_amd/csrc/cc_online.h
--- a/chronoclust_amd/csrc/cc_online.h
+++ b/chronoclust_amd/csrc/cc_online.h
@@ -101,6 +101,10 @@
 
 #define CC_TINY 0x1p-400
 __device__ __forceinline__ bool cc_is_tiny(double v) { return v != 0.0 && __builtin_fabs(v) < CC_TINY; }
+__device__ __forceinline__ unsigned cc_rb_flags(bool tiny, int kind)
+{
+    return (tiny ? CC_RB_TINY : 0u) | (kind != CC_KIND_PCORE ? CC_RB_NOT_PCORE : 0u) | (kind != CC_KIND_OUTLIER ? CC_RB_NOT_OUTLIER : 0u);
+}
 
 __device__ __forceinline__ unsigned long long cc_dsq_code(double dq) { return (unsigned long long)__double_as_longlong(dq) + 1ull; }
 __device__ __forceinline__ bool cc_dsq_below(unsigned long long code, double tau)
diff --git a/chronoclust_amd/csrc/cc_online_run.h b/chronoclust_amd/csrc/cc_online_run.h
--- a/chronoclust_amd/csrc/cc_online_run.h
+++ b/chronoclust_amd/csrc/cc_online_run.h
@@ -107,6 +107,7 @@
     bool la_on = false;
     bool shard_on = false;
     bool link_now = false;
+    bool rec_on = false;
     int Rcur = 1;
     int batch_windows = 2;
 
@@ -173,6 +174,9 @@
         refresh_ctl_params(h);
         h->scan_plan = scan_plan(h);
         const ScanPlan& plan = h->scan_plan;
+        rec_on = plan.scan_u && h->rowbits != 0;
+        h->rowrec_ok = false;
+        if (h->rowbits == 2) HIPCHK(hipMemsetAsync(h->badflag.p + 1, 0, sizeof(int), h->stream));
         win = h->tun.window; R = h->tun.rounds;
         S_cfg = std::max(1, h->tun.segments / plan.waves);
         Sd_full = std::max(1, (h->tun.dirty_segments > 0 ? h->tun.dirty_segments : h->tun.segments) / plan.dirty_waves);
@@ -296,8 +300,19 @@
         link_now = h->allow_link && !no_create && !wide();
     }
 
+    void ensure_rowrec(const Table& tab)
+    {
+        if (!rec_on || h->rowrec_ok) return;
+        if (h->hc.m_rows > 0)
+            hipLaunchKernelGGL((k_rowbits<false>), dim3((h->hc.m_rows + 7) / 8), dim3(256), 0, h->stream, (const Ctl*)h->ctl.p,
+                               (const double*)tab.cen, (const double*)tab.scl, (const int*)tab.kind, tab.rbm, tab.rbf, h->hc.m_rows,
+                               h->d, 0, 0, (int*)nullptr);
+        h->rowrec_ok = true;
+    }
+
     void sequential_stint(const Table& tab)
     {
+        h->rowrec_ok = false;
         const int chunk = 8192;
         const double t0 = now_ms();
         const bool use_g = seq_g_applies();
@@ -365,7 +380,7 @@
     {
         batch_t0 = now_ms();
         const Rows trows{tab.cen, tab.scl, tab.pref, tab.cf1, tab.cf2, tab.w, tab.kind, tab.key, nullptr, nullptr, nullptr,
-                         nullptr, nullptr, nullptr, nullptr, nullptr, 0};
+                         nullptr, nullptr, nullptr, nullptr, nullptr, 0, tab.rbm, tab.rbf};
         const Rows vrows{ver.cen, ver.scl, ver.pref, ver.cf1, ver.cf2, ver.w, ver.kind, ver.key, ver.next,
                          ver.tile_dsq, ver.dsq, ver.tau, ver.skip, nullptr, nullptr, nullptr, 0};
         const Rows crows{car.cen, car.scl, car.pref, car.cf1, car.cf2, car.w, car.kind, car.key, nullptr,
@@ -393,11 +408,12 @@
         int* const long_list = long_listed ? h->long_list.p : nullptr;
         const int long_cap = long_few ? (int)std::min<long long>(CC_LONG_CAP, 2 * long_avg + 8) : CC_LONG_CAP;
         ScanCopy scopy[2] = {ScanCopy{}, ScanCopy{}};
-        if (la_on) scan_copy_sync(h, scopy);
+        if (la_on) scan_copy_sync(h, scopy, rec_on);
         Rows srows[2];
         for (int q = 0; q < 2; ++q)
             srows[q] = Rows{scopy[q].cen, scopy[q].scl, nullptr, scopy[q].cf1, scopy[q].cf2, scopy[q].w, scopy[q].kind,
-                            scopy[q].key, nullptr, nullptr, nullptr, nullptr, nullptr, nullptr, nullptr, nullptr, 0};
+                            scopy[q].key, nullptr, nullptr, nullptr, nullptr, nullptr, nullptr, nullptr, nullptr, 0,
+                            scopy[q].rbm, scopy[q].rbf};
         evScan = nullptr;
         if (la_on) HIPCHK(hipEventRecord(evCommit, sA));
         int probe_left = (dec.probe != 0) ? 1 : 0;
@@ -721,16 +737,25 @@
         prepare();
         while (done < N) {
             ensure_table(h, (size_t)m_known + std::max<size_t>(window_rows(), seq_on ? 8192 : 0) + 1);
-            const Table tab = h->tab.view();
+            Table tab = h->tab.view();
+            if (!rec_on) tab.rbm = nullptr, tab.rbf = nullptr;
             if (seq_on) {
                 sequential_stint(tab);
                 continue;
             }
+            ensure_rowrec(tab);
             enqueue_batch(tab);
             const int rc = after_batch();
             if (rc != CC_OK) return rc;
         }
         finish();
+        if (rec_on && h->rowbits == 2) {
+            int bad_row = 0;
+            HIPCHK(hipMemcpy(&bad_row, h->badflag.p + 1, sizeof(int), hipMemcpyDeviceToHost));
+            if (bad_row != 0)
+                return fail(h, CC_ERR_INTERNAL, "CHRONOCLUST_HIP_ROWBITS=2: the scan record of table row " + std::to_string(bad_row - 1) +
+                            " (or of its scan copy) differs from the row a snapshot scan read");
+        }
         return (int)CC_OK;
     }
 };
diff --git a/chronoclust_amd/csrc/cc_scan.h b/chronoclust_amd/csrc/cc_scan.h
--- a/chronoclust_amd/csrc/cc_scan.h
+++ b/chronoclust_amd/csrc/cc_scan.h
@@ -541,14 +541,16 @@
     return row;
 }
 
-template <int DP, int NW>
+template <int DP, int NW, bool REC>
 __global__ __launch_bounds__(64 * NW, ScanUShape<DP>::WGS) void k_scan_u(const Ctl* __restrict__ ctl, const double* __restrict__ Xt,
                                                                  const double* __restrict__ g_cen,
                                                                  const double* __restrict__ g_scl,
                                                                  const int* __restrict__ g_kind,
                                                                  const int* __restrict__ g_key, Cand* __restrict__ part,
                                                                  int round, int mode, size_t part_stride, int shard_rank,
-                                                                 int shard_world, const int* __restrict__ plist = nullptr)
+                                                                 int shard_world, const int* __restrict__ plist,
+                                                                 const unsigned long long* __restrict__ g_rbm,
+                                                                 const unsigned* __restrict__ g_rbf)
 {
     static_assert(DP % 2 == 0 && DP >= 4 && DP <= 64, "padded dimensionalities are even");
     constexpr int NP = DP / 2;
@@ -622,9 +624,24 @@
 #pragma unroll
             for (int i = 0; i < 2 * (NP / NC); ++i) buf[0][i] = c0[i];
         }
+        unsigned pmask = 0u, omask = 0u;
+        bool all_p = false, all_o = false;
         constexpr int NL = (CC_SCAN_TM * DP + 63) / 64;
         int rm_lo = 0, rm_hi = 0;
         bool fuse_tile;
+        if constexpr (REC) {
+            const int rl = lane & (CC_SCAN_TM - 1);
+            const unsigned long long rmask = g_rbm[rt + rl];
+            const unsigned fl = (lane < tm) ? g_rbf[rt + lane] : (CC_RB_NOT_PCORE | CC_RB_NOT_OUTLIER);
+            rm_lo = (int)(unsigned)(rmask & 0xFFFFFFFFull);
+            rm_hi = (int)(unsigned)(rmask >> 32);
+            fuse_tile = fuse_wave && __builtin_amdgcn_ballot_w64((fl & CC_RB_TINY) != 0u) == 0ull;
+            pmask = (unsigned)__builtin_amdgcn_ballot_w64((fl & CC_RB_NOT_PCORE) == 0u);
+            omask = (unsigned)__builtin_amdgcn_ballot_w64((fl & CC_RB_NOT_OUTLIER) == 0u);
+            const unsigned full = (1u << tm) - 1u;
+            all_p = pmask == full;
+            all_o = omask == full;
+        } else {
         {
             const double* gc = g_cen + (size_t)rt * DP;
             const double* gs = g_scl + (size_t)rt * DP;
@@ -649,11 +666,14 @@
             rm_hi = (int)(unsigned)(rmask >> 32);
             fuse_tile = fuse_wave && __builtin_amdgcn_ballot_w64(tn) == 0ull;
         }
-        unsigned pmask, omask;
         {
             const int kd = (lane < tm) ? g_kind[rt + lane] : CC_KIND_DEAD;
             pmask = (unsigned)__builtin_amdgcn_ballot_w64(kd == CC_KIND_PCORE);
             omask = (unsigned)__builtin_amdgcn_ballot_w64(kd == CC_KIND_OUTLIER);
+            const unsigned full = (1u << tm) - 1u;
+            all_p = pmask == full;
+            all_o = omask == full;
+        }
         }
         auto rows_of_tile = [&](auto FUSEC, auto KSELC) {
             constexpr bool FUSE = decltype(FUSEC)::value;
@@ -729,10 +749,9 @@
                 }
             }
         };
-        const unsigned full = (1u << tm) - 1u;
         if (fuse_tile) {
-            if (pmask == full) rows_of_tile(std::true_type{}, std::integral_constant<int, 0>{});
-            else if (omask == full) rows_of_tile(std::true_type{}, std::integral_constant<int, 1>{});
+            if (all_p) rows_of_tile(std::true_type{}, std::integral_constant<int, 0>{});
+            else if (all_o) rows_of_tile(std::true_type{}, std::integral_constant<int, 1>{});
             else rows_of_tile(std::true_type{}, std::integral_constant<int, -1>{});
         } else rows_of_tile(std::false_type{}, std::integral_constant<int, -1>{});
     }
diff --git a/chronoclust_amd/csrc/cc_validate.h b/chronoclust_amd/csrc/cc_validate.h
--- a/chronoclust_amd/csrc/cc_validate.h
+++ b/chronoclust_amd/csrc/cc_validate.h
@@ -426,7 +426,57 @@
     double* w;
     int* kind;
     int* key;
+    unsigned long long* rbm;
+    unsigned* rbf;
 };
+
+__device__ __forceinline__ void cc_group_rowrec(const bool (&scaled)[2], bool tiny, int kind, unsigned long long* rbm, unsigned* rbf)
+{
+    const unsigned lo = cc_group_ballot(scaled[0]), hi = cc_group_ballot(scaled[1]);
+    *rbm = (unsigned long long)lo | ((unsigned long long)hi << 32);
+    *rbf = cc_rb_flags(cc_group_ballot(tiny) != 0u, kind);
+}
+
+template <bool VERIFY>
+__global__ __launch_bounds__(256) void k_rowbits(const Ctl* __restrict__ ctl, const double* __restrict__ cen,
+                                                 const double* __restrict__ scl, const int* __restrict__ kind,
+                                                 unsigned long long* __restrict__ rbm, unsigned* __restrict__ rbf, int m_rows, int d,
+                                                 int round, int mode, int* __restrict__ bad)
+{
+    if (VERIFY) {
+        if (mode == 1) {
+            if (ctl->la_b[round & 1] == 0) return;
+            m_rows = ctl->la_rows[round & 1];
+        } else {
+            if (ctl->mode != 0 || ctl->win_b == 0) return;
+            m_rows = ctl->m_rows;
+        }
+    }
+    const int gl = threadIdx.x & 31;
+    const int groups = (gridDim.x * blockDim.x) >> 5;
+    for (int r = (blockIdx.x * blockDim.x + threadIdx.x) >> 5; r < m_rows; r += groups) {
+        bool scaled[2] = {false, false}, tiny = false;
+#pragma unroll
+        for (int h = 0; h < 2; ++h) {
+            const int i = gl + 32 * h;
+            if (i >= d) continue;
+            const size_t e = (size_t)r * d + i;
+            scaled[h] = scl[e] != 1.0;
+            tiny = tiny || cc_is_tiny(cen[e]);
+        }
+        unsigned long long m;
+        unsigned f;
+        cc_group_rowrec(scaled, tiny, kind[r], &m, &f);
+        if (gl == 0) {
+            if (VERIFY) {
+                if (rbm[r] != m || rbf[r] != f) atomicMax(bad, r + 1);
+            } else {
+                rbm[r] = m;
+                rbf[r] = f;
+            }
+        }
+    }
+}
 
 struct CommitRec {
     int n;
@@ -450,19 +500,27 @@
         const int kind = car.kind[j];
         if (kind == CC_KIND_DEAD) continue;
         const size_t row = (size_t)car.slot[j];
+        bool scaled[2] = {false, false}, tiny = false;
 #pragma unroll
         for (int h = 0; h < 2; ++h) {
             const int i = gl + 32 * h;
             if (i >= d) continue;
             const size_t e = row * d + i, v = (size_t)j * d + i;
-            sc.cen[e] = car.cen[v];
-            sc.scl[e] = car.scl[v];
+            const double ncen = car.cen[v], nscl = car.scl[v];
+            sc.cen[e] = ncen;
+            sc.scl[e] = nscl;
+            scaled[h] = nscl != 1.0;
+            tiny = tiny || cc_is_tiny(ncen);
             if (filter) { sc.cf1[e] = car.cf1[v]; sc.cf2[e] = car.cf2[v]; }
         }
+        unsigned long long rbm = 0ull;
+        unsigned rbf = 0u;
+        if (sc.rbm) cc_group_rowrec(scaled, tiny, kind, &rbm, &rbf);
         if (gl == 0) {
             sc.kind[row] = kind;
             sc.key[row] = car.key[j];
             if (filter) sc.w[row] = car.w[j];
+            if (sc.rbm) { sc.rbm[row] = rbm; sc.rbf[row] = rbf; }
         }
     }
 }
@@ -1887,12 +1945,15 @@
         const int kind0 = (t < M0) ? tab.kind[row] : CC_KIND_DEAD;
         double dq = 0.0;
         bool metric_moved = false;
+        bool scaled[2] = {false, false}, tiny = false;
 #pragma unroll
         for (int h = 0; h < 2; ++h) {
             const int i = gl + 32 * h;
             if (i >= d) continue;
             const size_t e = row * d + i, v = (size_t)j * d + i;
             const double ncen = ver.cen[v], npref = ver.pref[v], nscl = ver.scl[v], n1 = ver.cf1[v], n2 = ver.cf2[v];
+            scaled[h] = nscl != 1.0;
+            tiny = tiny || cc_is_tiny(ncen);
             if (carry) {
                 const double oc = (t < M0) ? tab.cen[e] : 0.0;
                 const double ow = (t < M0) ? 1.0 / tab.pref[e] : 0.0;
@@ -1913,9 +1974,13 @@
             const bool promoted = kind == CC_KIND_PCORE && kind0 == CC_KIND_OUTLIER;
             if (kind0 == CC_KIND_DEAD || (kind != kind0 && !promoted) || !(dq >= 0.0) || cc_group_ballot(metric_moved) != 0u) dq = CC_INF;
         }
+        unsigned long long rbm = 0ull;
+        unsigned rbf = 0u;
+        if (tab.rbm) cc_group_rowrec(scaled, tiny, kind, &rbm, &rbf);
         if (gl == 0) {
             tab.w[row] = ver.w[j];
             tab.kind[row] = kind;
+            if (tab.rbm) { tab.rbm[row] = rbm; tab.rbf[row] = rbf; }
             if (u >= 0) {
                 tab.key[row] = key;
                 tab.id[row] = rec->pid0 + (long long)((unsigned)rk[u] >> 16);
@@ -1928,6 +1993,7 @@
                 sc.kind[row] = kind;
                 sc.key[row] = key;
                 if (filter) sc.w[row] = ver.w[j];
+                if (sc.rbm) { sc.rbm[row] = rbm; sc.rbf[row] = rbf; }
             }
             if (carry) {
                 car.w[j] = ver.w[j];
```

Measured after the change: 75.06 million points/s, median of 2. Within noise of the previous version (+0.0%).
